# lucieDLE/TMRNet

Measured on AMD Instinct MI355X. Metric: train frames/sec, TMRNet ResNet50 seq=10 LFB=40, higher is better.
Workload: dtype fp32; 1 GPU; C2/C3: TMRNet ResNet50+LSTM+NLBlock train step; model=resnet_lstm (train_only_non-local_pretrained), global_batch=64, clips_per_gpu=64, seq_len=10, lfb_len=40, parallelism=dp1, input_transform=reference train transform (use_flip=1) on device

## Files before the change

### include/tmr.h

```cpp
#ifndef TMR_H_
#define TMR_H_

#ifdef TMR_HOST_ONLY
typedef struct ihipStream_t* hipStream_t;
#else
#include <hip/hip_runtime.h>
#endif
#include <stddef.h>
#include <stdint.h>

#ifdef __cplusplus
extern "C" {
#endif

#define TMR_ABI_VERSION 8

int tmr_abi_version(void);
const char* tmr_last_error(void);
void tmr_clear_error(void);

typedef struct tmr_conv_desc {
  int n, h, w, c;
  int k;
  int r, s, stride, pad;
  int ho, wo;
  int pad_w;
  int x_ld, y_ld;
  int math;
  int max_frames;
  int io;
  int groups;
} tmr_conv_desc;
#define TMR_MATH_F32 0
#define TMR_MATH_BF16 1
#define TMR_IO_X_BF16 1
#define TMR_IO_W_BF16 2
#define TMR_IO_DY_BF16 4
#define TMR_IO_Y_BF16 16
#define TMR_IO_BN_BF16 32
#define TMR_IO_G16 128
#define TMR_IO_WT_BF16 8
#define TMR_IO_ENGINE 256
#define TMR_IO_CLASSES 512
#define TMR_IO_TILES 1024
#define TMR_IO_WT_F32 64

int tmr_conv2d_fwd(const tmr_conv_desc* d, const float* x, const float* w_krsc,
                   const float* bias, float* y, float beta, hipStream_t stream);
int tmr_conv2d_fwd_fused(const tmr_conv_desc* d, const float* x, const float* w_krsc,
                         const float* scale, const float* shift, const float* residual, float* y,
                         int relu, hipStream_t stream);
int tmr_conv2d_fwd_stats_parts(const tmr_conv_desc* d);
int tmr_conv2d_fwd_bnstats(const tmr_conv_desc* d, const float* x, const float* w_krsc, float* y,
                           void* stats, size_t stats_bytes, hipStream_t stream);
int tmr_conv2d_dgrad(const tmr_conv_desc* d, const float* dy, const float* w_krsc, float* dx,
                     float beta, hipStream_t stream);
int tmr_conv2d_dgrad_bnbwd_parts(const tmr_conv_desc* d);
int tmr_conv2d_dgrad_bnbwd(const tmr_conv_desc* d, const float* dy, const float* w_krsc, float* dx,
                           float beta, const float* y, const float* z, const float* scale,
                           const float* shift, const float* mean, int mask, void* parts,
                           size_t parts_bytes, hipStream_t stream);
size_t tmr_conv2d_wgrad_ws_bytes(const tmr_conv_desc* d);
int tmr_conv2d_wgrad(const tmr_conv_desc* d, const float* x, const float* dy, float* dw_oihw,
                     int c_real, float beta, float* ws, size_t ws_bytes, hipStream_t stream);
int tmr_conv2d_dgrad_bnbwd_acc(const tmr_conv_desc* d, const float* dy, const float* w_krsc,
                               void* dx, float beta, const void* dx_old, int old_bf16,
                               const float* y, const float* z, const float* scale,
                               const float* shift, const float* mean, int mask, void* parts,
                               size_t parts_bytes, hipStream_t stream);
int tmr_gemm_nt(int M, int N, int K, const float* A, int lda, const float* B, int ldb,
                const float* bias, float* C, int ldc, float beta, hipStream_t stream);
int tmr_gemm_nn(int M, int N, int K, const float* A, int lda, const float* B, int ldb, float* C,
                int ldc, float beta, hipStream_t stream);
int tmr_gemm_tn(int M, int N, int K, const float* A, int lda, const float* B, int ldb, float* C,
                int ldc, float beta, hipStream_t stream);

int tmr_weight_oihw_to_krsc(const float* w, float* wk, int k, int c, int r, int s, int cpad,
                            hipStream_t stream);
int tmr_nchw_to_nhwc(const float* x, float* y, int n, int c, int h, int w, int cpad,
                     hipStream_t stream);
int tmr_nhwc_to_nchw(const float* x, float* y, int n, int c, int cstore, int h, int w,
                     hipStream_t stream);
int tmr_crop_normalize(const uint8_t* frames, const int32_t* offsets, float* out, int f, int hin,
                       int win, int seq_len, int crop, float m0, float m1, float m2, float s0,
                       float s1, float s2, hipStream_t stream);

typedef struct tmr_clip_aug {
  int32_t x1, y1;
  int32_t flip;
  int32_t rotate;
  int32_t a[6];
  int32_t jitter;
  int32_t hue_shift;
  float brightness, contrast, saturation;
  int32_t reserved;
} tmr_clip_aug;
int tmr_clip_augment(const uint8_t* frames, const tmr_clip_aug* params, int32_t* lmean, float* out,
                     int f, int hin, int win, int crop, float m0, float m1, float m2, float s0,
                     float s1, float s2, hipStream_t stream);

size_t tmr_bn_ws_bytes(int rows, int c);
int tmr_bn_fwd_stats(const float* y, int rows, int c, const float* gamma, const float* beta,
                     float* running_mean, float* running_var, float momentum, float eps,
                     float* save_mean, float* save_invstd, float* scale, float* shift, void* ws,
                     size_t ws_bytes, hipStream_t stream);
int tmr_bn_finalize(const void* partials, int nparts, int c, const float* gamma, const float* beta,
                    float* running_mean, float* running_var, float momentum, float eps,
                    float* save_mean, float* save_invstd, float* scale, float* shift,
                    hipStream_t stream);
size_t tmr_bn_parts_ws_bytes(int nparts, int c);
int tmr_bn_finalize_ws(const void* partials, int nparts, int c, const float* gamma,
                       const float* beta, float* running_mean, float* running_var, float momentum,
                       float eps, float* save_mean, float* save_invstd, float* scale, float* shift,
                       void* ws, size_t ws_bytes, hipStream_t stream);
int tmr_bn_eval_params(const float* gamma, const float* beta, const float* running_mean,
                       const float* running_var, float eps, int c, float* scale, float* shift,
                       hipStream_t stream);
int tmr_bn_apply(const float* y, const float* scale, const float* shift, const float* residual,
                 float* z, int rows, int c, int relu, hipStream_t stream);
int tmr_bn_apply2(const float* y, const float* scale, const float* shift, const float* yr,
                  const float* rscale, const float* rshift, float* z, int rows, int c, int relu,
                  hipStream_t stream);
int tmr_bn_bwd_maxpool(const float* dyp, const uint8_t* argmax, int n, int h, int w, int ho, int wo,
                       const float* y, const float* scale, const float* shift,
                       const float* save_mean, const float* save_invstd, const float* gamma,
                       float* dy, float* dgamma, float* dbeta, int c, void* ws, size_t ws_bytes,
                       hipStream_t stream);
int tmr_bn_bwd_parts(const float* g, const float* y, const void* parts, int nparts,
                     const float* save_mean, const float* save_invstd, const float* gamma,
                     float* dy, float* dgamma, float* dbeta, int rows, int c, void* ws,
                     size_t ws_bytes, hipStream_t stream);
int tmr_bn_bwd(const float* dz, const float* y, const float* z, const float* scale,
               const float* shift, const float* save_mean, const float* save_invstd,
               const float* gamma, float* dy, float* dres, float* dgamma, float* dbeta, int rows,
               int c, int relu, void* ws, size_t ws_bytes, hipStream_t stream);

int tmr_bn_apply_x(const float* y, const float* scale, const float* shift, const float* residual,
                   void* z, int rows, int c, int relu, int out_bf16, hipStream_t stream);
int tmr_bn_bwd_parts_x(const float* g, const float* y, const void* parts, int nparts,
                       const float* save_mean, const float* save_invstd, const float* gamma,
                       void* dy, float* dgamma, float* dbeta, int rows, int c, void* ws,
                       size_t ws_bytes, int out_bf16, hipStream_t stream);
int tmr_bn_bwd_x(const float* dz, const float* y, const float* z, const float* scale,
                 const float* shift, const float* save_mean, const float* save_invstd,
                 const float* gamma, void* dy, float* dres, float* dgamma, float* dbeta, int rows,
                 int c, int relu, void* ws, size_t ws_bytes, int out_bf16, hipStream_t stream);
int tmr_bn_bwd_maxpool_x(const float* dyp, const uint8_t* argmax, int n, int h, int w, int ho,
                         int wo, const float* y, const float* scale, const float* shift,
                         const float* save_mean, const float* save_invstd, const float* gamma,
                         void* dy, float* dgamma, float* dbeta, int c, void* ws, size_t ws_bytes,
                         int out_bf16, hipStream_t stream);
int tmr_weight_oihw_to_krsc_x(const float* w, void* wk, int k, int c, int r, int s, int cpad,
                              int out_bf16, hipStream_t stream);
int tmr_weight_oihw_to_crsk_x(const float* w, void* wt, int k, int c, int r, int s, int out_bf16,
                              hipStream_t stream);
typedef struct tmr_wlayout {
  const float* w;
  void* out;
  long long n;
  long long block0;
  int k, c, rs, cpad;
  int kind, bf16;
} tmr_wlayout;
int tmr_weight_layouts_epb(void);
int tmr_weight_layouts_multi(const tmr_wlayout* table, int n, int total_blocks, hipStream_t stream);
int tmr_bn_apply_dual(const float* y, const float* scale, const float* shift, const float* residual,
                      float* z, void* z16, int rows, int c, int relu, hipStream_t stream);
int tmr_bn_apply_bits(const float* y, const float* scale, const float* shift,
                      const float* residual, float* z, uint32_t* bits, int rows, int c,
                      hipStream_t stream);
int tmr_bn_apply2_bits(const float* y, const float* scale, const float* shift, const float* yr,
                       const float* rscale, const float* rshift, float* z, uint32_t* bits,
                       int rows, int c, hipStream_t stream);
int tmr_bn_apply2_x(const float* y, const float* scale, const float* shift, const float* yr,
                    const float* rscale, const float* rshift, float* z, void* z16, int rows, int c,
                    int relu, hipStream_t stream);
int tmr_maxpool2d_fwd_bn_x(const float* x, const float* scale, const float* shift, void* y,
                           uint8_t* argmax, int n, int h, int w, int c, int ho, int wo, int out_bf16,
                           hipStream_t stream);

int tmr_bn_apply_a16(const void* y, const float* scale, const float* shift, const void* residual,
                     void* z, int rows, int c, int relu, hipStream_t stream);
int tmr_bn_apply2_a16(const void* y, const float* scale, const float* shift, const void* yr,
                      const float* rscale, const float* rshift, void* z, int rows, int c, int relu,
                      hipStream_t stream);
int tmr_bn_apply_bits_a16(const void* y, const float* scale, const float* shift,
                          const void* residual, void* z, uint32_t* bits, int rows, int c,
                          hipStream_t stream);
int tmr_bn_apply2_bits_a16(const void* y, const float* scale, const float* shift, const void* yr,
                           const float* rscale, const float* rshift, void* z, uint32_t* bits,
                           int rows, int c, hipStream_t stream);
int tmr_bn_bwd_a16(const float* dz, const void* y, const void* z, const float* scale,
                   const float* shift, const float* save_mean, const float* save_invstd,
                   const float* gamma, void* dy, float* dres, float* dgamma, float* dbeta, int rows,
                   int c, int relu, void* ws, size_t ws_bytes, hipStream_t stream);
int tmr_bn_bwd_parts_a16(const float* g, const void* y, const void* parts, int nparts,
                         const float* save_mean, const float* save_invstd, const float* gamma,
                         void* dy, float* dgamma, float* dbeta, int rows, int c, void* ws,
                         size_t ws_bytes, hipStream_t stream);
int tmr_bn_bwd_parts_g16(const void* g, const void* y, const void* parts, int nparts,
                         const float* save_mean, const float* save_invstd, const float* gamma,
                         void* dy, float* dgamma, float* dbeta, int rows, int c, void* ws,
                         size_t ws_bytes, hipStream_t stream);
int tmr_bn_bwd_g16(const void* dz, const void* y, const float* save_mean,
                   const float* save_invstd, const float* gamma, void* dy, float* dgamma,
                   float* dbeta, int rows, int c, void* ws, size_t ws_bytes, hipStream_t stream);
size_t tmr_bn_bwd_parts_ds_ws_bytes(int nparts, int rows, int c);
int tmr_bn_bwd_parts_ds(const void* g, const void* y, const void* parts, int nparts,
                        const float* save_mean, const float* save_invstd, const float* gamma,
                        void* dy, float* dgamma, float* dbeta, const void* y_ds,
                        const float* save_mean_ds, const float* save_invstd_ds,
                        const float* gamma_ds, void* dy_ds, float* dgamma_ds, float* dbeta_ds,
                        int rows, int c, int bf16, void* ws, size_t ws_bytes, hipStream_t stream);
int tmr_bn_bwd_maxpool_a16(const float* dyp, const uint8_t* argmax, int n, int h, int w, int ho,
                           int wo, const void* y, const float* scale, const float* shift,
                           const float* save_mean, const float* save_invstd, const float* gamma,
                           void* dy, float* dgamma, float* dbeta, int c, void* ws, size_t ws_bytes,
                           hipStream_t stream);
int tmr_maxpool2d_fwd_bn_a16(const void* x, const float* scale, const float* shift, void* y,
                             uint8_t* argmax, int n, int h, int w, int c, int ho, int wo,
                             hipStream_t stream);
int tmr_avgpool_fwd_a16(const void* x, float* y, int n, int hw, int c, hipStream_t stream);
int tmr_cast_f32_bf16(const float* x, void* y, long n, hipStream_t stream);
int tmr_nhwc4_to_bf16x8(const float* x4, void* y8, long npix, hipStream_t stream);

int tmr_resize_ksize(int in_size, int out_size);
int tmr_resize_coeffs(int in_size, int out_size, int32_t* bounds, int32_t* k, int ksize);
size_t tmr_resize_tmp_bytes(int n, int h, int w, int oh, int ow);
int tmr_resize_u8(const uint8_t* in, int n, int h, int w, uint8_t* tmp, size_t tmp_bytes,
                  uint8_t* out, int oh, int ow, const int32_t* bounds_h, const int32_t* k_h,
                  int ksize_h, const int32_t* bounds_v, const int32_t* k_v, int ksize_v, int y0,
                  int y1, hipStream_t stream);
#define TMR_RESIZE_BOX_INTS 10
int tmr_resize_u8_boxes(const uint8_t* in, int n, int h, int w, const int32_t* desc_host,
                        const int32_t* desc, const int32_t* pool, long pool_ints, uint8_t* tmp,
                        size_t tmp_bytes, uint8_t* out, int oh, int ow, hipStream_t stream);

size_t tmr_margin_ws_bytes(int n, int h, int w);
int tmr_margin_boxes(const uint8_t* in, int n, int h, int w, void* ws, size_t ws_bytes,
                     int32_t* boxes, hipStream_t stream);
int tmr_margin_mask(const uint8_t* in, int n, int h, int w, void* ws, size_t ws_bytes,
                    uint8_t* mask, hipStream_t stream);
int tmr_frame_sums(const uint8_t* in, int n, int h, int w, int64_t* sums, hipStream_t stream);

#define TMR_JPEG_GRAY 0
#define TMR_JPEG_444 1
#define TMR_JPEG_420 2
typedef struct tmr_jpeg_info {
  int32_t width, height;
  int32_t ncomp;
  int32_t sampling;
  int32_t blocks_w[3], blocks_h[3];
  uint16_t qt[3][64];
  uint64_t coef_bytes;
} tmr_jpeg_info;
int tmr_jpeg_probe(const uint8_t* data, size_t len, tmr_jpeg_info* info);
int tmr_jpeg_entropy_decode(const uint8_t* data, size_t len, tmr_jpeg_info* info, int16_t* coef,
                            size_t coef_bytes);
size_t tmr_jpeg_ws_bytes(int f, int h, int w, int sampling);
int tmr_jpeg_reconstruct(const int16_t* coef, const uint16_t* qt, int f, int h, int w,
                         int sampling, uint8_t* ws, size_t ws_bytes, uint8_t* out,
                         const int32_t* out_index, int out_frames, hipStream_t stream);

int tmr_maxpool2d_fwd(const float* x, float* y, uint8_t* argmax, int n, int h, int w, int c,
                      int ho, int wo, hipStream_t stream);
int tmr_maxpool2d_bwd(const float* dy, const uint8_t* argmax, float* dx, int n, int h, int w,
                      int c, int ho, int wo, hipStream_t stream);
int tmr_maxpool2d_fwd_bn(const float* x, const float* scale, const float* shift, float* y,
                         uint8_t* argmax, int n, int h, int w, int c, int ho, int wo,
                         hipStream_t stream);
int tmr_avgpool_fwd(const float* x, float* y, int n, int hw, int c, hipStream_t stream);
int tmr_avgpool_bwd(const float* dy, float* dx, int n, int hw, int c, hipStream_t stream);

int tmr_splat_gap(const float* x, float* gap, int n, int hw, int c, hipStream_t stream);
int tmr_splat_combine(const float* x, const float* z, float* att, float* out, int n, int hw, int c,
                      hipStream_t stream);
int tmr_splat_bwd(const float* dout, const float* x, const float* att, float* dz, int n, int hw,
                  int c, hipStream_t stream);
int tmr_splat_bwd_apply(const float* dout, const float* att, const float* dgap, float* dx, int n,
                        int hw, int c, hipStream_t stream);
int tmr_center_cols(const float* x, int rows, int cols, float* center, float* xc,
                    hipStream_t stream);
int tmr_axpy(int n, float alpha, const float* x, float* y, hipStream_t stream);
int tmr_avgpool2d_fwd(const float* x, float* y, int n, int h, int w, int c, int ho, int wo, int k,
                      int s, int p, int count_include_pad, hipStream_t stream);
int tmr_avgpool2d_bwd(const float* dy, float* dx, int n, int h, int w, int c, int ho, int wo, int k,
                      int s, int p, int count_include_pad, hipStream_t stream);

int tmr_splat_gap_bn(const void* y, const float* scale, const float* shift, float* gap, int n,
                     int hw, int c, int act16, hipStream_t stream);
int tmr_splat_att(const float* zl, float* att, int n, int c, hipStream_t stream);
int tmr_splat_combine_bn(const void* y, const float* scale, const float* shift, const float* att,
                         void* out, int n, int hw, int c, int act16, hipStream_t stream);
int tmr_splat_bwd_reduce_bn(const float* dout, const void* y, const float* scale,
                            const float* shift, const float* mean, const float* att, float* dzl,
// ... 147 lines not shown
```

### tmrnet_amd/_lib.py

```python
import ctypes
import os

import torch

_HERE = os.path.dirname(os.path.abspath(__file__))
LIB_PATH = os.environ.get("TMR_LIB_PATH") or os.path.join(_HERE, "libtmr.so")

P = ctypes.c_void_p
I = ctypes.c_int
L = ctypes.c_long
F = ctypes.c_float
U64 = ctypes.c_uint64
SZ = ctypes.c_size_t


class ConvDesc(ctypes.Structure):
    _fields_ = [(n, ctypes.c_int) for n in
                ("n", "h", "w", "c", "k", "r", "s", "stride", "pad", "ho", "wo", "pad_w",
                 "x_ld", "y_ld", "math", "max_frames", "io", "groups")]


DP = ctypes.POINTER(ConvDesc)


_NL_FIELDS = ("w1", "b1", "w2", "b2", "w3", "b3", "ln_w", "ln_b", "w4", "b4")


class NLBlockPtrs(ctypes.Structure):
    _fields_ = [(n, ctypes.c_void_p) for n in _NL_FIELDS]


class JpegInfo(ctypes.Structure):
    _fields_ = [("width", ctypes.c_int32), ("height", ctypes.c_int32), ("ncomp", ctypes.c_int32),
                ("sampling", ctypes.c_int32), ("blocks_w", ctypes.c_int32 * 3),
                ("blocks_h", ctypes.c_int32 * 3), ("qt", (ctypes.c_uint16 * 64) * 3),
                ("coef_bytes", ctypes.c_uint64)]


JP = ctypes.POINTER(JpegInfo)

SIGNATURES = {
    "tmr_abi_version": [],
    "tmr_last_error": [],
    "tmr_clear_error": [],
    "tmr_conv2d_fwd": [DP, P, P, P, P, F, P],
    "tmr_conv2d_fwd_fused": [DP, P, P, P, P, P, P, I, P],
    "tmr_conv2d_fwd_stats_parts": [DP],
    "tmr_conv2d_fwd_bnstats": [DP, P, P, P, P, SZ, P],
    "tmr_conv2d_dgrad": [DP, P, P, P, F, P],
    "tmr_conv2d_dgrad_bnbwd_parts": [DP],
    "tmr_conv2d_dgrad_bnbwd": [DP, P, P, P, F, P, P, P, P, P, I, P, SZ, P],
    "tmr_conv2d_wgrad_ws_bytes": [DP],
    "tmr_conv2d_wgrad": [DP, P, P, P, I, F, P, SZ, P],
    "tmr_conv2d_dgrad_bnbwd_acc": [DP, P, P, P, F, P, I, P, P, P, P, P, I, P, SZ, P],
    "tmr_bn_apply_x": [P, P, P, P, P, I, I, I, I, P],
    "tmr_bn_bwd_parts_x": [P, P, P, I, P, P, P, P, P, P, I, I, P, SZ, I, P],
    "tmr_bn_bwd_x": [P, P, P, P, P, P, P, P, P, P, P, P, I, I, I, P, SZ, I, P],
    "tmr_bn_bwd_maxpool_x": [P, P, I, I, I, I, I, P, P, P, P, P, P, P, P, P, I, P, SZ, I, P],
    "tmr_weight_oihw_to_krsc_x": [P, P, I, I, I, I, I, I, P],
    "tmr_weight_oihw_to_crsk_x": [P, P, I, I, I, I, I, P],
    "tmr_bn_apply_dual": [P, P, P, P, P, P, I, I, I, P],
    "tmr_bn_apply2_x": [P, P, P, P, P, P, P, P, I, I, I, P],
    "tmr_bn_apply_bits": [P, P, P, P, P, P, I, I, P],
    "tmr_bn_apply2_bits": [P, P, P, P, P, P, P, P, I, I, P],
    "tmr_maxpool2d_fwd_bn_x": [P, P, P, P, P, I, I, I, I, I, I, I, P],
    "tmr_bn_apply_a16": [P, P, P, P, P, I, I, I, P],
    "tmr_bn_apply2_a16": [P, P, P, P, P, P, P, I, I, I, P],
    "tmr_bn_apply_bits_a16": [P, P, P, P, P, P, I, I, P],
    "tmr_bn_apply2_bits_a16": [P, P, P, P, P, P, P, P, I, I, P],
    "tmr_bn_bwd_a16": [P, P, P, P, P, P, P, P, P, P, P, P, I, I, I, P, SZ, P],
    "tmr_bn_bwd_parts_a16": [P, P, P, I, P, P, P, P, P, P, I, I, P, SZ, P],
    "tmr_bn_bwd_parts_g16": [P, P, P, I, P, P, P, P, P, P, I, I, P, SZ, P],
    "tmr_bn_bwd_g16": [P, P, P, P, P, P, P, P, I, I, P, SZ, P],
    "tmr_weight_layouts_epb": [],
    "tmr_weight_layouts_multi": [P, I, I, P],
    "tmr_bn_bwd_parts_ds_ws_bytes": [I, I, I],
    "tmr_bn_bwd_parts_ds": [P, P, P, I, P, P, P, P, P, P, P, P, P, P, P, P, P, I, I, I, P, SZ, P],
    "tmr_bn_bwd_maxpool_a16": [P, P, I, I, I, I, I, P, P, P, P, P, P, P, P, P, I, P, SZ, P],
    "tmr_maxpool2d_fwd_bn_a16": [P, P, P, P, P, I, I, I, I, I, I, P],
    "tmr_avgpool_fwd_a16": [P, P, I, I, I, P],
    "tmr_cast_f32_bf16": [P, P, ctypes.c_long, P],
    "tmr_nhwc4_to_bf16x8": [P, P, ctypes.c_long, P],
    "tmr_adam_step_multi": [P, I, ctypes.c_int64, P, P],
    "tmr_resize_ksize": [I, I],
    "tmr_resize_coeffs": [I, I, P, P, I],
    "tmr_resize_tmp_bytes": [I, I, I, I, I],
    "tmr_resize_u8": [P, I, I, I, P, SZ, P, I, I, P, P, I, P, P, I, I, I, P],
    "tmr_resize_u8_boxes": [P, I, I, I, P, P, P, L, P, SZ, P, I, I, P],
    "tmr_margin_ws_bytes": [I, I, I],
    "tmr_margin_boxes": [P, I, I, I, P, SZ, P, P],
    "tmr_margin_mask": [P, I, I, I, P, SZ, P, P],
    "tmr_frame_sums": [P, I, I, I, P, P],
    "tmr_jpeg_probe": [P, SZ, JP],
    "tmr_jpeg_entropy_decode": [P, SZ, JP, P, SZ],
    "tmr_jpeg_ws_bytes": [I, I, I, I],
    "tmr_jpeg_reconstruct": [P, P, I, I, I, I, P, SZ, P, P, I, P],
    "tmr_gemm_nt": [I, I, I, P, I, P, I, P, P, I, F, P],
    "tmr_gemm_nn": [I, I, I, P, I, P, I, P, I, F, P],
    "tmr_gemm_tn": [I, I, I, P, I, P, I, P, I, F, P],
    "tmr_weight_oihw_to_krsc": [P, P, I, I, I, I, I, P],
    "tmr_nchw_to_nhwc": [P, P, I, I, I, I, I, P],
    "tmr_nhwc_to_nchw": [P, P, I, I, I, I, I, P],
    "tmr_clip_augment": [P, P, P, P, I, I, I, I, F, F, F, F, F, F, P],
    "tmr_crop_normalize": [P, P, P, I, I, I, I, I, F, F, F, F, F, F, P],
    "tmr_bn_ws_bytes": [I, I],
    "tmr_bn_fwd_stats": [P, I, I, P, P, P, P, F, F, P, P, P, P, P, SZ, P],
    "tmr_bn_finalize": [P, I, I, P, P, P, P, F, F, P, P, P, P, P],
    "tmr_bn_finalize_ws": [P, I, I, P, P, P, P, F, F, P, P, P, P, P, SZ, P],
    "tmr_bn_parts_ws_bytes": [I, I],
    "tmr_bn_eval_params": [P, P, P, P, F, I, P, P, P],
    "tmr_bn_apply": [P, P, P, P, P, I, I, I, P],
    "tmr_bn_apply2": [P, P, P, P, P, P, P, I, I, I, P],
    "tmr_bn_bwd_parts": [P, P, P, I, P, P, P, P, P, P, I, I, P, SZ, P],
    "tmr_bn_bwd_maxpool": [P, P, I, I, I, I, I, P, P, P, P, P, P, P, P, P, I, P, SZ, P],
    "tmr_bn_bwd": [P, P, P, P, P, P, P, P, P, P, P, P, I, I, I, P, SZ, P],
    "tmr_maxpool2d_fwd": [P, P, P, I, I, I, I, I, I, P],
    "tmr_maxpool2d_fwd_bn": [P, P, P, P, P, I, I, I, I, I, I, P],
    "tmr_maxpool2d_bwd": [P, P, P, I, I, I, I, I, I, P],
    "tmr_avgpool_fwd": [P, P, I, I, I, P],
    "tmr_avgpool_bwd": [P, P, I, I, I, P],
    "tmr_splat_gap": [P, P, I, I, I, P],
    "tmr_splat_combine": [P, P, P, P, I, I, I, P],
    "tmr_splat_bwd": [P, P, P, P, I, I, I, P],
    "tmr_splat_bwd_apply": [P, P, P, P, I, I, I, P],
    "tmr_splat_gap_bn": [P, P, P, P, I, I, I, I, P],
    "tmr_splat_att": [P, P, I, I, P],
    "tmr_splat_combine_bn": [P, P, P, P, P, I, I, I, I, P],
    "tmr_splat_bwd_reduce_bn": [P, P, P, P, P, P, P, P, I, I, I, I, P],
    "tmr_splat_bn0_coefs": [P, P, P, P, P, P, P, P, P, I, I, I, P],
    "tmr_splat_bwd_apply_bn": [P, P, P, P, P, P, P, P, P, I, I, I, I, P],
    "tmr_avgpool2d_fwd_a16": [P, P, I, I, I, I, I, I, I, I, I, I, P],
    "tmr_fill_f32": [P, L, F, P],
    "tmr_seq_last": [P, P, I, I, I, P],
    "tmr_seq_last_bwd": [P, P, P, I, I, I, P],
    "tmr_counters_add": [P, I, ctypes.c_int64, P],
    "tmr_center_cols": [P, I, I, P, P, P],
    "tmr_axpy": [I, F, P, P, P],
    "tmr_avgpool2d_fwd": [P, P, I, I, I, I, I, I, I, I, I, I, P],
    "tmr_avgpool2d_bwd": [P, P, I, I, I, I, I, I, I, I, I, I, P],
    "tmr_col_sum": [P, I, I, I, P, F, P],
    "tmr_dropout_mask": [P, L, F, U64, U64, P],
    "tmr_softmax_max": [P, I, I, P, P, P, P],
    "tmr_ce_sum": [P, P, P, I, I, F, P, P, P, P],
    "tmr_sgd_chunk": [],
    "tmr_sgd_step_multi": [P, I, ctypes.c_int64, P, P],
    "tmr_sgd_step": [P, P, P, L, F, F, F, F, I, I, P],
    "tmr_lfb_index": [P, I, P, I, I, P, P],
    "tmr_lfb_gather": [P, P, P, L, I, P],
    "tmr_layernorm_relu_fwd": [P, P, P, P, P, P, I, I, F, P],
    "tmr_layernorm_relu_bwd": [P, P, P, P, P, P, P, P, P, I, I, P],
    "tmr_residual_mask": [P, P, P, P, L, P],
    "tmr_mask_relu_fwd": [P, P, P, L, P],
    "tmr_mask_relu_bwd": [P, P, P, P, L, P],
    "tmr_mul": [P, P, P, P, L, P],
    "tmr_nl_attn_ws_bytes": [I, I, I],
    "tmr_nl_attn_fwd": [P, P, P, P, P, I, I, I, F, P, SZ, P],
    "tmr_nl_attn_bwd": [P, P, P, P, P, P, P, I, I, I, F, P, SZ, P],
    "tmr_linear_fwd": [P, I, I, I, P, P, P, P],
    "tmr_linear_bwd": [P, P, I, I, I, P, P, P, P, F, P],
    "tmr_nlblock_saved_bytes": [I, I],
    "tmr_nlblock_ws_bytes": [I, I],
    "tmr_nlblock_fwd": [P, P, P, P, I, I, P, P, P, SZ, P, SZ, P],
    "tmr_nlblock_bwd": [P, P, P, P, P, I, I, P, P, SZ, P, P, P, P, SZ, P],
    "tmr_timeconv_saved_bytes": [I, I],
    "tmr_timeconv_ws_bytes": [I, I],
    "tmr_timeconv_fwd": [P, I, I, P, P, P, P, P, P, P, P, SZ, P, SZ, P],
    "tmr_timeconv_wgrad": [P, P, I, I, P, P, P, P, SZ, P, P, P, P, P, P, P, P, SZ, P],
    "tmr_lstm_saved_bytes": [I, I, I],
    "tmr_lstm_ws_bytes": [I, I, I, I],
    "tmr_lstm_fwd": [P, I, I, I, I, P, P, P, P, P, P, P, P, SZ, P, SZ, P],
    "tmr_lstm_bwd": [P, P, I, I, I, I, P, P, P, P, SZ, P, P, P, P, P, P, SZ, P],
    "tmr_lstm_window_ws_bytes": [I, I, I],
    "tmr_lstm_window_fwd": [P, L, P, I, I, I, P, P, P, P, SZ, P],
    "tmr_lstm_sync_status": [P,ctypes.POINTER(ctypes.c_uint), P],
    "tmr_lstm_status_or": [P, P, P],
    "tmr_test_hold_cus": [I, F, P],
    "tmr_dgrad_ws_launches": [],
    "tmr_timeconv_max5_fwd": [P, P, P, P, P, P, I, I, I, P],
    "tmr_timeconv_max5_bwd": [P, P, P, P, P, P, I, I, I, P],
    "tmr_lstm_cell_fwd": [P, I, P, P, P, I, P, P, I, I, P],
    "tmr_lstm_cell_bwd": [P, I, P, P, P, P, P, P, I, P, I, I, P],
}
_RESTYPES = {
    "tmr_last_error": ctypes.c_char_p,
    "tmr_clear_error": None,
    "tmr_conv2d_wgrad_ws_bytes": SZ,
    "tmr_dgrad_ws_launches": L,
    "tmr_resize_tmp_bytes": SZ,
    "tmr_margin_ws_bytes": SZ,
    "tmr_jpeg_ws_bytes": SZ,
    "tmr_bn_ws_bytes": SZ,
    "tmr_bn_parts_ws_bytes": SZ,
    "tmr_bn_bwd_parts_ds_ws_bytes": SZ,
    "tmr_sgd_chunk": ctypes.c_int64,
    "tmr_nl_attn_ws_bytes": SZ,
    "tmr_nlblock_saved_bytes": SZ,
    "tmr_nlblock_ws_bytes": SZ,
    "tmr_timeconv_saved_bytes": SZ,
    "tmr_timeconv_ws_bytes": SZ,
    "tmr_lstm_saved_bytes": SZ,
    "tmr_lstm_ws_bytes": SZ,
    "tmr_lstm_window_ws_bytes": SZ,
}

_lib = None


def lib():
    global _lib
    if _lib is None:
        if not os.path.exists(LIB_PATH):
            raise RuntimeError(
                "libtmr.so not found at %s: build it with `make` or "
                "`python -c 'import __graft_entry__ as g; g.build()'` (no CPU fallback exists)"
                % LIB_PATH)
        h = ctypes.CDLL(LIB_PATH)
        for name, args in SIGNATURES.items():
            fn = getattr(h, name)
            fn.argtypes = args
            fn.restype = _RESTYPES.get(name, ctypes.c_int)
        _lib = h
    return _lib


def exported_symbols():
    return list(SIGNATURES)


def _conv(a):
    if isinstance(a, torch.Tensor):
        return ctypes.c_void_p(a.data_ptr())
    return a


def stream_ptr(device=None):
    return ctypes.c_void_p(torch.cuda.current_stream(device).cuda_stream)


def call(name, *args):
    fn = getattr(lib(), name)
    rc = fn(*[_conv(a) for a in args])
    if rc != 0:
        raise RuntimeError("%s failed (%d): %s" % (name, rc, lib().tmr_last_error().decode()))
    return rc


def query(name, *args):
    h = lib()
    h.tmr_clear_error()
    fn = getattr(h, name)
    v = fn(*[_conv(a) for a in args])
    err = h.tmr_last_error()
    if (_RESTYPES.get(name, ctypes.c_int) is ctypes.c_int and v < 0) or err:
        raise RuntimeError("%s failed (%d): %s" % (name, v, (err or b"").decode()))
    return v
```

### tmrnet_amd/csrc/bn.hip

```cpp
#include "common.h"
#include "tmr.h"
#include <type_traits>

namespace {

constexpr int NT = 256;

struct Plan {
  int cthreads;
  int rthreads;
  int cblocks;
  int rpb;
  int nrb;
};

Plan make_plan(int rows, int c) {
  Plan p;
  int c4 = c / 4;
  p.cthreads = c4 < 64 ? c4 : 64;
  p.rthreads = NT / p.cthreads;
  p.cblocks = c4 / p.cthreads;
  int rpb = rows / 1024;
  int minr = p.rthreads * 8;
  if (rpb < minr) rpb = minr;
// ... 914 lines not shown
        ld8(y, pix * c8 + cq, v);
#pragma unroll
        for (int e = 0; e < 8; ++e) g[e] = 0.f;
#pragma unroll
        for (int ddy = 0; ddy < 2; ++ddy)
#pragma unroll
          for (int ddx = 0; ddx < 2; ++ddx) {
            if (ddy > py || ddx > px || !pin[ddy][ddx]) continue;
            const uint32_t id = (uint32_t)((py + 1 - 2 * ddy) * 3 + (px + 1 - 2 * ddx));
            const float dv[8] = {d0[ddy][ddx].x, d0[ddy][ddx].y, d0[ddy][ddx].z, d0[ddy][ddx].w,
                                 d1[ddy][ddx].x, d1[ddy][ddx].y, d1[ddy][ddx].z, d1[ddy][ddx].w};
#pragma unroll
            for (int e = 0; e < 8; ++e) {
              const uint32_t ab = ((e < 4 ? a[ddy][ddx].x : a[ddy][ddx].y) >> (8 * (e & 3))) & 0xffu;
              if (ab == id) g[e] += dv[e];
            }
          }
        float o[8];
#pragma unroll
        for (int e = 0; e < 8; ++e) {
          const float gm = fmaf(v[e], sc[e], sf[e]) > 0.f ? g[e] : 0.f;
          o[e] = fmaf(A[e], gm, fmaf(B[e], v[e], C[e]));
        }
        st8(dy, pix * c8 + cq, o);
      }
  }
}

#ifndef TMR_BN_BITS8
#define TMR_BN_BITS8 1
#endif
template <bool RES>
__global__ __launch_bounds__(NT) void bn_apply_bits8_k(const float* __restrict__ y,
                                                       const float* __restrict__ scale,
                                                       const float* __restrict__ shift,
                                                       const float* __restrict__ res,
                                                       const float* __restrict__ yr,
                                                       const float* __restrict__ rscale,
                                                       const float* __restrict__ rshift,
                                                       float* __restrict__ z,
                                                       uint32_t* __restrict__ bits, long n8, int c8) {
  const int lane = threadIdx.x & 63;
  const long stride = (long)gridDim.x * NT;
  auto apply = [&](long i, const float (&yv)[8], const float (&rv)[8]) -> uint32_t {
    const int cc = chan_of(i, c8) * 8;
    float v[8];
#pragma unroll
    for (int h = 0; h < 2; ++h) {
      const float4 sc = *reinterpret_cast<const float4*>(scale + cc + 4 * h);
      const float4 sf = *reinterpret_cast<const float4*>(shift + cc + 4 * h);
      const float s4[4] = {sc.x, sc.y, sc.z, sc.w}, f4[4] = {sf.x, sf.y, sf.z, sf.w};
      if (yr) {
        const float4 rs = *reinterpret_cast<const float4*>(rscale + cc + 4 * h);
        const float4 rf = *reinterpret_cast<const float4*>(rshift + cc + 4 * h);
        const float r4[4] = {rs.x, rs.y, rs.z, rs.w}, q4[4] = {rf.x, rf.y, rf.z, rf.w};
#pragma unroll
        for (int e = 0; e < 4; ++e)
          v[4 * h + e] = fmaf(yv[4 * h + e], s4[e], f4[e]) + fmaf(rv[4 * h + e], r4[e], q4[e]);
      } else {
#pragma unroll
        for (int e = 0; e < 4; ++e) {
          v[4 * h + e] = fmaf(yv[4 * h + e], s4[e], f4[e]);
          if (RES) v[4 * h + e] += rv[4 * h + e];
        }
      }
    }
    uint32_t b = 0;
#pragma unroll
    for (int e = 0; e < 8; ++e) {
      v[e] = fmaxf(v[e], 0.f);
      b |= (uint32_t)(v[e] > 0.f) << e;
    }
    st8(z, i, v);
    return b;
  };
  auto put = [&](uint32_t byte, long i, bool ok) {
    uint32_t w = byte << (8 * (lane & 3));
    w |= (uint32_t)__shfl_xor((int)w, 1, 64);
    w |= (uint32_t)__shfl_xor((int)w, 2, 64);
    if ((lane & 3) == 0 && ok) bits[i >> 2] = w;
  };
  const float* rsrc = RES ? res : yr;
  for (long base = blockIdx.x * (long)NT + (threadIdx.x & ~63); base < n8; base += 2 * stride) {
    const long i = base + lane, j = i + stride;
    const bool oi = i < n8, oj = j < n8;
    float ya[8], ra[8], yb[8], rb[8];
    if (oi) {
      ld8(y, i, ya);
      if (rsrc) ld8(rsrc, i, ra);
    }
    if (oj) {
      ld8(y, j, yb);
      if (rsrc) ld8(rsrc, j, rb);
    }
    const uint32_t bi = oi ? apply(i, ya, ra) : 0u;
    const uint32_t bj = oj ? apply(j, yb, rb) : 0u;
    put(bi, i, oi);
    put(bj, j, oj);
  }
}

int ew_blocks(long n4) {
  long b = (n4 + NT - 1) / NT;
  if (b > 2048 * 4) b = 2048 * 4;
  return (int)(b > 0 ? b : 1);
}

}

TMR_API size_t tmr_bn_ws_bytes(int rows, int c) {
  if (rows <= 0 || c < 4 || c % 4) {
    tmr_set_error("tmr_bn_ws_bytes: bad size (rows %d, channels %d)", rows, c);
    return 0;
  }
  return ws_need(rows, c);
}

TMR_API int tmr_bn_fwd_stats(const float* y, int rows, int c, const float* gamma,
                             const float* beta, float* running_mean, float* running_var,
                             float momentum, float eps, float* save_mean, float* save_invstd,
                             float* scale, float* shift, void* ws, size_t ws_bytes,
                             hipStream_t stream) {
  TMR_CHECK_ARG(c % 4 == 0 && c >= 4, "tmr_bn_fwd_stats: channels %d must be a multiple of 4", c);
  TMR_CHECK_ARG(rows > 0, "tmr_bn_fwd_stats: empty input");
  TMR_CHECK_ARG(plan_covers(c), "tmr_bn_fwd_stats: unsupported channel count %d", c);
  TMR_CHECK_ARG(ws && ws_bytes >= ws_need(rows, c), "tmr_bn_fwd_stats: workspace too small");
  Plan p = make_plan(rows, c);
  float4* part = (float4*)ws;
  hipLaunchKernelGGL(bn_stats_partial, dim3(p.nrb, p.cblocks), dim3(NT), 0, stream, y, rows, c,
                     p.rpb, p.cthreads, part);
  TMR_CHECK_LAUNCH("bn_stats_partial");
  return tmr_bn_finalize(part, p.nrb, c, gamma, beta, running_mean, running_var, momentum, eps,
                         save_mean, save_invstd, scale, shift, stream);
}

TMR_API int tmr_bn_finalize(const void* partials, int nparts, int c, const float* gamma,
                            const float* beta, float* running_mean, float* running_var,
                            float momentum, float eps, float* save_mean, float* save_invstd,
                            float* scale, float* shift, hipStream_t stream) {
  TMR_CHECK_ARG(nparts > 0 && c > 0, "tmr_bn_finalize: empty partials");
  hipLaunchKernelGGL(bn_finalize_k, dim3(c), dim3(NT), 0, stream, (const float4*)partials,
                     nparts, c, gamma, beta, running_mean, running_var, momentum, eps, save_mean,
                     save_invstd, scale, shift);
  TMR_CHECK_LAUNCH("bn_finalize");
  return 0;
}

TMR_API size_t tmr_bn_parts_ws_bytes(int nparts, int c) {
  if (nparts <= 0 || c <= 0) {
    tmr_set_error("tmr_bn_parts_ws_bytes: bad size (parts %d, channels %d)", nparts, c);
    return 0;
  }
  return slab_ws_bytes(nparts, c) + (size_t)3 * c * sizeof(float) + 64;
}

TMR_API int tmr_bn_finalize_ws(const void* partials, int nparts, int c, const float* gamma,
                               const float* beta, float* running_mean, float* running_var,
                               float momentum, float eps, float* save_mean, float* save_invstd,
                               float* scale, float* shift, void* ws, size_t ws_bytes,
                               hipStream_t stream) {
  TMR_CHECK_ARG(nparts > 0 && c > 0, "tmr_bn_finalize_ws: empty partials");
  TMR_CHECK_ARG(ws && ws_bytes >= slab_ws_bytes(nparts, c), "tmr_bn_finalize_ws: workspace too small");
  const SlabPlan p = slab_plan(nparts, c);
  hipLaunchKernelGGL(parts_slab_k<0>, dim3(p.groups, p.nslabs), dim3(256), 0, stream, partials,
                     nparts, c, p.rows, (double*)ws);
  TMR_CHECK_LAUNCH("bn_parts_slab");
  hipLaunchKernelGGL(finalize_slabs_k, dim3(p.groups), dim3(SLAB_CH * SLAB_PH), 0, stream,
                     (const double*)ws, p.nslabs, (const float4*)partials, c, gamma, beta,
                     running_mean, running_var, momentum, eps, save_mean, save_invstd, scale,
                     shift);
  TMR_CHECK_LAUNCH("bn_finalize_slabs");
  return 0;
}

TMR_API int tmr_bn_eval_params(const float* gamma, const float* beta, const float* running_mean,
                               const float* running_var, float eps, int c, float* scale,
                               float* shift, hipStream_t stream) {
  hipLaunchKernelGGL(bn_eval_params_k, dim3(cdiv(c, 256)), dim3(256), 0, stream, gamma, beta,
                     running_mean, running_var, eps, c, scale, shift);
  TMR_CHECK_LAUNCH("bn_eval_params");
  return 0;
}

TMR_API int tmr_bn_apply(const float* y, const float* scale, const float* shift,
                         const float* residual, float* z, int rows, int c, int relu,
                         hipStream_t stream) {
  return tmr_bn_apply_x(y, scale, shift, residual, z, rows, c, relu, 0, stream);
}

TMR_API int tmr_bn_apply_x(const float* y, const float* scale, const float* shift,
                           const float* residual, void* zv, int rows, int c, int relu,
                           int out_bf16, hipStream_t stream) {
  TMR_CHECK_ARG(c % 4 == 0, "tmr_bn_apply: channels %d must be a multiple of 4", c);
  long n4 = (long)rows * c / 4;
  int nb = ew_blocks(n4);
  int c4 = c / 4;
  if (out_bf16) {
    TMR_CHECK_ARG(!residual, "tmr_bn_apply_x: a bf16 output is for conv-operand-only tensors (no residual)");
    if (relu) hipLaunchKernelGGL((bn_apply_k<false, true, __bf16>), dim3(nb), dim3(NT), 0, stream, y, scale, shift, residual, (__bf16*)zv, n4, c4);
    else hipLaunchKernelGGL((bn_apply_k<false, false, __bf16>), dim3(nb), dim3(NT), 0, stream, y, scale, shift, residual, (__bf16*)zv, n4, c4);
    TMR_CHECK_LAUNCH("bn_apply");
    return 0;
  }
  float* z = (float*)zv;
  if (residual) {
    if (relu) hipLaunchKernelGGL((bn_apply_k<true, true>), dim3(nb), dim3(NT), 0, stream, y, scale, shift, residual, z, n4, c4);
    else hipLaunchKernelGGL((bn_apply_k<true, false>), dim3(nb), dim3(NT), 0, stream, y, scale, shift, residual, z, n4, c4);
  } else {
    if (relu) hipLaunchKernelGGL((bn_apply_k<false, true>), dim3(nb), dim3(NT), 0, stream, y, scale, shift, residual, z, n4, c4);
    else hipLaunchKernelGGL((bn_apply_k<false, false>), dim3(nb), dim3(NT), 0, stream, y, scale, shift, residual, z, n4, c4);
  }
  TMR_CHECK_LAUNCH("bn_apply");
  return 0;
}

TMR_API int tmr_bn_apply2(const float* y, const float* scale, const float* shift, const float* yr,
                          const float* rscale, const float* rshift, float* z, int rows, int c,
                          int relu, hipStream_t stream) {
  return tmr_bn_apply2_x(y, scale, shift, yr, rscale, rshift, z, nullptr, rows, c, relu, stream);
}

TMR_API int tmr_bn_apply2_x(const float* y, const float* scale, const float* shift, const float* yr,
                            const float* rscale, const float* rshift, float* z, void* z16,
                            int rows, int c, int relu, hipStream_t stream) {
  TMR_CHECK_ARG(c % 4 == 0, "tmr_bn_apply2: channels %d must be a multiple of 4", c);
  TMR_CHECK_ARG(y && scale && shift && yr && rscale && rshift && z, "tmr_bn_apply2: null operand");
  TMR_CHECK_ARG(yr != z, "tmr_bn_apply2: the branch input must not alias z");
  const long n4 = (long)rows * c / 4;
  __bf16* h = (__bf16*)z16;
  if (relu && h)
    hipLaunchKernelGGL((bn_apply2_k<true, true>), dim3(ew_blocks(n4)), dim3(NT), 0, stream, y, scale,
                       shift, yr, rscale, rshift, z, n4, c / 4, h);
  else if (relu)
    hipLaunchKernelGGL((bn_apply2_k<true>), dim3(ew_blocks(n4)), dim3(NT), 0, stream, y, scale, shift,
                       yr, rscale, rshift, z, n4, c / 4, h);
  else if (h)
    hipLaunchKernelGGL((bn_apply2_k<false, true>), dim3(ew_blocks(n4)), dim3(NT), 0, stream, y, scale,
                       shift, yr, rscale, rshift, z, n4, c / 4, h);
  else
    hipLaunchKernelGGL((bn_apply2_k<false>), dim3(ew_blocks(n4)), dim3(NT), 0, stream, y, scale, shift,
                       yr, rscale, rshift, z, n4, c / 4, h);
  TMR_CHECK_LAUNCH("bn_apply2");
  return 0;
}

TMR_API int tmr_bn_apply_bits(const float* y, const float* scale, const float* shift,
                              const float* residual, float* z, uint32_t* bits, int rows, int c,
                              hipStream_t stream) {
  TMR_CHECK_ARG(c % 4 == 0 && y && scale && shift && z && bits,
                "tmr_bn_apply_bits: null operand or channels %d not a multiple of 4", c);
  const long n4 = (long)rows * c / 4;
  if (n4 == 0) return 0;
  if (TMR_BN_BITS8 && c % 8 == 0 && (((uintptr_t)y | (uintptr_t)residual | (uintptr_t)z) & 15) == 0) {
    if (residual)
      hipLaunchKernelGGL((bn_apply_bits8_k<true>), dim3(ew_blocks(n4 / 2)), dim3(NT), 0, stream, y,
                         scale, shift, residual, nullptr, nullptr, nullptr, z, bits, n4 / 2, c / 8);
    else
      hipLaunchKernelGGL((bn_apply_bits8_k<false>), dim3(ew_blocks(n4 / 2)), dim3(NT), 0, stream, y,
                         scale, shift, nullptr, nullptr, nullptr, nullptr, z, bits, n4 / 2, c / 8);
  } else if (residual)
    hipLaunchKernelGGL((bn_apply_bits_k<true, float>), dim3(ew_blocks(n4)), dim3(NT), 0, stream, y, scale,
                       shift, residual, nullptr, nullptr, nullptr, z, bits, n4, c / 4);
  else
    hipLaunchKernelGGL((bn_apply_bits_k<false, float>), dim3(ew_blocks(n4)), dim3(NT), 0, stream, y, scale,
                       shift, nullptr, nullptr, nullptr, nullptr, z, bits, n4, c / 4);
  TMR_CHECK_LAUNCH("bn_apply_bits");
  return 0;
}

TMR_API int tmr_bn_apply2_bits(const float* y, const float* scale, const float* shift,
                               const float* yr, const float* rscale, const float* rshift, float* z,
                               uint32_t* bits, int rows, int c, hipStream_t stream) {
  TMR_CHECK_ARG(c % 4 == 0 && y && scale && shift && yr && rscale && rshift && z && bits,
                "tmr_bn_apply2_bits: null operand or channels %d not a multiple of 4", c);
  TMR_CHECK_ARG(yr != z, "tmr_bn_apply2_bits: the branch input must not alias z");
  const long n4 = (long)rows * c / 4;
  if (n4 == 0) return 0;
  if (TMR_BN_BITS8 && c % 8 == 0 && (((uintptr_t)y | (uintptr_t)yr | (uintptr_t)z) & 15) == 0)
    hipLaunchKernelGGL((bn_apply_bits8_k<false>), dim3(ew_blocks(n4 / 2)), dim3(NT), 0, stream, y,
                       scale, shift, nullptr, yr, rscale, rshift, z, bits, n4 / 2, c / 8);
  else
    hipLaunchKernelGGL((bn_apply_bits_k<false, float>), dim3(ew_blocks(n4)), dim3(NT), 0, stream, y, scale,
                       shift, nullptr, yr, rscale, rshift, z, bits, n4, c / 4);
  TMR_CHECK_LAUNCH("bn_apply2_bits");
  return 0;
}

TMR_API int tmr_bn_apply_bits_a16(const void* y, const float* scale, const float* shift,
                                  const void* residual, void* z, uint32_t* bits, int rows, int c,
                                  hipStream_t stream) {
  TMR_CHECK_ARG(c % 4 == 0 && y && scale && shift && z && bits,
                "tmr_bn_apply_bits_a16: null operand or channels %d not a multiple of 4", c);
  const long n4 = (long)rows * c / 4;
  if (n4 == 0) return 0;
  const __bf16* yb = (const __bf16*)y;
  if (residual)
    hipLaunchKernelGGL((bn_apply_bits_k<true, __bf16>), dim3(ew_blocks(n4)), dim3(NT), 0, stream, yb,
                       scale, shift, (const __bf16*)residual, nullptr, nullptr, nullptr, (__bf16*)z,
                       bits, n4, c / 4);
  else
    hipLaunchKernelGGL((bn_apply_bits_k<false, __bf16>), dim3(ew_blocks(n4)), dim3(NT), 0, stream, yb,
                       scale, shift, nullptr, nullptr, nullptr, nullptr, (__bf16*)z, bits, n4, c / 4);
  TMR_CHECK_LAUNCH("bn_apply_bits_a16");
  return 0;
}

// ... 55 lines not shown
  double* part = (double*)ws;
  float* coef = (float*)((char*)ws + (size_t)p.nrb * c * 2 * sizeof(double));
  const dim3 pg(p.nrb, p.cblocks);
  float* dzw = const_cast<float*>(dz);
  if (dres == dz) {
    if (mask == 1)
      hipLaunchKernelGGL((bn_bwd_partial<1, true>), pg, dim3(NT), 0, stream, dzw, y, z, scale, shift, save_mean, rows, c, p.rpb, p.cthreads, part);
    else if (mask == 2)
      hipLaunchKernelGGL((bn_bwd_partial<2, true>), pg, dim3(NT), 0, stream, dzw, y, z, scale, shift, save_mean, rows, c, p.rpb, p.cthreads, part);
    else
      hipLaunchKernelGGL((bn_bwd_partial<0>), pg, dim3(NT), 0, stream, dzw, y, z, scale, shift, save_mean, rows, c, p.rpb, p.cthreads, part);
    mask = 0;
    dres = nullptr;
  } else if (mask == 1)
    hipLaunchKernelGGL((bn_bwd_partial<1>), pg, dim3(NT), 0, stream, dzw, y, z, scale, shift, save_mean, rows, c, p.rpb, p.cthreads, part);
  else if (mask == 2)
    hipLaunchKernelGGL((bn_bwd_partial<2>), pg, dim3(NT), 0, stream, dzw, y, z, scale, shift, save_mean, rows, c, p.rpb, p.cthreads, part);
  else
    hipLaunchKernelGGL((bn_bwd_partial<0>), pg, dim3(NT), 0, stream, dzw, y, z, scale, shift, save_mean, rows, c, p.rpb, p.cthreads, part);
  TMR_CHECK_LAUNCH("bn_bwd_partial");
  hipLaunchKernelGGL(bn_bwd_final, dim3(c), dim3(NT), 0, stream, part, p.nrb, rows, c,
                     save_mean, save_invstd, gamma, dgamma, dbeta, coef);
  TMR_CHECK_LAUNCH("bn_bwd_final");
  long n4 = (long)rows * c / 4;
  int nb = ew_blocks(n4);
  int c4 = c / 4;
#define TMR_BN_APPLY(M, D)                                                                     \
  if (out_bf16)                                                                                  \
    hipLaunchKernelGGL((bn_bwd_apply<M, D, __bf16>), dim3(nb), dim3(NT), 0, stream, dz, y, z,    \
                       scale, shift, coef, (__bf16*)dyv, dres, n4, c4);                          \
  else                                                                                           \
    hipLaunchKernelGGL((bn_bwd_apply<M, D>), dim3(nb), dim3(NT), 0, stream, dz, y, z, scale,     \
                       shift, coef, (float*)dyv, dres, n4, c4)
  if (dres) {
    if (mask == 1) { TMR_BN_APPLY(1, true); } else if (mask == 2) { TMR_BN_APPLY(2, true); } else { TMR_BN_APPLY(0, true); }
  } else {
    if (mask == 1) { TMR_BN_APPLY(1, false); } else if (mask == 2) { TMR_BN_APPLY(2, false); } else { TMR_BN_APPLY(0, false); }
  }
#undef TMR_BN_APPLY
  TMR_CHECK_LAUNCH("bn_bwd_apply");
  return 0;
}

TMR_API int tmr_bn_bwd_maxpool(const float* dyp, const uint8_t* argmax, int n, int h, int w,
                               int ho, int wo, const float* y, const float* scale,
                               const float* shift, const float* save_mean,
                               const float* save_invstd, const float* gamma, float* dy,
                               float* dgamma, float* dbeta, int c, void* ws, size_t ws_bytes,
                               hipStream_t stream) {
  return tmr_bn_bwd_maxpool_x(dyp, argmax, n, h, w, ho, wo, y, scale, shift, save_mean,
                              save_invstd, gamma, dy, dgamma, dbeta, c, ws, ws_bytes, 0, stream);
}

static int bn_bwd_maxpool_impl(const float* dyp, const uint8_t* argmax, int n, int h, int w,
                               int ho, int wo, const float* y, const float* scale,
                               const float* shift, const float* save_mean,
                               const float* save_invstd, const float* gamma, void* dyv,
                               float* dgamma, float* dbeta, int c, void* ws, size_t ws_bytes,
                               int out_bf16, float* coef_out, hipStream_t stream);

TMR_API int tmr_bn_bwd_maxpool_x(const float* dyp, const uint8_t* argmax, int n, int h, int w,
                                 int ho, int wo, const float* y, const float* scale,
                                 const float* shift, const float* save_mean,
                                 const float* save_invstd, const float* gamma, void* dyv,
                                 float* dgamma, float* dbeta, int c, void* ws, size_t ws_bytes,
                                 int out_bf16, hipStream_t stream) {
  TMR_CHECK_ARG(c >= 4 && plan_covers(c), "tmr_bn_bwd_maxpool: unsupported channel count %d", c);
  TMR_CHECK_ARG(dyv, "tmr_bn_bwd_maxpool: null dy");
  return bn_bwd_maxpool_impl(dyp, argmax, n, h, w, ho, wo, y, scale, shift, save_mean,
                             save_invstd, gamma, dyv, dgamma, dbeta, c, ws, ws_bytes, out_bf16,
                             nullptr, stream);
}

static int bn_bwd_maxpool_impl(const float* dyp, const uint8_t* argmax, int n, int h, int w,
                               int ho, int wo, const float* y, const float* scale,
                               const float* shift, const float* save_mean,
                               const float* save_invstd, const float* gamma, void* dyv,
                               float* dgamma, float* dbeta, int c, void* ws, size_t ws_bytes,
                               int out_bf16, float* coef_out, hipStream_t stream) {
  const long rows_l = (long)n * h * w;
  TMR_CHECK_ARG(c % 4 == 0 && c >= 4 && rows_l > 0 && rows_l < 0x7fffffffL,
                "tmr_bn_bwd_maxpool: bad shape n=%d h=%d w=%d c=%d", n, h, w, c);
  TMR_CHECK_ARG(ho == (h + 2 - 3) / 2 + 1 && wo == (w + 2 - 3) / 2 + 1,
                "tmr_bn_bwd_maxpool: pooled %dx%d is not MaxPool2d(3,2,1) of %dx%d", ho, wo, h, w);
  const int rows = (int)rows_l;
  TMR_CHECK_ARG(plan_covers(c), "tmr_bn_bwd_maxpool: unsupported channel count %d", c);
  TMR_CHECK_ARG(ws && ws_bytes >= ws_need(rows, c), "tmr_bn_bwd_maxpool: workspace too small");
  PoolGeo pg;
  pg.dyp = dyp; pg.am = (const uchar4*)argmax;
  pg.dHW = make_fastdiv((uint32_t)(h * w)); pg.dW = make_fastdiv((uint32_t)w);
  pg.ho = ho; pg.wo = wo;
  const int prows = n * ho * wo;
  Plan p = make_plan(prows, c);
  double* part = (double*)ws;
  float* coef = coef_out ? coef_out : (float*)((char*)ws + (size_t)p.nrb * c * 2 * sizeof(double));
  hipLaunchKernelGGL(stem_bwd_partial_pooled<float>, dim3(p.nrb, p.cblocks), dim3(NT), 0, stream, pg, h, w,
                     y, scale, shift, save_mean, prows, c, p.rpb, p.cthreads,
                     make_fastdiv((uint32_t)(ho * wo)), make_fastdiv((uint32_t)wo), part);
  TMR_CHECK_LAUNCH("stem_bwd_partial_pooled");
  hipLaunchKernelGGL(bn_bwd_final, dim3(c), dim3(NT), 0, stream, part, p.nrb, rows, c,
                     save_mean, save_invstd, gamma, dgamma, dbeta, coef);
  TMR_CHECK_LAUNCH("bn_bwd_final");
  if (!dyv) return 0;
  const long n4 = rows_l * c / 4;
  const int c8 = c / 8;
  if (c % 8 == 0 && (c8 & (c8 - 1)) == 0 && n4 / 2 < 0x7fffffffL &&
      (((uintptr_t)dyp | (uintptr_t)y | (uintptr_t)dyv) & 15) == 0 && ((uintptr_t)argmax & 7) == 0) {
    const int qh = (h + 1) / 2, qw = (w + 1) / 2;
    const int nq = n * qh * qw * c8;
    const FastDiv dqhw = make_fastdiv((uint32_t)(qh * qw)), dqw = make_fastdiv((uint32_t)qw);
    if (out_bf16)
      hipLaunchKernelGGL((stem_bwd_apply8q<float, __bf16>), dim3(ew_blocks(nq)), dim3(NT), 0, stream,
                         pg, h, w, dqhw, dqw, y, scale, shift, coef, (__bf16*)dyv, nq, __builtin_ctz(c8));
    else
      hipLaunchKernelGGL((stem_bwd_apply8q<float, float>), dim3(ew_blocks(nq)), dim3(NT), 0, stream,
                         pg, h, w, dqhw, dqw, y, scale, shift, coef, (float*)dyv, nq, __builtin_ctz(c8));
  } else if (out_bf16)
    hipLaunchKernelGGL(stem_bwd_apply<__bf16>, dim3(ew_blocks(n4)), dim3(NT), 0, stream, pg, y, scale,
                       shift, coef, (__bf16*)dyv, n4, c / 4);
  else
    hipLaunchKernelGGL(stem_bwd_apply<float>, dim3(ew_blocks(n4)), dim3(NT), 0, stream, pg, y, scale,
                       shift, coef, (float*)dyv, n4, c / 4);
  TMR_CHECK_LAUNCH("stem_bwd_apply");
  return 0;
}

TMR_API int tmr_bn_bwd_parts(const float* g, const float* y, const void* parts, int nparts,
                             const float* save_mean, const float* save_invstd, const float* gamma,
                             float* dy, float* dgamma, float* dbeta, int rows, int c, void* ws,
                             size_t ws_bytes, hipStream_t stream) {
  return tmr_bn_bwd_parts_x(g, y, parts, nparts, save_mean, save_invstd, gamma, dy, dgamma, dbeta,
                            rows, c, ws, ws_bytes, 0, stream);
}

TMR_API int tmr_bn_bwd_parts_x(const float* g, const float* y, const void* parts, int nparts,
                               const float* save_mean, const float* save_invstd,
                               const float* gamma, void* dyv, float* dgamma, float* dbeta,
                               int rows, int c, void* ws, size_t ws_bytes, int out_bf16,
                               hipStream_t stream) {
  TMR_CHECK_ARG(c % 4 == 0 && c >= 4 && rows > 0 && nparts > 0,
                "tmr_bn_bwd_parts: bad shape rows=%d c=%d parts=%d", rows, c, nparts);
  TMR_CHECK_ARG(ws && ws_bytes >= tmr_bn_parts_ws_bytes(nparts, c),
                "tmr_bn_bwd_parts: workspace too small (need tmr_bn_parts_ws_bytes)");
  const SlabPlan sp = slab_plan(nparts, c);
  double* slabs = (double*)ws;
  float* coef = (float*)((char*)ws + slab_ws_bytes(nparts, c));
  hipLaunchKernelGGL(parts_slab_k<1>, dim3(sp.groups, sp.nslabs), dim3(256), 0, stream, parts,
                     nparts, c, sp.rows, slabs);
  TMR_CHECK_LAUNCH("bn_parts_slab");
  hipLaunchKernelGGL(bwd_final_slabs_k, dim3(sp.groups), dim3(SLAB_CH * SLAB_PH), 0, stream,
                     (const double*)slabs, sp.nslabs, rows, c, save_mean, save_invstd, gamma,
                     dgamma, dbeta, coef);
  TMR_CHECK_LAUNCH("bn_bwd_final_slabs");
  const long n4 = (long)rows * c / 4;
  if (out_bf16)
    hipLaunchKernelGGL((bn_bwd_apply<0, false, __bf16, float>), dim3(ew_blocks(n4)), dim3(NT), 0, stream, g,
                       y, nullptr, nullptr, nullptr, coef, (__bf16*)dyv, nullptr, n4, c / 4);
  else if (c % 8 == 0 && (((uintptr_t)g | (uintptr_t)y | (uintptr_t)dyv) & 15) == 0)
    hipLaunchKernelGGL((bn_bwd_apply8_k<float, float, float>), dim3(ew_blocks(n4 / 2)), dim3(NT), 0,
                       stream, g, y, coef, (float*)dyv, n4 / 2, c / 8);
  else
    hipLaunchKernelGGL((bn_bwd_apply<0, false, float, float>), dim3(ew_blocks(n4)), dim3(NT), 0, stream, g, y,
                       nullptr, nullptr, nullptr, coef, (float*)dyv, nullptr, n4, c / 4);
  TMR_CHECK_LAUNCH("bn_bwd_apply");
  return 0;
}


static bool apply8_ok(int c, const void* y, const void* r, const void* z) {
  return c % 8 == 0 && (((uintptr_t)y | (uintptr_t)r | (uintptr_t)z) & 15) == 0;
}

TMR_API int tmr_bn_apply_a16(const void* y, const float* scale, const float* shift,
                             const void* residual, void* z, int rows, int c, int relu,
                             hipStream_t stream) {
  TMR_CHECK_ARG(c % 4 == 0 && y && scale && shift && z, "tmr_bn_apply_a16: bad arguments (c %d)", c);
  const long n4 = (long)rows * c / 4;
  const int nb = ew_blocks(n4), c4 = c / 4;
  const __bf16 *yb = (const __bf16*)y, *rb = (const __bf16*)residual;
  __bf16* zb = (__bf16*)z;
  if (apply8_ok(c, y, residual, z)) {
    const long n8 = n4 / 2;
    const int nb8 = ew_blocks(n8), c8 = c / 8;
    if (rb) {
      if (relu) hipLaunchKernelGGL((bn_apply8_a16_k<true, true, false>), dim3(nb8), dim3(NT), 0, stream, yb, scale, shift, rb, nullptr, nullptr, zb, n8, c8);
      else hipLaunchKernelGGL((bn_apply8_a16_k<true, false, false>), dim3(nb8), dim3(NT), 0, stream, yb, scale, shift, rb, nullptr, nullptr, zb, n8, c8);
    } else {
      if (relu) hipLaunchKernelGGL((bn_apply8_a16_k<false, true, false>), dim3(nb8), dim3(NT), 0, stream, yb, scale, shift, nullptr, nullptr, nullptr, zb, n8, c8);
      else hipLaunchKernelGGL((bn_apply8_a16_k<false, false, false>), dim3(nb8), dim3(NT), 0, stream, yb, scale, shift, nullptr, nullptr, nullptr, zb, n8, c8);
    }
  } else if (rb) {
    if (relu) hipLaunchKernelGGL((bn_apply_k<true, true, __bf16, false, __bf16>), dim3(nb), dim3(NT), 0, stream, yb, scale, shift, rb, zb, n4, c4, nullptr);
    else hipLaunchKernelGGL((bn_apply_k<true, false, __bf16, false, __bf16>), dim3(nb), dim3(NT), 0, stream, yb, scale, shift, rb, zb, n4, c4, nullptr);
  } else {
    if (relu) hipLaunchKernelGGL((bn_apply_k<false, true, __bf16, false, __bf16>), dim3(nb), dim3(NT), 0, stream, yb, scale, shift, rb, zb, n4, c4, nullptr);
    else hipLaunchKernelGGL((bn_apply_k<false, false, __bf16, false, __bf16>), dim3(nb), dim3(NT), 0, stream, yb, scale, shift, rb, zb, n4, c4, nullptr);
  }
  TMR_CHECK_LAUNCH("bn_apply_a16");
  return 0;
}

TMR_API int tmr_bn_apply2_a16(const void* y, const float* scale, const float* shift, const void* yr,
                              const float* rscale, const float* rshift, void* z, int rows, int c,
                              int relu, hipStream_t stream) {
  TMR_CHECK_ARG(c % 4 == 0, "tmr_bn_apply2_a16: channels %d must be a multiple of 4", c);
  TMR_CHECK_ARG(y && scale && shift && yr && rscale && rshift && z, "tmr_bn_apply2_a16: null operand");
  TMR_CHECK_ARG(yr != z, "tmr_bn_apply2_a16: the branch input must not alias z");
  const long n4 = (long)rows * c / 4;
  const __bf16 *yb = (const __bf16*)y, *rb = (const __bf16*)yr;
  if (apply8_ok(c, y, yr, z)) {
    const long n8 = n4 / 2;
    if (relu)
      hipLaunchKernelGGL((bn_apply8_a16_k<false, true, true>), dim3(ew_blocks(n8)), dim3(NT), 0,
                         stream, yb, scale, shift, rb, rscale, rshift, (__bf16*)z, n8, c / 8);
    else
      hipLaunchKernelGGL((bn_apply8_a16_k<false, false, true>), dim3(ew_blocks(n8)), dim3(NT), 0,
                         stream, yb, scale, shift, rb, rscale, rshift, (__bf16*)z, n8, c / 8);
  } else if (relu)
    hipLaunchKernelGGL((bn_apply2_k<true, false, __bf16, __bf16>), dim3(ew_blocks(n4)), dim3(NT), 0,
                       stream, yb, scale, shift, rb, rscale, rshift, (__bf16*)z, n4, c / 4, nullptr);
  else
    hipLaunchKernelGGL((bn_apply2_k<false, false, __bf16, __bf16>), dim3(ew_blocks(n4)), dim3(NT), 0,
                       stream, yb, scale, shift, rb, rscale, rshift, (__bf16*)z, n4, c / 4, nullptr);
  TMR_CHECK_LAUNCH("bn_apply2_a16");
  return 0;
}

TMR_API int tmr_bn_bwd_a16(const float* dz, const void* y, const void* z, const float* scale,
                           const float* shift, const float* save_mean, const float* save_invstd,
                           const float* gamma, void* dy, float* dres, float* dgamma, float* dbeta,
                           int rows, int c, int relu, void* ws, size_t ws_bytes,
                           hipStream_t stream) {
  TMR_CHECK_ARG(c % 4 == 0 && c >= 4, "tmr_bn_bwd_a16: channels %d must be a multiple of 4", c);
  TMR_CHECK_ARG(rows > 0, "tmr_bn_bwd_a16: empty input");
  TMR_CHECK_ARG(plan_covers(c), "tmr_bn_bwd_a16: unsupported channel count %d", c);
  TMR_CHECK_ARG(ws && ws_bytes >= ws_need(rows, c), "tmr_bn_bwd_a16: workspace too small");
  TMR_CHECK_ARG(!relu || z || (scale && shift),
                "tmr_bn_bwd_a16: relu backward needs the saved output z or the forward scale/shift");
  int mask = relu ? (z ? 1 : 2) : 0;
  Plan p = make_plan(rows, c);
  double* part = (double*)ws;
  float* coef = (float*)((char*)ws + (size_t)p.nrb * c * 2 * sizeof(double));
  const dim3 pg(p.nrb, p.cblocks);
  float* dzw = const_cast<float*>(dz);
  const __bf16 *yb = (const __bf16*)y, *zb = (const __bf16*)z;
  if (dres == dz) {
    if (mask == 1)
      hipLaunchKernelGGL((bn_bwd_partial<1, true, __bf16>), pg, dim3(NT), 0, stream, dzw, yb, zb, scale, shift, save_mean, rows, c, p.rpb, p.cthreads, part);
    else if (mask == 2)
      hipLaunchKernelGGL((bn_bwd_partial<2, true, __bf16>), pg, dim3(NT), 0, stream, dzw, yb, zb, scale, shift, save_mean, rows, c, p.rpb, p.cthreads, part);
    else
      hipLaunchKernelGGL((bn_bwd_partial<0, false, __bf16>), pg, dim3(NT), 0, stream, dzw, yb, zb, scale, shift, save_mean, rows, c, p.rpb, p.cthreads, part);
    mask = 0;
    dres = nullptr;
  } else if (mask == 1)
    hipLaunchKernelGGL((bn_bwd_partial<1, false, __bf16>), pg, dim3(NT), 0, stream, dzw, yb, zb, scale, shift, save_mean, rows, c, p.rpb, p.cthreads, part);
  else if (mask == 2)
    hipLaunchKernelGGL((bn_bwd_partial<2, false, __bf16>), pg, dim3(NT), 0, stream, dzw, yb, zb, scale, shift, save_mean, rows, c, p.rpb, p.cthreads, part);
  else
    hipLaunchKernelGGL((bn_bwd_partial<0, false, __bf16>), pg, dim3(NT), 0, stream, dzw, yb, zb, scale, shift, save_mean, rows, c, p.rpb, p.cthreads, part);
  TMR_CHECK_LAUNCH("bn_bwd_partial");
  hipLaunchKernelGGL(bn_bwd_final, dim3(c), dim3(NT), 0, stream, part, p.nrb, rows, c,
                     save_mean, save_invstd, gamma, dgamma, dbeta, coef);
  TMR_CHECK_LAUNCH("bn_bwd_final");
  const long n4 = (long)rows * c / 4;
  const int nb = ew_blocks(n4), c4 = c / 4;
  __bf16* db = (__bf16*)dy;
#define TMR_BN_APPLY16(M, D)                                                                    \
  hipLaunchKernelGGL((bn_bwd_apply<M, D, __bf16, __bf16>), dim3(nb), dim3(NT), 0, stream, dz, yb, \
                     zb, scale, shift, coef, db, dres, n4, c4)
  if (dres) {
    if (mask == 1) { TMR_BN_APPLY16(1, true); } else if (mask == 2) { TMR_BN_APPLY16(2, true); } else { TMR_BN_APPLY16(0, true); }
  } else if (mask == 0 && c % 8 == 0 && (((uintptr_t)dz | (uintptr_t)y | (uintptr_t)dy) & 15) == 0) {
    hipLaunchKernelGGL(bn_bwd_apply8_a16<float>, dim3(ew_blocks(n4 / 2)), dim3(NT), 0, stream, dz,
                       yb, coef, db, n4 / 2, c / 8);
  } else {
    if (mask == 1) { TMR_BN_APPLY16(1, false); } else if (mask == 2) { TMR_BN_APPLY16(2, false); } else { TMR_BN_APPLY16(0, false); }
  }
#undef TMR_BN_APPLY16
  TMR_CHECK_LAUNCH("bn_bwd_apply");
  return 0;
}

TMR_API int tmr_bn_bwd_g16(const void* dz, const void* y, const float* save_mean,
                           const float* save_invstd, const float* gamma, void* dy, float* dgamma,
                           float* dbeta, int rows, int c, void* ws, size_t ws_bytes,
                           hipStream_t stream) {
  TMR_CHECK_ARG(c % 8 == 0 && c >= 8 && rows > 0, "tmr_bn_bwd_g16: bad shape rows=%d c=%d", rows, c);
  TMR_CHECK_ARG((((uintptr_t)dz | (uintptr_t)y | (uintptr_t)dy) & 15) == 0,
                "tmr_bn_bwd_g16: dz / y / dy must be 16-B aligned");
  TMR_CHECK_ARG(plan_covers(c), "tmr_bn_bwd_g16: unsupported channel count %d", c);
  TMR_CHECK_ARG(ws && ws_bytes >= ws_need(rows, c), "tmr_bn_bwd_g16: workspace too small");
  Plan p = make_plan(rows, c);
  double* part = (double*)ws;
  float* coef = (float*)((char*)ws + (size_t)p.nrb * c * 2 * sizeof(double));
  const __bf16 *gb = (const __bf16*)dz, *yb = (const __bf16*)y;
  hipLaunchKernelGGL((bn_bwd_partial<0, false, __bf16, const __bf16>), dim3(p.nrb, p.cblocks), dim3(NT),
                     0, stream, gb, yb, nullptr, nullptr, nullptr, save_mean, rows, c, p.rpb,
                     p.cthreads, part);
  TMR_CHECK_LAUNCH("bn_bwd_partial_g16");
  hipLaunchKernelGGL(bn_bwd_final, dim3(c), dim3(NT), 0, stream, part, p.nrb, rows, c,
                     save_mean, save_invstd, gamma, dgamma, dbeta, coef);
  TMR_CHECK_LAUNCH("bn_bwd_final");
  const long n8 = (long)rows * c / 8;
  hipLaunchKernelGGL(bn_bwd_apply8_a16<__bf16>, dim3(ew_blocks(n8)), dim3(NT), 0, stream, gb, yb,
                     coef, (__bf16*)dy, n8, c / 8);
// ... 212 lines not shown
```

### tmrnet_amd/csrc/gemm16_kernel.h

```cpp
#pragma once
#include "gemm16_select.h"
#include <cstring>
#include <type_traits>

namespace tmrg {

typedef short s16x4_t __attribute__((ext_vector_type(4)));
typedef short s16x8_t __attribute__((ext_vector_type(8)));
#define TMR_LDS_AS __attribute__((address_space(3)))

__device__ __forceinline__ void glds16(__amdgpu_buffer_rsrc_t r, unsigned char* dst, uint32_t voff) {
  __builtin_amdgcn_raw_ptr_buffer_load_lds(r, (TMR_LDS_AS void*)dst, 16, voff, 0, 0, 0);
}

template <int R>
__device__ __forceinline__ int mn_swz(int k) {
  return R >= 128 ? ((k & 3) << 2) : (((k >> 1) & 1) << 2);
}

__device__ __forceinline__ void store_g8(const GemmArgs& a, long off, const float (&v)[8]) {
  if (a.g16) {
    uint32_t w[4];
#pragma unroll
    for (int e = 0; e < 4; ++e)
// ... 270 lines not shown
      if (n0 + c < a.N) a.bn_part[(long)(m0 / BM) * a.part_ld + n0 + c] = make_float2(t0, t1);
    }
  }
};

template <int BM, int BN, int WM, int WN, int TM, int TN>
__device__ __forceinline__ void epilogue_lds_bnbwd(const GemmArgs& a, floatx16 (&acc)[TM][TN],
                                                   float* lds, int lds_floats, int m0, int n0) {
  constexpr int NT = 64 * WM * WN;
  constexpr int LDC = BN + 4;
  constexpr int CG = BN / 8;
  constexpr int RPP = NT / CG;
  static_assert(NT % CG == 0, "threads per column group");
  int etid = threadIdx.x;
  asm volatile("" : "+v"(etid));
  const int lane = etid & 63, wave = etid >> 6;
  const int wm = wave / WN, wn = wave % WN;
  const int l31 = lane & 31, hh = lane >> 5;
  const int cg = etid % CG, rsub = etid / CG;
  const int col = n0 + 8 * cg;
  const bool okc = col < a.N;
  float mu[8], bsc[8], bsh[8], cs[8], cq[8];
#pragma unroll
  for (int e = 0; e < 8; ++e) {
    const int c = okc ? col + e : 0;
    mu[e] = okc ? a.bn_mean[c] : 0.f;
    bsc[e] = (okc && a.bn_mask == 2) ? a.bn_sc[c] : 0.f;
    bsh[e] = (okc && a.bn_mask == 2) ? a.bn_sh[c] : (a.bn_mask == 0 ? 1.f : 0.f);
    cs[e] = 0.f;
    cq[e] = 0.f;
  }
  const bool has_beta = a.beta != 0.f;
  const int rchunk = min(BM, (lds_floats / LDC) / (BM / WM) * (BM / WM));
  for (int r0 = 0; r0 < BM; r0 += rchunk) {
    __syncthreads();
    const int wr0 = wm * (BM / WM);
    if (wr0 >= r0 && wr0 < r0 + rchunk) {
#pragma unroll
      for (int i = 0; i < TM; ++i)
#pragma unroll
        for (int j = 0; j < TN; ++j)
#pragma unroll
          for (int r = 0; r < 16; ++r) {
            const int row = wr0 - r0 + 32 * i + (r & 3) + 8 * (r >> 2) + 4 * hh;
            lds[row * LDC + wn * (BN / WN) + 32 * j + l31] = acc[i][j][r];
          }
    }
    __syncthreads();
    const int nrow = min(rchunk, BM - r0);
    for (int rr = rsub; rr < nrow; rr += RPP) {
      const int row = m0 + r0 + rr;
      const bool ok = okc && row < a.M;
      long pix = row;
      if (ok && a.osy != 0) {
        const uint32_t n = fdiv((uint32_t)row, a.dHW);
        const uint32_t rem = row - n * a.dHW.d;
        const uint32_t y = fdiv(rem, a.dW);
        const uint32_t x = rem - y * a.dW.d;
        pix = ((long)n * a.oH + (long)y * a.osy + a.oyc) * a.oW + (long)x * a.osx + a.oxc;
      }
      const long off = pix * a.ldc + col;
      float yv[8], zv[8], old[8];
      if (ok) {
        if (a.bn16) {
          const uint4 yw = *reinterpret_cast<const uint4*>(reinterpret_cast<const __bf16*>(a.bn_y) + off);
          const uint32_t yu[4] = {yw.x, yw.y, yw.z, yw.w};
#pragma unroll
          for (int e = 0; e < 4; ++e) {
            yv[2 * e] = __uint_as_float(yu[e] << 16);
            yv[2 * e + 1] = __uint_as_float(yu[e] & 0xffff0000u);
          }
          if (a.bn_mask == 1) {
            const uint4 zw = *reinterpret_cast<const uint4*>(reinterpret_cast<const __bf16*>(a.bn_z) + off);
            const uint32_t zu[4] = {zw.x, zw.y, zw.z, zw.w};
#pragma unroll
            for (int e = 0; e < 4; ++e) {
              zv[2 * e] = __uint_as_float(zu[e] << 16);
              zv[2 * e + 1] = __uint_as_float(zu[e] & 0xffff0000u);
            }
          }
        } else {
          const float4 y0 = *reinterpret_cast<const float4*>(a.bn_y + off);
          const float4 y1 = *reinterpret_cast<const float4*>(a.bn_y + off + 4);
          yv[0] = y0.x; yv[1] = y0.y; yv[2] = y0.z; yv[3] = y0.w;
          yv[4] = y1.x; yv[5] = y1.y; yv[6] = y1.z; yv[7] = y1.w;
          if (a.bn_mask == 1) {
            const float4 z0 = *reinterpret_cast<const float4*>(a.bn_z + off);
            const float4 z1 = *reinterpret_cast<const float4*>(a.bn_z + off + 4);
            zv[0] = z0.x; zv[1] = z0.y; zv[2] = z0.z; zv[3] = z0.w;
            zv[4] = z1.x; zv[5] = z1.y; zv[6] = z1.z; zv[7] = z1.w;
          }
        }
        if (a.bn_mask == 3) {
          const uint32_t wrd = reinterpret_cast<const uint32_t*>(a.bn_z)[off >> 5];
          const uint32_t b8 = wrd >> (off & 31);
#pragma unroll
          for (int e = 0; e < 8; ++e) zv[e] = ((b8 >> e) & 1u) ? 1.f : 0.f;
        } else if (a.bn_mask != 1) {
#pragma unroll
          for (int e = 0; e < 8; ++e) zv[e] = 0.f;
        }
        if (has_beta) {
          uint4 c0, c1;
          load_old8(a, off, c0, c1);
          unpack_old8(a, c0, c1, old);
        } else {
#pragma unroll
          for (int e = 0; e < 8; ++e) old[e] = 0.f;
        }
        const float4 a0 = *reinterpret_cast<const float4*>(lds + rr * LDC + 8 * cg);
        const float4 a1 = *reinterpret_cast<const float4*>(lds + rr * LDC + 8 * cg + 4);
        const float av[8] = {a0.x, a0.y, a0.z, a0.w, a1.x, a1.y, a1.z, a1.w};
        float v[8];
#pragma unroll
        for (int e = 0; e < 8; ++e) {
          float t = fmaf(a.beta, old[e], av[e]);
          const bool keep = zv[e] + fmaf(yv[e], bsc[e], bsh[e]) > 0.f;
          t = keep ? t : 0.f;
          if (a.g16) t = bf16_rne(t);
          v[e] = t;
          cs[e] += t;
          cq[e] = fmaf(t, yv[e] - mu[e], cq[e]);
        }
        store_g8(a, off, v);
      }
    }
  }
  __syncthreads();
  float* red = lds;
#pragma unroll
  for (int e = 0; e < 8; ++e) {
    red[(rsub * BN + 8 * cg + e) * 2] = cs[e];
    red[(rsub * BN + 8 * cg + e) * 2 + 1] = cq[e];
  }
  __syncthreads();
  for (int c = etid; c < BN; c += NT) {
    float t0 = 0.f, t1 = 0.f;
    for (int q = 0; q < RPP; ++q) {
      t0 += red[(q * BN + c) * 2];
      t1 += red[(q * BN + c) * 2 + 1];
    }
    if (n0 + c < a.N) a.bn_part[(long)(m0 / BM) * a.part_ld + n0 + c] = make_float2(t0, t1);
  }
}

typedef float f32x4_t __attribute__((ext_vector_type(4)));

template <int BM, int BN, int WM, int WN, int NST>
constexpr int occ16() {
  return (WM * WN >= 16 || (WM * WN == 8 && (BM * BN <= 128 * 128 || NST == 1))) ? 4 : 2;
}

template <int MODE, int BM, int BN, int WM, int WN, int TAPV, int PIPE, int F32, int NST, int EPF = 0,
          int INF16 = 0>
__device__ __forceinline__ void gemm16_body(const GemmArgs& a, const int bid, const int split) {
  constexpr uint32_t ES = F32 ? 4u : 2u;
  constexpr int EPC = 16 / ES;
  constexpr int BK = 128 / ES;
  constexpr int NW = WM * WN;
  constexpr int TM = BM / WM / 32, TN = BN / WN / 32;
  constexpr bool MN = (MODE == MODE_WGRAD);
  constexpr int ABYTES = BM * 128, BBYTES = BN * 128, STAGE = ABYTES + BBYTES;
  constexpr int NIA = ABYTES / (1024 * NW), NIB = BBYTES / (1024 * NW);
  static_assert(NIA >= 1 && NIB >= 1 && NIA * 1024 * NW == ABYTES && NIB * 1024 * NW == BBYTES,
                "LDS-DMA pieces per wave");
  static_assert(TM >= 1 && TN >= 1, "wave tile");
  static_assert(!MN || (BM >= 64 && BN >= 64), "reduction-major images need >= 64 columns");
  constexpr int CPRA = BM * (int)ES / 16, CPRB = BN * (int)ES / 16;
  using Frag = typename std::conditional<F32 != 0, f32x4_t, bf16x8>::type;
  constexpr int EPI = WM * BN * 2 * 4;
  static_assert(NST == 2 || (NST == 1 && MODE != MODE_WGRAD), "one-stage form: FWD / DGRAD");
  constexpr int LDSROWB = (BN + 4) * (BM / WM) * 4, LDSFULL = (BN + 4) * BM * 4;
  constexpr int LDSNEED = MODE != MODE_DGRAD ? 0 : (LDSFULL <= 70 * 1024 ? LDSFULL : LDSROWB);
  constexpr int SMEM1 = STAGE > EPI ? (STAGE > LDSNEED ? STAGE : LDSNEED) : (EPI > LDSNEED ? EPI : LDSNEED);
  constexpr int SMEM2 = 2 * STAGE > EPI ? 2 * STAGE : EPI;
  constexpr int SMEM = NST == 1 ? SMEM1 : (SMEM2 > LDSNEED ? SMEM2 : LDSNEED);
  __shared__ __attribute__((aligned(1024))) unsigned char smem[SMEM];

  const int tid = threadIdx.x;
  const int lane = tid & 63;
  const int wave = __builtin_amdgcn_readfirstlane(tid >> 6);
  const int wm = wave / WN, wn = wave % WN;
  const int l31 = lane & 31, hh = lane >> 5;

  const int nnt = (a.N + BN - 1) / BN;
  const int m0 = (bid / nnt) * BM;
  const int n0 = (bid % nnt) * BN;

  int kbeg = 0, kend = a.K;
  if (MODE == MODE_WGRAD) {
    kbeg = split * a.kchunk;
    kend = min(a.K, kbeg + a.kchunk);
  }
  const int ntiles = kend > kbeg ? (kend - kbeg + BK - 1) / BK : 0;

  const __amdgpu_buffer_rsrc_t rA = make_rsrc(a.A, a.Abytes);
  const __amdgpu_buffer_rsrc_t rB = make_rsrc(a.B, a.Bbytes);
  const int cmask = (1 << a.log2C) - 1;

  auto kc_row = [&](int q) { return 8 * (wave + NW * q) + (lane >> 3); };
  auto kc_chunk = [&](int q) { return (lane & 7) ^ ((kc_row(q) >> 1) & 7); };

  uint32_t apix[MN ? 1 : NIA];
  int ay[MN ? 1 : NIA], ax[MN ? 1 : NIA], ach[MN ? 1 : NIA];
  bool aok[MN ? 1 : NIA];
  uint32_t aco[MN ? NIA : 1];
  int akr[MN ? NIA : 1];
  bool acok[MN ? NIA : 1];
  if constexpr (!MN) {
#pragma unroll
    for (int q = 0; q < NIA; ++q) {
      const int m = m0 + kc_row(q);
      aok[q] = m < a.M;
      const uint32_t mm = aok[q] ? (uint32_t)m : 0u;
      const uint32_t n = fdiv(mm, a.dHW);
      const uint32_t rem = mm - n * a.dHW.d;
      const uint32_t y = fdiv(rem, a.dW);
      const uint32_t x = rem - y * a.dW.d;
      ay[q] = (int)y * a.sy;
      ax[q] = (int)x * a.sx;
      apix[q] = (uint32_t)(((int)n * a.Hs + ay[q]) * a.Ws + ax[q]) * (uint32_t)a.lds * ES;
      ach[q] = EPC * kc_chunk(q);
    }
  } else {
#pragma unroll
    for (int q = 0; q < NIA; ++q) {
      const int s = 64 * (wave + NW * q) + lane;
      const int k = s / CPRA;
      const int ch = (s % CPRA) ^ (F32 ? (k & 1) << 3 : mn_swz<BM>(k));
      const int i = m0 + EPC * ch;
      akr[q] = k;
      acok[q] = i < a.M;
      aco[q] = (uint32_t)i * ES;
    }
  }
  uint32_t brow[MN ? 1 : NIB];
  int bch[MN ? 1 : NIB];
  bool bok[NIB];
  int bdy[MN ? NIB : 1], bdx[MN ? NIB : 1], bkr[MN ? NIB : 1];
  uint32_t bco[MN ? NIB : 1];
  if constexpr (!MN) {
#pragma unroll
    for (int q = 0; q < NIB; ++q) {
      const int j = n0 + kc_row(q);
      bok[q] = j < a.N;
      const uint32_t jj = bok[q] ? (uint32_t)j : 0u;
      brow[q] = jj * (uint32_t)(MODE == MODE_DGRAD ? a.ldbt : a.ldb) * ES;
      bch[q] = EPC * kc_chunk(q);
    }
  } else {
#pragma unroll
    for (int q = 0; q < NIB; ++q) {
      const int s = 64 * (wave + NW * q) + lane;
      const int k = s / CPRB;
      const int ch = (s % CPRB) ^ (F32 ? (k & 1) << 3 : mn_swz<BN>(k));
      const int j = n0 + EPC * ch;
      const int tap = a.ntaps == 1 ? 0 : (j >> a.log2C);
      const int c = a.ntaps == 1 ? j : (j & cmask);
      int ri, si;
      tap_split(a, tap, ri, si);
      bdy[q] = a.oy0 + a.dyr * ri;
      bdx[q] = a.ox0 + a.dxs * si;
      bco[q] = (uint32_t)c * ES;
      bok[q] = j < a.N && tap < a.ntaps;
      bkr[q] = k;
    }
  }

  auto stage = [&](int kt, int buf) {
    const int kb = kbeg + kt * BK;
    unsigned char* As = smem + buf * STAGE;
    unsigned char* Bs = As + ABYTES;
    if constexpr (!MN) {
      int tapU = 0, cbU = kb, dyU = a.oy0, dxU = a.ox0;
      if (!TAPV && a.ntaps != 1) {
        tapU = kb >> a.log2C;
        cbU = kb & cmask;
        int ri, si;
        tap_split(a, tapU, ri, si);
        dyU = a.oy0 + a.dyr * ri;
        dxU = a.ox0 + a.dxs * si;
      }
#pragma unroll
      for (int q = 0; q < NIA; ++q) {
        const int k = kb + ach[q];
        int tap = tapU, c = cbU + ach[q], dy = dyU, dx = dxU;
        if (TAPV) {
          tap = k >> a.log2C;
          c = k & cmask;
          int ri, si;
          tap_split(a, tap, ri, si);
          dy = a.oy0 + a.dyr * ri;
          dx = a.ox0 + a.dxs * si;
        }
        const int ys = ay[q] + dy, xs = ax[q] + dx;
        const bool ok = aok[q] && k < kend && tap < a.ntaps && (unsigned)ys < (unsigned)a.Hs &&
                        (unsigned)xs < (unsigned)a.Ws;
        const uint32_t off = apix[q] + (uint32_t)((dy * a.Ws + dx) * a.lds + c) * ES;
        glds16(rA, As + 1024 * (wave + NW * q), ok ? off : OOB);
      }
      if constexpr (MODE == MODE_FWD) {
#pragma unroll
        for (int q = 0; q < NIB; ++q) {
          const int k = kb + bch[q];
          const bool ok = bok[q] && k < kend;
          glds16(rB, Bs + 1024 * (wave + NW * q), ok ? brow[q] + (uint32_t)k * ES : OOB);
        }
      } else {
        int tapB = 0, coB = kb, rsB = 0;
        if (!TAPV) {
          if (a.ntaps != 1) {
            tapB = kb >> a.log2C;
            coB = kb & cmask;
          }
          int ri, si;
          tap_split(a, tapB, ri, si);
          rsB = (a.wr0 + a.wst * ri) * a.wS + (a.ws0 + a.wst * si);
        }
#pragma unroll
        for (int q = 0; q < NIB; ++q) {
          const int k = kb + bch[q];
          int tap = tapB, co = coB + bch[q], rs = rsB;
          if (TAPV) {
            tap = k >> a.log2C;
            co = k & cmask;
            int ri, si;
            tap_split(a, tap, ri, si);
            rs = (a.wr0 + a.wst * ri) * a.wS + (a.ws0 + a.wst * si);
          }
          const bool ok = bok[q] && k < kend && tap < a.ntaps;
          const uint32_t off = brow[q] + (uint32_t)((rs << a.log2C) + co) * ES;
          glds16(rB, Bs + 1024 * (wave + NW * q), ok ? off : OOB);
        }
      }
    } else {
#pragma unroll
      for (int q = 0; q < NIA; ++q) {
        const int m = kb + akr[q];
        const bool ok = acok[q] && m < kend;
        const uint32_t off = (uint32_t)m * (uint32_t)a.ldb * ES + aco[q];
        glds16(rA, As + 1024 * (wave + NW * q), ok ? off : OOB);
      }
#pragma unroll
      for (int q = 0; q < NIB; ++q) {
        const int m = kb + bkr[q];
        const uint32_t mm = m < kend ? (uint32_t)m : 0u;
        const uint32_t n = fdiv(mm, a.dHW);
        const uint32_t rem = mm - n * a.dHW.d;
        const uint32_t y = fdiv(rem, a.dW);
        const uint32_t x = rem - y * a.dW.d;
        const int ys = (int)y * a.sy + bdy[q], xs = (int)x * a.sx + bdx[q];
        const bool ok = m < kend && bok[q] && (unsigned)ys < (unsigned)a.Hs &&
                        (unsigned)xs < (unsigned)a.Ws;
        const uint32_t off = (uint32_t)(((int)n * a.Hs + ys) * a.Ws + xs) * (uint32_t)a.lds * ES + bco[q];
        glds16(rB, Bs + 1024 * (wave + NW * q), ok ? off : OOB);
      }
    }
  };

  const int kx = (l31 >> 1) & 7;
  const int tg = lane >> 4, tq = (lane >> 2) & 3, tp = lane & 3;
  auto tr_frag = [&](const unsigned char* img, int R, int swz, int cb, int s) -> bf16x8 {
    const int col = cb + 16 * (tg & 1) + 4 * tp;
    const int k0 = 16 * s + 8 * (tg >> 1) + tq;
    const uint32_t cbyte = (uint32_t)((((col >> 3) ^ swz) << 4) + (col & 7) * 2);
    const s16x4_t v0 = __builtin_amdgcn_ds_read_tr16_b64_v4i16(
        (TMR_LDS_AS s16x4_t*)(img + k0 * R * 2 + cbyte));
    const s16x4_t v1 = __builtin_amdgcn_ds_read_tr16_b64_v4i16(
        (TMR_LDS_AS s16x4_t*)(img + (k0 + 4) * R * 2 + cbyte));
    const s16x8_t w = __builtin_shufflevector(v0, v1, 0, 1, 2, 3, 4, 5, 6, 7);
    return __builtin_bit_cast(bf16x8, w);
  };
  const int swzA = mn_swz<BM>(tq), swzB = mn_swz<BN>(tq);
  auto mn_frag32 = [&](const unsigned char* img, int R, int cb, int s) -> f32x4_t {
    const int col = cb + l31;
    const uint32_t cbyte = (uint32_t)((((col >> 2) ^ (hh << 3)) << 4) + (col & 3) * 4);
    f32x4_t v;
#pragma unroll
    for (int t = 0; t < 4; ++t)
      v[t] = *reinterpret_cast<const float*>(img + (8 * s + 2 * t + hh) * R * 4 + cbyte);
    return v;
  };

  floatx16 acc[TM][TN];
#pragma unroll
  for (int i = 0; i < TM; ++i)
#pragma unroll
    for (int j = 0; j < TN; ++j)
#pragma unroll
      for (int r = 0; r < 16; ++r) acc[i][j][r] = 0.f;

  constexpr bool LDSEPI = MODE == MODE_DGRAD && LDSROWB <= SMEM;
  constexpr bool PRE = LDSEPI && NW < 8;
  constexpr int LATED = EPF != 0 ? TMR_EPI_LATE_F : TMR_EPI_LATE;
  constexpr bool LATE = LDSEPI && NW == 8 && LDSNEED == LDSFULL && LATED > 0;
  using Epi = LdsBnbwd<BM, BN, WM, WN, SMEM,
                      PRE ? (EPF == 1 ? TMR_EPI_DEPTH_F16 : TMR_EPI_DEPTH) : (LATE ? 0 : 1),
                      PRE ? (EPF == 1 ? TMR_EPI_TOPUP_F16 : (EPF == 2 ? TMR_EPI_TOPUP_F32 : TMR_EPI_TOPUP))
                          : (LATE ? LATED : 0),
                      EPF>;
  typename Epi::In pf[(PRE || LATE) ? Epi::DT : 1];
  if constexpr (PRE) {
    if (a.bn_part != nullptr) Epi::prefetch(a, m0, n0, pf);
  }

  const int arow0 = wm * (BM / WM) + l31;
  const int brow0 = wn * (BN / WN) + l31;
  auto frags = [&](int buf, int s, Frag (&av)[TM], Frag (&bv)[TN]) {
    const unsigned char* As = smem + buf * STAGE;
    const unsigned char* Bs = As + ABYTES;
    const int ch = (2 * s + hh) ^ kx;
#pragma unroll
    for (int i = 0; i < TM; ++i) {
      if constexpr (!MN)
        av[i] = *reinterpret_cast<const Frag*>(As + (arow0 + 32 * i) * 128 + (ch << 4));
      else if constexpr (!F32)
        av[i] = tr_frag(As, BM, swzA, wm * (BM / WM) + 32 * i, s);
      else
        av[i] = mn_frag32(As, BM, wm * (BM / WM) + 32 * i, s);
    }
#pragma unroll
    for (int j = 0; j < TN; ++j) {
      if constexpr (!MN)
        bv[j] = *reinterpret_cast<const Frag*>(Bs + (brow0 + 32 * j) * 128 + (ch << 4));
      else if constexpr (!F32)
        bv[j] = tr_frag(Bs, BN, swzB, wn * (BN / WN) + 32 * j, s);
      else
        bv[j] = mn_frag32(Bs, BN, wn * (BN / WN) + 32 * j, s);
    }
  };
  auto mfmas = [&](const Frag (&av)[TM], const Frag (&bv)[TN]) {
    if (PIPE) __builtin_amdgcn_s_setprio(1);
    if constexpr (F32) {
#pragma unroll
      for (int t = 0; t < 4; ++t)
#pragma unroll
        for (int i = 0; i < TM; ++i)
#pragma unroll
          for (int j = 0; j < TN; ++j)
            acc[i][j] = __builtin_amdgcn_mfma_f32_32x32x2f32(av[i][t], bv[j][t], acc[i][j], 0, 0, 0);
    } else {
#pragma unroll
      for (int i = 0; i < TM; ++i)
#pragma unroll
        for (int j = 0; j < TN; ++j)
          acc[i][j] = __builtin_amdgcn_mfma_f32_32x32x16_bf16(av[i], bv[j], acc[i][j], 0, 0, 0);
    }
    if (PIPE) __builtin_amdgcn_s_setprio(0);
  };
  constexpr int KSTEPS = BK / (2 * EPC);
  static_assert(KSTEPS == 4, "four k-steps per k-tile (the PIPE 1 schedule)");
  auto compute = [&](int buf) {
#pragma unroll
    for (int s = 0; s < KSTEPS; ++s) {
      Frag av[TM], bv[TN];
      frags(buf, s, av, bv);
      mfmas(av, bv);
    }
  };

  if (ntiles > 0 && PIPE == 0) {
    stage(0, 0);
    for (int kt = 0; kt < ntiles; ++kt) {
      asm volatile("s_waitcnt vmcnt(0)" ::: "memory");
      __syncthreads();
      if (kt + 1 < ntiles) stage(kt + 1, (kt + 1) & 1);
      compute(kt & 1);
    }
  } else if (NST == 1 && ntiles > 0) {
    for (int kt = 0; kt < ntiles; ++kt) {
      if (kt > 0) __syncthreads();
      stage(kt, 0);
      asm volatile("s_waitcnt vmcnt(0)" ::: "memory");
      __syncthreads();
      compute(0);
    }
  } else if (ntiles > 0) {
    stage(0, 0);
    for (int kt = 0; kt < ntiles; ++kt) {
      asm volatile("s_waitcnt vmcnt(0)" ::: "memory");
      __syncthreads();
      const int buf = kt & 1;
      Frag a0[TM], b0[TN], a1[TM], b1[TN];
      frags(buf, 0, a0, b0);
      if (kt + 1 < ntiles) stage(kt + 1, buf ^ 1);
      frags(buf, 1, a1, b1);
      mfmas(a0, b0);
      frags(buf, 2, a0, b0);
      mfmas(a1, b1);
      frags(buf, 3, a1, b1);
      mfmas(a0, b0);
      mfmas(a1, b1);
    }
  }
  __syncthreads();

  if constexpr (LDSEPI) {
    if (a.bn_part != nullptr) {
      if constexpr (PRE) {
        Epi::run(a, acc, reinterpret_cast<float*>(smem), m0, n0, pf);
      } else if constexpr (LATE) {
        Epi::prefetch(a, m0, n0, pf);
        Epi::run(a, acc, reinterpret_cast<float*>(smem), m0, n0, pf);
      } else
        epilogue_lds_bnbwd<BM, BN, WM, WN, TM, TN>(a, acc, reinterpret_cast<float*>(smem), SMEM / 4,
                                                    m0, n0);
      return;
    }
  }
  epilogue_batched<MODE, BM, BN, WM, WN, TM, TN, INF16>(a, acc, reinterpret_cast<float*>(smem), m0,
                                                        n0, split);
}

template <int MODE, int BM, int BN, int WM, int WN, int TAPV, int PIPE = 1, int F32 = 0, int NST = 2,
          int EPF = 0>
__global__ __launch_bounds__(64 * WM * WN, (occ16<BM, BN, WM, WN, NST>()))
void gemm16_kernel(const GemmArgs a) {
  int bid, split;
  xcd_work(bid, split);
  gemm16_body<MODE, BM, BN, WM, WN, TAPV, PIPE, F32, NST, EPF>(a, bid, split);
}

__device__ __forceinline__ void par_tile(const GemmPar& p, int w, int& cls, int& t) {
  const int ch = w / PAR_G, off = w - ch * PAR_G;
  int base = 0, prev = 0;
  cls = 0;
  t = 1 << 30;
  for (int n = p.n; n > 0; --n) {
    const int tn = (p.c[n - 1].tiles + PAR_G - 1) / PAR_G;
    const int span = n * (tn - prev);
    if (ch < base + span) {
      const int q = ch - base;
      cls = q % n;
      t = (prev + q / n) * PAR_G + off;
      return;
    }
    base += span;
    prev = tn;
  }
}

template <int BM, int BN, int WM, int WN, int F32, int EPF = 0>
__global__ __launch_bounds__(64 * WM * WN, (occ16<BM, BN, WM, WN, 2>()))
void gemm16_par_kernel(const GemmPar p) {
  int w, split;
  xcd_work(w, split);
  int cls, t;
  par_tile(p, w, cls, t);
  cls = __builtin_amdgcn_readfirstlane(cls);
  t = __builtin_amdgcn_readfirstlane(t);
  if (t >= p.c[cls].tiles) return;
  GemmArgs a = p.a;
  const ParClass& c = p.c[cls];
  auto own = [](auto v) {
    asm volatile("" : "+s"(v));
    return v;
  };
  a.M = own(c.M);
  a.K = own(c.K);
  a.ntaps = own(c.ntaps);
  a.tapS = own(c.tapS);
  a.tapSinv = own(c.tapSinv);
  a.oy0 = own(c.oy0);
  a.ox0 = own(c.ox0);
  a.wr0 = own(c.wr0);
  a.ws0 = own(c.ws0);
  a.oyc = own(c.oyc);
  a.oxc = own(c.oxc);
  a.dHW = FastDiv{own(c.dHW.d), own(c.dHW.m), own(c.dHW.s)};
  a.dW = FastDiv{own(c.dW.d), own(c.dW.m), own(c.dW.s)};
  a.bn_part = own(c.bn_part);
  gemm16_body<MODE_DGRAD, BM, BN, WM, WN, 0, 1, F32, 2, EPF>(a, t, 0);
}

}
#include "gemm16_ws.h"
namespace tmrg {

template <int MODE, int BM, int BN, int WM, int WN, int F32>
int launch16_cfg(const GemmArgs& a, bool tapv, dim3 grid, hipStream_t st) {
  const dim3 blk(64 * WM * WN);
  if constexpr (MODE == MODE_FWD && F32 == 0) {
    if (a.c16 && a.scale) return launch16_inf16<BM, BN, WM, WN>(a, tapv, grid, st);
  }
  constexpr int kmax = 64;
  if constexpr (MODE == MODE_FWD && F32 == 0 && WM * WN == 4 &&
                ((BM == 128 && BN == 128) || (BM == 256 && BN == 64))) {
    if (!tapv && a.K > 0 && a.K <= kmax) {
      hipLaunchKernelGGL((gemm16_kernel<MODE, BM, BN, WM, WN, 0, 1, F32, 1>), grid, blk, 0, st, a);
      TMR_CHECK_LAUNCH("gemm16_kernel (one stage)");
      return 0;
    }
  }
  if constexpr (MODE == MODE_FWD && F32 == 0 && BM == 256 && BN == 256) {
    if (!tapv && a.K > 0 && a.K <= kmax) {
      const dim3 g2((unsigned)(cdiv(a.M, 256) * cdiv(a.N, 128)), grid.y, 1);
      hipLaunchKernelGGL((gemm16_kernel<MODE, 256, 128, 4, 2, 0, 1, F32, 1>), g2, dim3(512), 0, st, a);
      TMR_CHECK_LAUNCH("gemm16_kernel (one stage, 256x128)");
      return 0;
    }
  }
  constexpr bool FORMS = MODE == MODE_DGRAD && TMR_EPI_FORMS &&
                         (WM * WN == 4 || (WM * WN == 8 && TMR_EPI_LATE_F > 0));
  if constexpr (FORMS) {
    const int f = a.bn_part != nullptr ? epi_form(a) : 0;
    if (f == (F32 ? 2 : 1)) {
      if (tapv)
        hipLaunchKernelGGL((gemm16_kernel<MODE, BM, BN, WM, WN, 1, 1, F32, 2, F32 ? 2 : 1>), grid, blk, 0, st, a);
      else
        hipLaunchKernelGGL((gemm16_kernel<MODE, BM, BN, WM, WN, 0, 1, F32, 2, F32 ? 2 : 1>), grid, blk, 0, st, a);
      TMR_CHECK_LAUNCH("gemm16_kernel (dgrad epilogue form)");
      return 0;
    }
  }
  if (tapv) {
    hipLaunchKernelGGL((gemm16_kernel<MODE, BM, BN, WM, WN, 1, 1, F32>), grid, blk, 0, st, a);
  } else {
    hipLaunchKernelGGL((gemm16_kernel<MODE, BM, BN, WM, WN, 0, 1, F32>), grid, blk, 0, st, a);
  }
  TMR_CHECK_LAUNCH(F32 ? "gemm16_kernel (fp32)" : "gemm16_kernel");
  return 0;
}

template <int MODE, int F32>
int launch16_switch(const GemmArgs& a, int cfg, bool tapv, dim3 grid, hipStream_t st) {
  switch (cfg) {
    case 1: return launch16_cfg<MODE, 256, 128, 4, 2, F32>(a, tapv, grid, st);
    case 2: return launch16_cfg<MODE, 128, 128, 2, 2, F32>(a, tapv, grid, st);
    case 3: return launch16_cfg<MODE, 256, 64, 4, 1, F32>(a, tapv, grid, st);
    case 4: return launch16_cfg<MODE, 64, 256, 1, 4, F32>(a, tapv, grid, st);
    case 7: return launch16_cfg<MODE, 128, 128, 4, 2, F32>(a, tapv, grid, st);
    case 5: return launch16_cfg<MODE, 64, 64, 2, 2, F32>(a, tapv, grid, st);
    case 0: return launch16_cfg<MODE, 256, 256, 2, 4, F32>(a, tapv, grid, st);
    case 6: return launch16_cfg<MODE, 256, 256, 4, 4, F32>(a, tapv, grid, st);
    default: break;
  }
  TMR_CHECK_ARG(false, "gemm16: no tile config %d", cfg);
  return 1;
}

template <int MODE, int F32>
int check16(const GemmArgs& a, int cfg) {
  TMR_CHECK_ARG(((uintptr_t)a.A & 15) == 0 && ((uintptr_t)a.B & 15) == 0,
                "gemm (LDS-DMA path): operands must be 16-B aligned");
  constexpr bool f32 = F32 != 0;
  TMR_CHECK_ARG((a.prec == TMR_MATH_F32) == f32, "gemm (LDS-DMA path): precision dispatch");
  TMR_CHECK_ARG(!f32 || (a.lds % 4 == 0 && a.log2C >= 2 &&
                         (MODE == MODE_DGRAD ? (a.ldbt % 4 == 0 && a.N % 8 == 0 && a.ldc % 4 == 0 &&
                                                ((uintptr_t)a.C & 15) == 0)
                                             : a.ldb % 4 == 0)),
                "gemm (fp32 LDS-DMA path): 4-channel pieces, 16-B row strides (view %d)", MODE);
  const Cfg16 c = kCfgs16[cfg];
  TMR_CHECK_ARG(a.bn_part == nullptr || a.bn_mask != 3 ||
                    (MODE == MODE_DGRAD && !(c.bm == 256 && c.bn == 256)),
                "gemm: ReLU-mask bits (mask 3) need the LDS-DMA dgrad's LDS-staged epilogue (tile %dx%d)",
                c.bm, c.bn);
  TMR_CHECK_ARG(!a.g16 || (MODE == MODE_DGRAD && a.bn_part != nullptr &&
                           !(c.bm == 256 && c.bn == 256) && ((uintptr_t)a.C & 15) == 0 &&
                           a.ldc % 8 == 0),
                "gemm: a bf16 BN-backward gradient (TMR_IO_G16) needs the fused LDS-staged dgrad "
                "epilogue, 16-B aligned rows (tile %dx%d)", c.bm, c.bn);
  TMR_CHECK_ARG((!a.Cold && !a.cold16) ||
                    (MODE == MODE_DGRAD && a.bn_part != nullptr && !(c.bm == 256 && c.bn == 256) &&
                     ((uintptr_t)(a.Cold ? a.Cold : a.C) & 15) == 0),
                "gemm: a separate / bf16 old dx needs the fused LDS-staged dgrad epilogue (tile %dx%d)",
                c.bm, c.bn);
  return 0;
}

template <int MODE, int F32>
int launch_gemm16_t(const GemmArgs& a, int splits, hipStream_t st) {
  constexpr bool f32 = F32 != 0;
  const int cfg = pick_cfg16(a.M, a.N, a.K, MODE, f32);
// ... 92 lines not shown
```

### tmrnet_amd/csrc/gemm16_select.h

```cpp
#pragma once
#include "gemm_kernel.h"

namespace tmrg {

struct Cfg16 { int bm, bn; };
constexpr Cfg16 kCfgs16[] = {{256, 256}, {256, 128}, {128, 128}, {256, 64}, {64, 256}, {64, 64},
                              {256, 256},
                              {128, 128}};

inline bool use32(const GemmArgs& a, int mode) {
  if (a.prec != TMR_MATH_F32 || a.sab) return false;
  if (mode == MODE_DGRAD) return a.wt != 0;
  if (!a.dma32) return false;
  if ((((uintptr_t)a.A | (uintptr_t)a.B) & 15) != 0) return false;
  if (mode == MODE_WGRAD)
    return a.M % 4 == 0 && a.log2C >= 2 && a.ldb % 4 == 0 && a.lds % 4 == 0 && a.N % 4 == 0;
  return a.lds % 4 == 0 && a.ldb % 4 == 0 && a.log2C >= 2 && (a.ntaps != 1 || a.K % 4 == 0);
}

inline bool use16(const GemmArgs& a, int mode) {
  if (a.prec == TMR_MATH_F32) return use32(a, mode);
  if (a.prec != TMR_MATH_BF16 || a.sab != 3) return false;
  if (mode == MODE_DGRAD && !a.wt) return false;
  if (a.lds % 8) return false;
  if (mode == MODE_WGRAD) return a.M % 8 == 0 && a.log2C >= 3 && a.ldb % 8 == 0 && a.N % 8 == 0;
  if (mode == MODE_FWD && a.ldb % 8) return false;
  if (mode == MODE_DGRAD && a.ldbt % 8) return false;
  return a.ntaps == 1 ? (a.K % 8 == 0 && (mode == MODE_FWD || a.log2C >= 3)) : a.log2C >= 3;
}

inline long cfg16_tiles(long M, long N, int c) {
  return ((M + kCfgs16[c].bm - 1) / kCfgs16[c].bm) * ((N + kCfgs16[c].bn - 1) / kCfgs16[c].bn);
}

inline int pick_cfg16(long M, long N, long K, int mode, bool f32 = false) {
  static const int forced = env_int("TMR_GEMM16_CFG", -1);
  if (forced >= 0 && forced < (int)(sizeof(kCfgs16) / sizeof(kCfgs16[0]))) return forced;
  int cfg;
  if (f32 && mode == MODE_WGRAD) {
    if (M <= 64) return (N <= 64 || N >= 512) ? 5 : 4;
    if (N <= 64) return 5;
    if (M >= 256 && N >= 256 && 2.0 * M * N * K >= 100e9) return 6;
    return 7;
  }
  if (f32 && M >= 256 && mode == MODE_DGRAD && N >= 512) {
    static const int wide = env_int("TMR_DGRAD32_WIDE_CFG", 7);
    return cfg16_tiles(M, N, wide) >= 256 ? wide : 2;
  }
  if (f32 && M >= 256 && mode == MODE_FWD && N == 128)
    return cfg16_tiles(M, N, 7) >= 256 ? 7 : 2;
  if (mode == MODE_WGRAD) {
    if (M <= 64) cfg = N <= 64 ? 5 : (N >= 512 ? 4 : 2);
    else if (N <= 64) cfg = 3;
    else cfg = (M >= 256 && N >= 1024 && K * cfg16_tiles(M, N, 6) >= (1L << 21)) ? 6 : 7;
  } else if (N <= 64) {
    cfg = M >= 256 ? 3 : 5;
  } else if (mode == MODE_FWD && N >= 256 && M >= 256) {
    cfg = 6;
  } else {
    cfg = 2;
  }
  if (mode != MODE_WGRAD && cfg16_tiles(M, N, cfg) < (f32 && cfg == 6 ? 224 : 256)) {
    for (const int c2 : {1, 2, 5}) {
      if ((long)kCfgs16[c2].bm * kCfgs16[c2].bn >= (long)kCfgs16[cfg].bm * kCfgs16[cfg].bn ||
          cfg16_tiles(M, N, c2) <= cfg16_tiles(M, N, cfg))
        continue;
      cfg = c2;
      if (cfg16_tiles(M, N, cfg) >= 256) break;
    }
  }
  return cfg;
}

inline int gemm_tile_bm(const GemmArgs& a, int mode) {
  return use16(a, mode) ? kCfgs16[pick_cfg16(a.M, a.N, a.K, mode, a.prec == TMR_MATH_F32)].bm
                        : kCfgs[pick_cfg(a.M, a.N, a.K, mode)].bm;
}
inline long gemm_tiles(const GemmArgs& a, int mode) {
  return use16(a, mode) ? cfg16_tiles(a.M, a.N, pick_cfg16(a.M, a.N, a.K, mode, a.prec == TMR_MATH_F32))
                        : cfg_tiles(a.M, a.N, pick_cfg(a.M, a.N, a.K, mode));
}

constexpr int PAR_MAX = 4;
struct ParClass {
  int M, K, ntaps, tapS, tapSinv, oy0, ox0, wr0, ws0, oyc, oxc, tiles;
  FastDiv dHW, dW;
  float2* bn_part;
};
struct GemmPar {
  GemmArgs a;
  ParClass c[PAR_MAX];
  int n;
};
constexpr int PAR_G = 64;

extern long g_dgrad_ws_launches;

template <int F32>
int launch_gemm16_par(const GemmArgs* as, int n, hipStream_t st);
extern template int launch_gemm16_par<0>(const GemmArgs*, int, hipStream_t);
extern template int launch_gemm16_par<1>(const GemmArgs*, int, hipStream_t);
template <int MODE, int F32>
int launch_gemm16(const GemmArgs& a, int splits, hipStream_t st);
extern template int launch_gemm16<MODE_FWD, 0>(const GemmArgs&, int, hipStream_t);
extern template int launch_gemm16<MODE_FWD, 1>(const GemmArgs&, int, hipStream_t);
extern template int launch_gemm16<MODE_DGRAD, 0>(const GemmArgs&, int, hipStream_t);
extern template int launch_gemm16<MODE_DGRAD, 1>(const GemmArgs&, int, hipStream_t);
extern template int launch_gemm16<MODE_WGRAD, 0>(const GemmArgs&, int, hipStream_t);
extern template int launch_gemm16<MODE_WGRAD, 1>(const GemmArgs&, int, hipStream_t);

template <int BM, int BN, int WM, int WN>
int launch16_inf16(const GemmArgs& a, bool tapv, dim3 grid, hipStream_t st);
extern template int launch16_inf16<256, 128, 4, 2>(const GemmArgs&, bool, dim3, hipStream_t);
extern template int launch16_inf16<128, 128, 2, 2>(const GemmArgs&, bool, dim3, hipStream_t);
extern template int launch16_inf16<256, 64, 4, 1>(const GemmArgs&, bool, dim3, hipStream_t);
extern template int launch16_inf16<64, 256, 1, 4>(const GemmArgs&, bool, dim3, hipStream_t);
extern template int launch16_inf16<128, 128, 4, 2>(const GemmArgs&, bool, dim3, hipStream_t);
extern template int launch16_inf16<64, 64, 2, 2>(const GemmArgs&, bool, dim3, hipStream_t);
extern template int launch16_inf16<256, 256, 2, 4>(const GemmArgs&, bool, dim3, hipStream_t);
extern template int launch16_inf16<256, 256, 4, 4>(const GemmArgs&, bool, dim3, hipStream_t);

}
```

### tmrnet_amd/csrc/gemm16_wgrad_f32.hip

```cpp
#include "gemm16_kernel.h"

namespace tmrg {
template int launch_gemm16<MODE_WGRAD, 1>(const GemmArgs& a, int splits, hipStream_t st);
}
```

### tmrnet_amd/csrc/gemm_conv.hip

```cpp
#include "direct_conv.h"
#include "gemm16_select.h"

#include <type_traits>

using namespace tmrg;

namespace {

__device__ __forceinline__ float split_sum(const float* __restrict__ slabs, int nsplit, long slab,
                                           long src) {
  float s = 0.f;
  int p = 0;
  for (; p + 8 <= nsplit; p += 8) {
    float v[8];
#pragma unroll
    for (int u = 0; u < 8; ++u) v[u] = slabs[(p + u) * slab + src];
#pragma unroll
    for (int u = 0; u < 8; ++u) s += v[u];
  }
  for (; p < nsplit; ++p) s += slabs[p * slab + src];
  return s;
}

__global__ void wgrad_reduce_kernel(const float* __restrict__ slabs, int nsplit, long slab,
// ... 397 lines not shown

long tmrg::g_dgrad_ws_launches = 0;
TMR_API long tmr_dgrad_ws_launches(void) { return __atomic_load_n(&g_dgrad_ws_launches, __ATOMIC_RELAXED); }

TMR_API int tmr_conv2d_dgrad_bnbwd_parts(const tmr_conv_desc* d) {
  if (!d || d->n <= 0) {
    tmr_set_error("tmr_conv2d_dgrad_bnbwd_parts: null or empty descriptor");
    return -1;
  }
  if (const auto* f = direct_view(d, &DirectConv::dgrad)) return f->parts(d);
  BnBwdFuse fz{};
  fz.count_only = true;
  long np = 0;
  if (dgrad_bnbwd_run(d, nullptr, nullptr, nullptr, 1.f, fz, &np, nullptr)) return -1;
  return (int)np;
}

static int dgrad_bnbwd_entry(const tmr_conv_desc* d, const float* dy, const float* w_krsc,
                             float* dx, float beta, const void* dx_old, int old_bf16,
                             const float* y, const float* z, const float* scale,
                             const float* shift, const float* mean, int mask, void* parts,
                             size_t parts_bytes, hipStream_t stream) {
  TMR_CHECK_ARG(xld_of(d) == d->c, "tmr_conv2d_dgrad_bnbwd: dx must be dense (x_ld == c)");
  TMR_CHECK_ARG(ngroups(d) == 1 || mask != 3,
                "tmr_conv2d_dgrad_bnbwd: a grouped dgrad takes no ReLU-mask bits");
  TMR_CHECK_ARG(y && mean && parts, "tmr_conv2d_dgrad_bnbwd: null y / mean / parts");
  TMR_CHECK_ARG(!(d->io & TMR_IO_G16) ||
                    (d->math == TMR_MATH_BF16 && (d->io & TMR_IO_WT_BF16) &&
                     (d->c / ngroups(d)) % 8 == 0),
                "tmr_conv2d_dgrad_bnbwd: a bf16 gradient (TMR_IO_G16) needs bf16 math on the LDS-DMA "
                "engine (TMR_IO_WT_BF16), channels per group a multiple of 8");
  TMR_CHECK_ARG(!dx_old || ngroups(d) == 1, "tmr_conv2d_dgrad_bnbwd: a separate old dx takes no groups");
  TMR_CHECK_ARG(ngroups(d) == 1 || beta == 0.f || !(d->io & TMR_IO_G16),
                "tmr_conv2d_dgrad_bnbwd: a grouped dgrad accumulates (beta != 0) into fp32 dx only");
  TMR_CHECK_ARG(mask == 0 || (mask == 1 && z) || (mask == 2 && scale && shift) || (mask == 3 && z),
                "tmr_conv2d_dgrad_bnbwd: mask %d needs z (1, 3: bits) or scale/shift (2)", mask);
  TMR_CHECK_ARG(mask != 3 || ((d->io & (TMR_IO_WT_F32 | TMR_IO_WT_BF16)) &&
                              ((long)d->h * d->w * d->c) % 32 == 0),
                "tmr_conv2d_dgrad_bnbwd: ReLU-mask bits (mask 3) need the LDS-DMA dgrad "
                "(TMR_IO_WT_F32 / TMR_IO_WT_BF16) and h*w*c a multiple of 32");
  const int np = tmr_conv2d_dgrad_bnbwd_parts(d);
  TMR_CHECK_ARG(np >= 0 && parts_bytes >= (size_t)np * d->c * sizeof(float2),
                "tmr_conv2d_dgrad_bnbwd: parts buffer too small");
  if (const auto* f = direct_view(d, &DirectConv::dgrad)) {
    TMR_CHECK_ARG(!dx_old && !((d->io & TMR_IO_G16) && beta != 0.f),
                  "tmr_conv2d_dgrad_bnbwd: the direct 3x3 dgrad takes no old dx / "
                  "accumulating bf16 gradient");
    return f->run(d, dy, w_krsc, dx, beta, y, z, scale, shift, mean, mask, parts, stream);
  }
  BnBwdFuse fz{};
  fz.y = y; fz.z = z; fz.sc = scale; fz.sh = shift; fz.mean = mean; fz.mask = mask;
  fz.part = (float2*)parts;
  fz.part_ld = d->c;
  fz.old = dx_old;
  fz.old16 = beta != 0.f ? old_bf16 : 0;
  return dgrad_bnbwd_run(d, dy, w_krsc, dx, beta, fz, nullptr, stream);
}

TMR_API int tmr_conv2d_dgrad_bnbwd(const tmr_conv_desc* d, const float* dy, const float* w_krsc,
                                   float* dx, float beta, const float* y, const float* z,
                                   const float* scale, const float* shift, const float* mean,
                                   int mask, void* parts, size_t parts_bytes, hipStream_t stream) {
  TMR_CHECK_ARG(d, "tmr_conv2d_dgrad_bnbwd: null descriptor");
  return dgrad_bnbwd_entry(d, dy, w_krsc, dx, beta, nullptr, (d->io & TMR_IO_G16) ? 1 : 0, y, z,
                           scale, shift, mean, mask, parts, parts_bytes, stream);
}

TMR_API int tmr_conv2d_dgrad_bnbwd_acc(const tmr_conv_desc* d, const float* dy,
                                       const float* w_krsc, void* dx, float beta,
                                       const void* dx_old, int old_bf16, const float* y,
                                       const float* z, const float* scale, const float* shift,
                                       const float* mean, int mask, void* parts,
                                       size_t parts_bytes, hipStream_t stream) {
  TMR_CHECK_ARG(d, "tmr_conv2d_dgrad_bnbwd_acc: null descriptor");
  TMR_CHECK_ARG(beta != 0.f && dx_old && ((uintptr_t)dx_old & 15) == 0 &&
                    (d->io & TMR_IO_G16) && (d->io & TMR_IO_WT_BF16),
                "tmr_conv2d_dgrad_bnbwd_acc: needs beta != 0, a 16-B aligned old dx and a bf16 "
                "output (TMR_IO_G16) on the bf16 LDS-DMA engine (TMR_IO_WT_BF16)");
  return dgrad_bnbwd_entry(d, dy, w_krsc, (float*)dx, beta, dx_old, old_bf16 ? 1 : 0, y, z, scale,
                           shift, mean, mask, parts, parts_bytes, stream);
}

TMR_API int tmr_conv2d_dgrad(const tmr_conv_desc* d, const float* dy, const float* w_krsc,
                             float* dx, float beta, hipStream_t stream) {
  TMR_CHECK_ARG(d, "tmr_conv2d_dgrad: null descriptor");
  return for_slices(d, [&](const tmr_conv_desc& c, int g, int f0) {
    return conv_dgrad_impl(&c, adv(dy, y_off(c, g, f0), esz_dy(d)), adv(w_krsc, w_off(c, g), esz_w(d)),
                           dx + x_off(c, g, f0), beta, stream);
  });
}

static void wgrad_fill(const tmr_conv_desc* d, GemmArgs& a) {
  a = GemmArgs{};
  a.M = d->k; a.N = d->r * d->s * d->c; a.K = d->n * d->ho * d->wo;
  a.log2C = ilog2_exact(d->c);
  set_taps(a, d->r, d->s);
  a.oy0 = -d->pad; a.ox0 = -d->pad_w; a.dyr = 1; a.dxs = 1;
  set_grid(a, d->n, d->ho, d->wo);
  a.Hs = d->h; a.Ws = d->w; a.sy = d->stride; a.sx = d->stride;
  a.lds = xld_of(d); a.ldb = yld_of(d); a.ldc = a.N; a.beta = 0.f;
  a.Abytes = clamp_bytes_e(span((long)d->n * d->ho * d->wo, a.ldb, d->k), esz_dy(d));
  a.prec = d->math;
  a.Bbytes = clamp_bytes_e(span((long)d->n * d->h * d->w, a.lds, d->c), esz_x(d));
  a.sab = ((d->io & TMR_IO_DY_BF16) ? 1 : 0) | ((d->io & TMR_IO_X_BF16) ? 2 : 0);
  a.dma32 = d->math == TMR_MATH_F32;
}

static int wgrad_plan(const tmr_conv_desc* d, int* splits, int* kchunk, long* slab) {
  const long Mred = (long)d->n * d->ho * d->wo;
  const long Mo = d->k, No = (long)d->r * d->s * d->c;
  GemmArgs a;
  wgrad_fill(d, a);
  const long tiles = gemm_tiles(a, MODE_WGRAD);
  static const long target = env_int("TMR_WGRAD_TARGET", 512);
  static const long minrows = env_int("TMR_WGRAD_MINROWS", 1024);
  long sp = target / (tiles > 0 ? tiles : 1);
  if (sp < 1) sp = 1;
  long maxsp = Mred / minrows;
  if (maxsp < 1) maxsp = 1;
  if (sp > maxsp) sp = maxsp;
  long kc = (Mred + sp - 1) / sp;
  kc = (kc + 63) / 64 * 64;
  sp = (Mred + kc - 1) / kc;
  *splits = (int)sp;
  *kchunk = (int)kc;
  *slab = Mo * No;
  return 0;
}

static const DirectConv::Wgrad* direct_wgrad(const tmr_conv_desc* d, int c_real) {
  const DirectConv::Wgrad* f = direct_view(d, &DirectConv::wgrad);
  return f && (c_real == 0 || f->c_real == 0 || f->c_real == c_real) ? f : nullptr;
}

TMR_API size_t tmr_conv2d_wgrad_ws_bytes(const tmr_conv_desc* d) {
  if (!d || d->n <= 0 || d->k <= 0 || d->c <= 0 || d->r <= 0 || d->s <= 0) {
    tmr_set_error("tmr_conv2d_wgrad_ws_bytes: null or empty descriptor");
    return 0;
  }
  size_t bytes = 0;
  const auto plan = [&](const tmr_conv_desc& c, int, int) {
    int sp, kc;
    long slab;
    wgrad_plan(&c, &sp, &kc, &slab);
    if ((size_t)sp * slab * sizeof(float) > bytes) bytes = (size_t)sp * slab * sizeof(float);
    return 0;
  };
  if (for_slices(d, plan, true)) return 0;
  if (const auto* f = direct_wgrad(d, 0))
    if (bytes < f->ws_bytes(d)) bytes = f->ws_bytes(d);
  return bytes;
}

static int conv_wgrad_impl(const tmr_conv_desc* d, const float* x, const float* dy,
                           float* dw_oihw, int c_real, float beta, float* ws, size_t ws_bytes,
                           hipStream_t stream) {
  TMR_CHECK_ARG(d->math == TMR_MATH_F32 || d->math == TMR_MATH_BF16, "tmr_conv2d: bad math mode %d", d->math);
  const int lc = ilog2_exact(d->c);
  TMR_CHECK_ARG(lc >= 2, "tmr_conv2d_wgrad: stored input channels %d must be a power of two >= 4", d->c);
  TMR_CHECK_ARG(c_real >= 1 && c_real <= d->c, "tmr_conv2d_wgrad: bad c_real %d", c_real);
  if (const auto* f = direct_wgrad(d, c_real)) {
    DirectSlabs sl{};
    const int rc = f->run(d, x, dy, ws, ws_bytes, &sl, stream);
    if (rc) return rc;
    hipLaunchKernelGGL(wgrad_reduce_taps_kernel, dim3(d->k, cdiv(c_real, 64)), dim3(256), 0, stream,
                       ws, sl.n, sl.elems, dw_oihw, sl.taps, sl.cstored, c_real, beta);
    TMR_CHECK_LAUNCH("wgrad_reduce_taps_kernel");
    return 0;
  }
  int sp, kc;
  long slab;
  wgrad_plan(d, &sp, &kc, &slab);
  TMR_CHECK_ARG(ws && ws_bytes >= (size_t)sp * slab * sizeof(float),
                "tmr_conv2d_wgrad: workspace too small (%zu < %zu)", ws_bytes,
                (size_t)sp * slab * sizeof(float));
  GemmArgs a;
  wgrad_fill(d, a);
  a.A = dy; a.B = x; a.C = ws; a.bias = nullptr;
  a.kchunk = kc; a.slab = slab;
  a.Cbytes = clamp_bytes(slab);
  bool al = aligned16(x) && aligned16(dy) && (d->k % 4 == 0) && a.lds % 4 == 0 && a.ldb % 4 == 0;
  const int rc = launch_gemm<MODE_WGRAD>(a, al, sp, stream);
  if (rc) return rc;
  const int ntaps = d->r * d->s;
  if (ntaps > 1 && ntaps <= kReduceTaps) {
    hipLaunchKernelGGL(wgrad_reduce_taps_kernel, dim3(d->k, cdiv(c_real, 64)), dim3(256), 0,
                       stream, ws, sp, slab, dw_oihw, ntaps, d->c, c_real, beta);
    TMR_CHECK_LAUNCH("wgrad_reduce_taps_kernel");
    return 0;
  }
  long total = (long)d->k * ntaps * c_real;
  int blocks = (int)((total + 255) / 256);
  if (blocks > 4096) blocks = 4096;
  hipLaunchKernelGGL(wgrad_reduce_kernel, dim3(blocks), dim3(256), 0, stream, ws, sp, slab,
                     dw_oihw, d->k, ntaps, d->c, c_real, beta);
  TMR_CHECK_LAUNCH("wgrad_reduce_kernel");
  return 0;
}

TMR_API int tmr_conv2d_wgrad(const tmr_conv_desc* d, const float* x, const float* dy,
                             float* dw_oihw, int c_real, float beta, float* ws, size_t ws_bytes,
                             hipStream_t stream) {
  TMR_CHECK_ARG(d, "tmr_conv2d_wgrad: null descriptor");
  return for_slices(d, [&](const tmr_conv_desc& c, int g, int f0) {
    return conv_wgrad_impl(&c, adv(x, x_off(c, g, f0), esz_x(d)), adv(dy, y_off(c, g, f0), esz_dy(d)),
                           dw_oihw + (long)g * c.k * c_real * c.r * c.s, c_real,
                           f0 == 0 ? beta : 1.f, ws, ws_bytes, stream);
  });
}

TMR_API int tmr_gemm_nt(int M, int N, int K, const float* A, int lda, const float* B, int ldb,
                        const float* bias, float* C, int ldc, float beta, hipStream_t stream) {
  TMR_CHECK_ARG(M >= 0 && N >= 0 && K >= 0, "tmr_gemm_nt: negative size");
  GemmArgs a{};
  a.A = A; a.B = B; a.C = C; a.bias = bias;
  a.M = M; a.N = N; a.K = K; a.log2C = 0;
  set_taps(a, 1, 1);
  a.dyr = 1; a.dxs = 1;
  set_grid(a, M, 1, 1);
  a.Hs = 1; a.Ws = 1; a.sy = 1; a.sx = 1;
  a.lds = lda; a.ldb = ldb; a.ldc = ldc; a.beta = beta;
  a.Abytes = clamp_bytes(M > 0 ? (long)(M - 1) * lda + K : 0);
  a.Bbytes = clamp_bytes(N > 0 ? (long)(N - 1) * ldb + K : 0);
  a.Cbytes = clamp_bytes(M > 0 ? (long)(M - 1) * ldc + N : 0);
  bool al = aligned16(A) && aligned16(B) && lda % 4 == 0 && ldb % 4 == 0 && K % 4 == 0;
  return launch_gemm<MODE_FWD>(a, al, 1, stream);
}

TMR_API int tmr_gemm_nn(int M, int N, int K, const float* A, int lda, const float* B, int ldb,
                        float* C, int ldc, float beta, hipStream_t stream) {
  TMR_CHECK_ARG(M >= 0 && N >= 0 && K >= 0, "tmr_gemm_nn: negative size");
  GemmArgs a{};
  a.A = A; a.B = B; a.C = C; a.bias = nullptr;
  a.M = M; a.N = N; a.K = K; a.log2C = 0;
  set_taps(a, 1, 1);
  a.oy0 = 0; a.ox0 = 0; a.dyr = -1; a.dxs = -1;
  a.wr0 = 0; a.ws0 = 0; a.wst = 1; a.wS = 1;
  set_grid(a, M, 1, 1);
  a.Hs = 1; a.Ws = 1; a.sy = 1; a.sx = 1;
  a.lds = lda; a.ldb = ldb; a.ldc = ldc; a.beta = beta;
  a.oH = 1; a.oW = 1; a.osy = 1; a.osx = 1; a.oyc = 0; a.oxc = 0;
  a.Abytes = clamp_bytes(M > 0 ? (long)(M - 1) * lda + K : 0);
  a.Bbytes = clamp_bytes(K > 0 ? (long)(K - 1) * ldb + N : 0);
  a.Cbytes = clamp_bytes(M > 0 ? (long)(M - 1) * ldc + N : 0);
  bool al = aligned16(A) && aligned16(B) && lda % 4 == 0 && ldb % 4 == 0 && K % 4 == 0 &&
            N % 4 == 0;
  return launch_gemm<MODE_DGRAD>(a, al, 1, stream);
}

TMR_API int tmr_gemm_tn(int M, int N, int K, const float* A, int lda, const float* B, int ldb,
                        float* C, int ldc, float beta, hipStream_t stream) {
  TMR_CHECK_ARG(M >= 0 && N >= 0 && K >= 0, "tmr_gemm_tn: negative size");
  GemmArgs a{};
  a.A = A; a.B = B; a.C = C; a.bias = nullptr;
  a.M = M; a.N = N; a.K = K; a.log2C = 0;
  set_taps(a, 1, 1);
  a.dyr = 1; a.dxs = 1;
  set_grid(a, K, 1, 1);
  a.Hs = 1; a.Ws = 1; a.sy = 1; a.sx = 1;
  a.lds = ldb; a.ldb = lda; a.ldc = ldc; a.beta = beta;
  a.kchunk = K > 0 ? K : 1; a.slab = 0;
  a.Abytes = clamp_bytes(K > 0 ? (long)(K - 1) * lda + M : 0);
  a.Bbytes = clamp_bytes(K > 0 ? (long)(K - 1) * ldb + N : 0);
  a.Cbytes = clamp_bytes(M > 0 ? (long)(M - 1) * ldc + N : 0);
  bool al = aligned16(A) && aligned16(B) && lda % 4 == 0 && ldb % 4 == 0 && M % 4 == 0 &&
            N % 4 == 0;
  return launch_gemm<MODE_WGRAD>(a, al, 1, stream);
}
```

### tmrnet_amd/ops.py

```python
import contextlib
import threading
import weakref

import numpy as np
import torch

from ._lib import call, query, stream_ptr, ConvDesc
from . import health
import ctypes

f32 = torch.float32

PROF = None


class _prof:
    def __init__(self, kind, flops, shape=None, nbytes=0):
        self.kind, self.flops, self.shape, self.nbytes = kind, flops, shape, nbytes

    def __enter__(self):
        if PROF is not None:
            self.e0 = torch.cuda.Event(enable_timing=True)
            self.e1 = torch.cuda.Event(enable_timing=True)
            self.e0.record()
# ... 229 lines not shown
    n, ho, wo, k = dy.shape
    k2, r, s, c = _dgrad_w(w_krsc, wt, groups)
    h, w = in_hw
    d = conv_desc(n, h, w, c, k, r, s, stride, pad, pad_w, math=math, io=_io(None, w_krsc, dy, wt),
                  groups=groups)
    assert (d.ho, d.wo) == (ho, wo), ((d.ho, d.wo), (ho, wo))
    if out is None:
        out = _empty((n, h, w, c), dy)
    d.x_ld = _nhwc_ld(out, "dx")
    d.y_ld = _nhwc_ld(dy, "dy")
    with _prof("conv_dgrad" + _SUFFIX[math], 2.0 * n * ho * wo * k * r * s * c / groups, (n, h, w, c, k, r, stride),
               _esz(dy) * n * ho * wo * k + _esz(w_krsc) * w_krsc.numel()
               + 4 * n * h * w * c * (2 if beta else 1)):
        call("tmr_conv2d_dgrad", ctypes.byref(d), dy, w_krsc, out, float(beta), stream_ptr())
    return out


def conv_dgrad_bnbwd(dy, w_krsc, in_hw, stride, pad, y, mean, mask, z=None, scale=None,
                     shift=None, out=None, beta=0.0, math="fp32", wt=False, groups=1,
                     g16=False, old=None):
    if old is not None:
        if not (g16 and beta != 0.0 and out is None and groups == 1):
            raise RuntimeError("conv_dgrad_bnbwd: a separate old dx needs g16, beta, no out / "
                               "groups")
        if old.dtype not in (f32, BF16) or not old.is_contiguous():
            raise RuntimeError("conv_dgrad_bnbwd: old dx must be a contiguous fp32 / bf16 tensor")
    if g16 and groups > 1 and beta != 0.0:
        raise RuntimeError("conv_dgrad_bnbwd: a grouped dgrad accumulates (beta != 0) into an fp32 "
                           "dx only")
    _req_op(w_krsc, "w"); _req_op(y, "y"); _req(mean, "mean")
    if mask == 3:
        if z is None or z.dtype != torch.int32 or z.numel() * 32 < y.numel():
            raise RuntimeError("conv_dgrad_bnbwd: mask 3 takes the int32 ReLU-mask bits of y's shape")
    elif z is not None and z.dtype != y.dtype:
        raise RuntimeError("conv_dgrad_bnbwd: y and z must have one dtype")
    n, ho, wo, k = dy.shape
    k2, r, s, c = _dgrad_w(w_krsc, wt, groups)
    h, w = in_hw
    d = conv_desc(n, h, w, c, k, r, s, stride, pad, math=math,
                  io=_io(None, w_krsc, dy, wt) | (IO_BN if y.dtype == BF16 else 0)
                  | (IO_G16 if g16 else 0), groups=groups)
    assert (d.ho, d.wo) == (ho, wo), ((d.ho, d.wo), (ho, wo))
    if out is None:
        out = _empty((n, h, w, c), dy, dtype=BF16 if g16 else f32)
    elif out.dtype != (BF16 if g16 else f32):
        raise RuntimeError("conv_dgrad_bnbwd: dx must be %s" % ("bf16 (g16)" if g16 else "fp32"))
    if tuple(y.shape) != tuple(out.shape) or (z is not None and mask != 3
                                              and tuple(z.shape) != tuple(out.shape)):
        raise RuntimeError("conv_dgrad_bnbwd: y/z must have dx's shape %s" % (tuple(out.shape),))
    if old is not None and tuple(old.shape) != tuple(out.shape):
        raise RuntimeError("conv_dgrad_bnbwd: old dx must have dx's shape %s" % (tuple(out.shape),))
    d.x_ld = _nhwc_ld(out, "dx")
    d.y_ld = _nhwc_ld(dy, "dy")
    nparts = query("tmr_conv2d_dgrad_bnbwd_parts", ctypes.byref(d))
    if nparts < 0:
        raise RuntimeError("tmr_conv2d_dgrad_bnbwd_parts failed")
    parts = torch.empty((max(nparts, 1), c, 2), dtype=f32, device=dy.device)
    with _prof("conv_dgrad" + _SUFFIX[math], 2.0 * n * ho * wo * k * r * s * c / groups, (n, h, w, c, k, r, stride),
               _esz(dy) * n * ho * wo * k + _esz(w_krsc) * w_krsc.numel()
               + (2 if g16 else 4) * n * h * w * c
               + ((old.element_size() if old is not None else (2 if g16 else 4)) * n * h * w * c
                  if beta else 0)
               + y.element_size() * n * h * w * c * (2 if z is not None and mask != 3 else 1)
               + (n * h * w * c // 8 if mask == 3 else 0)):
        if old is not None:
            call("tmr_conv2d_dgrad_bnbwd_acc", ctypes.byref(d), dy, w_krsc, out, float(beta), old,
                 int(old.dtype == BF16), y, z, scale, shift, mean, int(mask), parts,
                 ctypes.c_size_t(parts.numel() * 4), stream_ptr())
        else:
            call("tmr_conv2d_dgrad_bnbwd", ctypes.byref(d), dy, w_krsc, out, float(beta), y, z,
                 scale, shift, mean, int(mask), parts, ctypes.c_size_t(parts.numel() * 4),
                 stream_ptr())
    return out, parts, nparts


def bn_bwd_maxpool(dyp, am, y, scale, shift, mean, inv, gamma, bf16=False):
    n, h, w, c = y.shape
    _, ho, wo, _ = dyp.shape
    ws, nb = _bn_ws(n * h * w, c, y.device)
    if y.dtype == BF16:
        dy = torch.empty_like(y)
        dgamma = _empty((c,), dyp); dbeta = _empty((c,), dyp)
        call("tmr_bn_bwd_maxpool_a16", dyp, am, n, h, w, ho, wo, y, scale, shift, mean, inv, gamma,
             dy, dgamma, dbeta, c, ws, ctypes.c_size_t(nb), stream_ptr())
        return dy, dgamma, dbeta
    dy = torch.empty_like(y, dtype=torch.bfloat16 if bf16 else y.dtype)
    dgamma = _empty((c,), y); dbeta = _empty((c,), y)
    call("tmr_bn_bwd_maxpool_x", dyp, am, n, h, w, ho, wo, y, scale, shift, mean, inv, gamma, dy,
         dgamma, dbeta, c, ws, ctypes.c_size_t(nb), int(bf16), stream_ptr())
    return dy, dgamma, dbeta


def bn_bwd_parts_ds(g, y, parts, nparts, mean, inv, gamma, yd, mean_d, inv_d, gamma_d):
    c = y.shape[-1]
    rows = y.numel() // c
    t = y.dtype
    if not (g.dtype == t and yd.dtype == t and t in (f32, BF16) and g.shape == y.shape == yd.shape
            and g.is_contiguous() and y.is_contiguous() and yd.is_contiguous()):
        raise RuntimeError("bn_bwd_parts_ds: g, y and y_ds must be contiguous tensors of one shape "
                           "and one dtype (fp32 or bf16)")
    nb = query("tmr_bn_bwd_parts_ds_ws_bytes", int(nparts), rows, c)
    ws = torch.empty(((nb + 7) // 8,), dtype=torch.float64, device=y.device)
    dy, dyd = torch.empty_like(y), torch.empty_like(yd)
    dg, db = _empty((c,), mean), _empty((c,), mean)
    dgd, dbd = _empty((c,), mean), _empty((c,), mean)
    call("tmr_bn_bwd_parts_ds", g, y, parts, int(nparts), mean, inv, gamma, dy, dg, db, yd, mean_d,
         inv_d, gamma_d, dyd, dgd, dbd, rows, c, int(t == BF16), ws, ctypes.c_size_t(ws.numel() * 8),
         stream_ptr())
    return dy, dg, db, dyd, dgd, dbd


def bn_bwd_parts(g, y, parts, nparts, mean, inv, gamma, bf16=False):
    c = y.shape[-1]
    rows = y.numel() // c
    nb = query("tmr_bn_parts_ws_bytes", int(nparts), c)
    ws = torch.empty(((nb + 7) // 8,), dtype=torch.float64, device=y.device)
    if y.dtype == BF16:
        dy = torch.empty_like(y)
        dgamma = _empty((c,), mean); dbeta = _empty((c,), mean)
        call("tmr_bn_bwd_parts_g16" if g.dtype == BF16 else "tmr_bn_bwd_parts_a16", g, y, parts,
             int(nparts), mean, inv, gamma, dy, dgamma, dbeta, rows, c, ws,
             ctypes.c_size_t(ws.numel() * 8), stream_ptr())
        return dy, dgamma, dbeta
    dy = torch.empty_like(y, dtype=torch.bfloat16 if bf16 else y.dtype)
    dgamma = _empty((c,), y); dbeta = _empty((c,), y)
    call("tmr_bn_bwd_parts_x", g, y, parts, int(nparts), mean, inv, gamma, dy, dgamma, dbeta, rows,
         c, ws, ctypes.c_size_t(ws.numel() * 8), int(bf16), stream_ptr())
    return dy, dgamma, dbeta


def conv_wgrad(x, dy, r, s, stride, pad, c_real=None, out=None, beta=0.0, pad_w=None,
               math="fp32", groups=1):
    n, h, w, c = x.shape
    k = dy.shape[3]
    c_real = c // groups if c_real is None else c_real
    d = conv_desc(n, h, w, c, k, r, s, stride, pad, pad_w, math=math, io=_io(x, None, dy),
                  groups=groups)
    d.x_ld = _nhwc_ld(x, "x")
    d.y_ld = _nhwc_ld(dy, "dy")
    assert (d.ho, d.wo) == tuple(dy.shape[1:3])
    if out is None:
        out = _empty((k, c_real, r, s), x)
    ws_bytes = query("tmr_conv2d_wgrad_ws_bytes", ctypes.byref(d))
    ws = torch.empty(max(1, (ws_bytes + 3) // 4), dtype=f32, device=x.device)
    with _prof("conv_wgrad" + _SUFFIX[math], 2.0 * n * d.ho * d.wo * k * r * s * c_real,
               (n, h, w, c, k, r, stride),
               _esz(x) * n * h * w * c + _esz(dy) * n * d.ho * d.wo * k
               + 4 * k * r * s * c_real):
        call("tmr_conv2d_wgrad", ctypes.byref(d), x, dy, out, int(c_real), float(beta), ws,
             ctypes.c_size_t(ws.numel() * 4), stream_ptr())
    return out


def gemm_nt(a, b, bias=None, out=None, beta=0.0, M=None, N=None, K=None, lda=None, ldb=None,
            ldc=None):
    M = a.shape[0] if M is None else M
    K = a.shape[1] if K is None else K
    N = b.shape[0] if N is None else N
    lda = a.stride(0) if lda is None else lda
    ldb = b.stride(0) if ldb is None else ldb
    if out is None:
        out = _empty((M, N), a)
    ldc = out.stride(0) if ldc is None else ldc
    call("tmr_gemm_nt", M, N, K, a, lda, b, ldb, bias, out, ldc, float(beta), stream_ptr())
    return out


def gemm_nn(a, b, out=None, beta=0.0, M=None, N=None, K=None, lda=None, ldb=None, ldc=None):
    M = a.shape[0] if M is None else M
    K = a.shape[1] if K is None else K
    N = b.shape[1] if N is None else N
    lda = a.stride(0) if lda is None else lda
    ldb = b.stride(0) if ldb is None else ldb
    if out is None:
        out = _empty((M, N), a)
    ldc = out.stride(0) if ldc is None else ldc
    call("tmr_gemm_nn", M, N, K, a, lda, b, ldb, out, ldc, float(beta), stream_ptr())
    return out


def gemm_tn(a, b, out=None, beta=0.0, M=None, N=None, K=None, lda=None, ldb=None, ldc=None):
    K = a.shape[0] if K is None else K
    M = a.shape[1] if M is None else M
    N = b.shape[1] if N is None else N
    lda = a.stride(0) if lda is None else lda
    ldb = b.stride(0) if ldb is None else ldb
    if out is None:
        out = _empty((M, N), a)
    ldc = out.stride(0) if ldc is None else ldc
    call("tmr_gemm_tn", M, N, K, a, lda, b, ldb, out, ldc, float(beta), stream_ptr())
    return out


def col_sum(x, rows, cols, ld, out=None, beta=0.0):
    if out is None:
        out = _empty((cols,), x)
    call("tmr_col_sum", x, rows, cols, ld, out, float(beta), stream_ptr())
    return out


class _LayoutRecord:
    def __init__(self, owner):
        self.lookup = {}
        self.rows = []
        self.table = None
        self.blocks = 0
        self.valid = True
        self.sources = [(weakref.ref(p), p.data_ptr()) for p in owner.parameters()]

    def live(self):
        for ref, ptr in self.sources:
            p = ref()
            if p is None or p.data_ptr() != ptr:
                return False
        return True


_LAYOUTS = weakref.WeakKeyDictionary()
_TLS = threading.local()


_WL_DTYPE = np.dtype([("w", "<u8"), ("out", "<u8"), ("n", "<i8"), ("block0", "<i8"),
                      ("k", "<i4"), ("c", "<i4"), ("rs", "<i4"), ("cpad", "<i4"),
                      ("kind", "<i4"), ("bf16", "<i4")])


def _session():
    st = getattr(_TLS, "session", None)
    if st is None:
        st = _TLS.session = [None, False]
    return st


LAYOUT_SESSIONS = True


def clear_layout_sessions(owner=None):
    if owner is None:
        _LAYOUTS.clear()
    else:
        _LAYOUTS.pop(owner, None)


def layout_session_count():
    return sum(len(v) for v in _LAYOUTS.values())


@contextlib.contextmanager
def layout_session(owner, key):
    if not LAYOUT_SESSIONS:
        yield
        return
    recs = _LAYOUTS.get(owner)
    if recs is None:
        recs = _LAYOUTS[owner] = {}
    key = (key, threading.get_ident())
    rec = recs.get(key)
    recording = rec is None or not rec.valid or rec.table is None or not rec.live()
    if recording:
        rec = recs[key] = _LayoutRecord(owner)
    else:
        call("tmr_weight_layouts_multi", rec.table, len(rec.rows), rec.blocks, stream_ptr())
    st = _session()
    prev = list(st)
    st[0], st[1] = rec, recording
    try:
        yield
    finally:
        st[0], st[1] = prev
        if recording and rec.rows and rec.valid:
            epb = int(query("tmr_weight_layouts_epb"))
            tab = np.zeros(len(rec.rows), dtype=_WL_DTYPE)
            b0 = 0
            for j, (wp, out, k, c, rs, cpad, kind, b16) in enumerate(rec.rows):
                n = out.numel()
                tab[j] = (wp, out.data_ptr(), n, b0, k, c, rs, cpad, kind, b16)
                b0 += (n + epb - 1) // epb
            rec.table = torch.from_numpy(tab.view(np.uint8).copy()).to(rec.rows[0][1].device)
            rec.blocks = b0


def _layout(key, convert, rows):
    rec, recording = _session()
    if rec is None:
        return convert()
    out = rec.lookup.get(key)
    if out is not None and not recording:
        return out
    out = convert()
    if recording:
        rec.lookup[key] = out
        rec.rows.extend(rows(out))
    else:
        rec.valid = False
    return out


def weight_to_krsc(w, cpad=None, bf16=False):
    k, c, r, s = w.shape
    cpad = c if cpad is None else cpad
    _req(w, "w")

    def convert():
        out = _empty((k, r, s, cpad), w, dtype=torch.bfloat16 if bf16 else f32)
        call("tmr_weight_oihw_to_krsc_x", w, out, k, c, r, s, cpad, int(bf16), stream_ptr())
        return out
# ... 644 lines not shown
```

### tmrnet_amd/trunk.py

```python
import os
import weakref

import torch
import torch.nn as nn

from . import ops


class Bottleneck(nn.Module):
    expansion = 4

    def __init__(self, inplanes, planes, stride=1, downsample=None):
        super().__init__()
        self.conv1 = nn.Conv2d(inplanes, planes, 1, bias=False)
        self.bn1 = nn.BatchNorm2d(planes)
        self.conv2 = nn.Conv2d(planes, planes, 3, stride=stride, padding=1, bias=False)
        self.bn2 = nn.BatchNorm2d(planes)
        self.conv3 = nn.Conv2d(planes, planes * 4, 1, bias=False)
        self.bn3 = nn.BatchNorm2d(planes * 4)
        self.relu = nn.ReLU(inplace=True)
        self.downsample = downsample
        self.stride = stride


def _make_layer(inplanes, planes, blocks, stride):
    downsample = None
    if stride != 1 or inplanes != planes * 4:
        downsample = nn.Sequential(nn.Conv2d(inplanes, planes * 4, 1, stride=stride, bias=False),
                                   nn.BatchNorm2d(planes * 4))
    layers = [Bottleneck(inplanes, planes, stride, downsample)]
    for _ in range(1, blocks):
        layers.append(Bottleneck(planes * 4, planes))
    return nn.Sequential(*layers)


_GRAD_READY = weakref.WeakKeyDictionary()


def set_grad_ready(share, fn):
    if fn is None:
        _GRAD_READY.pop(share, None)
    else:
        _GRAD_READY[share] = fn


def get_grad_ready(share):
    return _GRAD_READY.get(share, getattr(share, "grad_ready", None))

def _bn_momentum(bn):
    if bn.momentum is None:
        raise NotImplementedError("BatchNorm2d(momentum=None) (cumulative average) is not supported")
    return bn.momentum


BF16_STORE = os.environ.get("TMR_BF16_STORE", "1") != "0"


def _store16(math):
    return math == "bf16" and BF16_STORE


FULL16 = True

ACT16 = os.environ.get("TMR_BF16_ACT", "1") != "0"


G16 = os.environ.get("TMR_G16", "1") != "0"

R16 = os.environ.get("TMR_BF16_RESGRAD", "1") != "0"

DS_DUAL = True


def _ds_dual(g, r3, rd):
    y = r3["y"]
    return (DS_DUAL and g.is_contiguous() and g.dtype == y.dtype == rd["y"].dtype
            and y.shape == rd["y"].shape and y.shape[-1] % 8 == 0
            and not (_store16(r3["math"]) and y.dtype == torch.float32))



def _dma32(math):
    return math == "fp32"




def _full16(math):
    return _store16(math) and FULL16


def _act16(math):
    return _full16(math) and ACT16


def _infer16(share):
    return bool(not share.training and _full16(share.precision)
                and getattr(share, "infer_act16", False))


def _conv_bn(x, conv, bn, stride, pad, relu, training, residual=None, recs=None, math="fp32",
             defer=False, branch=None, nbt=None, dual=False, groups=1, y16=False):
    w = conv.weight
    k, c, r, s = w.shape
    cs = x.shape[3]
    s16 = _store16(math)
    if r == 1 and s == 1 and c == cs and not s16:
        wk = w.detach().contiguous().view(k, 1, 1, c)
    else:
        wk = ops.weight_to_krsc(w.detach().contiguous(), cpad=cs // groups, bf16=s16)
    if groups > 1 and not training:
        raise RuntimeError("grouped convs run in the train-mode trunk only")
    if training:
        y, stats, nparts = ops.conv_fwd_bnstats(x, wk, stride, pad, c_real=c * groups, math=math,
                                                y16=_act16(math), groups=groups)
        mean, inv, scale, shift = ops.bn_finalize(
            stats, nparts, bn.weight.detach(), bn.bias.detach(), bn.running_mean,
            bn.running_var, _bn_momentum(bn), bn.eps)
        if nbt is None:
            bn.num_batches_tracked.add_(1)
        else:
            nbt.append(bn.num_batches_tracked)
    else:
        scale, shift = ops.bn_eval_params(bn.weight.detach(), bn.bias.detach(), bn.running_mean,
                                          bn.running_var, bn.eps)
        return ops.conv_fwd_fused(x, wk, stride, pad, scale, shift, residual, relu, c_real=c,
                                  math=math, y16=y16)
    zbits = None
    bits = (recs is not None and relu and not dual and _dma32(math) and y.dtype == torch.float32
            and (residual is not None or branch is not None))
    if defer:
        z = None
    elif branch is not None and bits:
        z, zbits = ops.bn_apply2_bits(y, scale, shift, branch[0], branch[1], branch[2])
    elif bits:
        z, zbits = ops.bn_apply_bits(y, scale, shift, residual)
    elif branch is not None:
        z = ops.bn_apply2(y, scale, shift, branch[0], branch[1], branch[2], relu, dual=dual)
    elif dual:
        z = ops.bn_apply_dual(y, scale, shift, residual, relu)
    else:
        z = ops.bn_apply(y, scale, shift, residual, relu, bf16=s16 and residual is None)
    if recs is not None:
        has_res = residual is not None or branch is not None
        if groups > 1 and ((_full16(math) and x.dtype == torch.bfloat16) or _dma32(math)):
            wt = ops.weight_to_crsk_grouped(w.detach().contiguous(), groups,
                                            bf16=x.dtype == torch.bfloat16)
        elif _full16(math) and x.dtype == torch.bfloat16:
            wt = ops.weight_to_crsk(w.detach().contiguous())
        elif _dma32(math) and c % 8 == 0 and x.dtype == torch.float32:
            wt = ops.weight_to_crsk(w.detach().contiguous(), bf16=False)
        else:
            wt = None
        recs.append({"x": x, "wk": wk, "wt": wt, "y": y,
                     "z": (z[0] if dual else z) if has_res else None, "zbits": zbits,
                     "scale": scale, "shift": shift, "mean": mean, "inv": inv,
                     "stride": stride, "pad": pad, "relu": relu, "conv": conv, "bn": bn,
                     "c_real": c, "math": math, "groups": groups})
    return (y, scale, shift) if defer else z


def _conv_bn_bwd(rec, dz, grads, want_dres=False, dx_out=None, dx_beta=0.0, need_dx=True,
                 dres_inplace=False, parts=None, fuse_prev=None, pool=None, dy=None, g16=False,
                 r16=False):
    conv, bn = rec["conv"], rec["bn"]
    s16 = _store16(rec["math"])
    dy_given = dy is not None
    if dy_given:
        dres = None
    elif pool is not None:
        dy, dg, db = ops.bn_bwd_maxpool(pool[0], pool[1], rec["y"], rec["scale"], rec["shift"],
                                        rec["mean"], rec["inv"], bn.weight.detach(), bf16=s16)
        dres = None
    elif parts is not None:
        dy, dg, db = ops.bn_bwd_parts(dz, rec["y"], parts[0], parts[1], rec["mean"], rec["inv"],
                                      bn.weight.detach(), bf16=s16)
        dres = dz if want_dres else None
    else:
        dy, dres, dg, db = ops.bn_bwd(dz, rec["y"], rec["z"], rec["mean"], rec["inv"],
                                      bn.weight.detach(), rec["relu"], want_dres=want_dres,
                                      dres_out=dz if dres_inplace else None,
                                      scale=rec["scale"], shift=rec["shift"], bf16=s16)
    if not dy_given:
        grads[bn.weight] = dg
        grads[bn.bias] = db
    x = rec["x"]
    k, c, r, s = conv.weight.shape
    grp = rec.get("groups", 1)
    grads[conv.weight] = ops.conv_wgrad(x, dy, r, s, rec["stride"], rec["pad"],
                                        c_real=rec["c_real"], math=rec["math"],
                                        groups=grp)
    dx, fused = None, None
    if need_dx:
        hw = (x.shape[1], x.shape[2])
        wt = rec.get("wt") is not None
        wdg = rec["wt"] if wt else rec["wk"]
        if fuse_prev is not None:
            p = fuse_prev
            mask = (1 if p["z"] is not None else 2) if p["relu"] else 0
            zm = p["z"]
            if mask == 1 and wt and p.get("zbits") is not None:
                mask, zm = 3, p["zbits"]
            bf8 = (wt and p["y"].dtype == torch.bfloat16 and
                   (p["y"].shape[-1] // grp) % 8 == 0)
            gb = (g16 and G16 and mask == 2 and dx_out is None and dx_beta == 0.0 and bf8)
            rb = (r16 and R16 and mask in (1, 3) and dx_out is not None and dx_beta == 1.0 and bf8
                  and grp == 1)
            old = None
            if rb and dx_out.dtype != torch.bfloat16:
                old, dx_out = dx_out, None
            dx, pp, npp = ops.conv_dgrad_bnbwd(dy, wdg, hw, rec["stride"], rec["pad"],
                                               p["y"], p["mean"], mask, z=zm,
                                               scale=p["scale"], shift=p["shift"], out=dx_out,
                                               beta=dx_beta, math=rec["math"],
                                               wt=wt, groups=grp, g16=gb or rb, old=old)
            fused = (pp, npp)
        else:
            dx = ops.conv_dgrad(dy, wdg, hw, rec["stride"], rec["pad"], out=dx_out,
                                beta=dx_beta, math=rec["math"], wt=wt, groups=grp)
    return dx, dres, fused


class TrunkFn(torch.autograd.Function):

    @staticmethod
    def forward(ctx, x4, share, keep, *params):
        with ops.layout_session(share, ("resnet50", share.training, bool(keep),
                                 share.precision, _infer16(share))):
            return TrunkFn._forward(ctx, x4, share, keep, params)

    @staticmethod
    def _forward(ctx, x4, share, keep, params):
        training = share.training
        keep = keep and training
        recs = [] if keep else None
        nbt = []
        conv1, bn1, layers = share.trunk_parts()
        mt = share.precision
        a16 = training and _act16(mt)
        f16 = training and _full16(mt) and not a16
        i16 = _infer16(share)
        if training:
            xs = ops.nhwc4_to_bf16x8(x4) if (a16 and ops.engine_forced()) else x4
            y0, sc0, sh0 = _conv_bn(xs, conv1, bn1, 2, 3, True, training, recs=recs, math=mt,
                                    defer=True, nbt=nbt)
            p, am = ops.maxpool_fwd_bn(y0, sc0, sh0, bf16=f16)
            stem_hw = (y0.shape[1], y0.shape[2])
        elif i16:
            z = _conv_bn(ops.nhwc4_to_bf16x8(x4), conv1, bn1, 2, 3, True, training, math=mt,
                         y16=True)
            p, am = ops.maxpool_fwd_bn(z, torch.ones_like(bn1.running_mean),
                                       torch.zeros_like(bn1.running_mean))
            stem_hw = (z.shape[1], z.shape[2])
        else:
            z = _conv_bn(x4, conv1, bn1, 2, 3, True, training, recs=recs, math=mt, nbt=nbt)
            p, am = ops.maxpool_fwd(z)
            stem_hw = (z.shape[1], z.shape[2])
        h, hx = (None, p) if f16 else (p, p)
        blocks = []
        for layer in layers:
            for blk in layer:
                brec = [] if keep else None
                z1 = _conv_bn(hx, blk.conv1, blk.bn1, 1, 0, True, training, recs=brec, math=mt,
                              nbt=nbt, y16=i16)
                z2 = _conv_bn(z1, blk.conv2, blk.bn2, blk.stride, 1, True, training, recs=brec,
                              math=mt, nbt=nbt, y16=i16)
                if blk.downsample is not None:
                    idn = _conv_bn(hx, blk.downsample[0], blk.downsample[1], blk.stride, 0, False,
                                   training, recs=brec, math=mt, defer=training, nbt=nbt,
                                   y16=i16)
                else:
                    if h is None:
                        raise RuntimeError("identity residual of the stem output (no downsample)")
                    idn = h
                if isinstance(idn, tuple):
                    h = _conv_bn(z2, blk.conv3, blk.bn3, 1, 0, True, training, branch=idn,
                                 recs=brec, math=mt, nbt=nbt, dual=f16)
                else:
                    h = _conv_bn(z2, blk.conv3, blk.bn3, 1, 0, True, training, residual=idn,
                                 recs=brec, math=mt, nbt=nbt, dual=f16, y16=i16)
                h, hx = h if f16 else (h, h)
                blocks.append((blk, brec))
        feat = ops.avgpool_fwd(h)
        ops.counters_add_one(nbt)
        ctx.keep = keep
        if keep:
            ctx.share = share
            ctx.params = params
            ctx.stem = recs
            ctx.pool = (am, stem_hw)
            ctx.blocks = blocks
            ctx.last_hw = (h.shape[1], h.shape[2])
        return feat

    @staticmethod
    def backward(ctx, dfeat):
        if not ctx.keep:
            raise RuntimeError("trunk backward needs train mode and a forward with grad enabled")
        grads = {}
        g = ops.avgpool_bwd(dfeat.contiguous(), ctx.last_hw)
        blocks = ctx.blocks
        pending = None
        ready = get_grad_ready(ctx.share)
        while blocks:
            blk, brec = blocks.pop()
            has_ds = blk.downsample is not None
            r1, r2 = brec[0], brec[1]
            rd = brec[2] if has_ds else None
            r3 = brec[-1]
            prev3 = blocks[-1][1][-1] if blocks else None
            dyd = None
            if (has_ds and _ds_dual(g, r3, rd) and pending is not None):
                dy3, dg3, db3, dyd, dgd, dbd = ops.bn_bwd_parts_ds(
                    g, r3["y"], pending[0], pending[1], r3["mean"], r3["inv"],
                    r3["bn"].weight.detach(), rd["y"], rd["mean"], rd["inv"],
                    rd["bn"].weight.detach())
                grads[r3["bn"].weight], grads[r3["bn"].bias] = dg3, db3
                grads[rd["bn"].weight], grads[rd["bn"].bias] = dgd, dbd
                dz2, _, fz2 = _conv_bn_bwd(r3, None, grads, fuse_prev=r2, g16=True, dy=dy3)
                dres = g
                del dy3
            else:
                dz2, dres, fz2 = _conv_bn_bwd(r3, g, grads, want_dres=True, dres_inplace=True,
                                              parts=pending, fuse_prev=r2, g16=True)
            dz1, _, fz1 = _conv_bn_bwd(r2, dz2, grads, parts=fz2, fuse_prev=r1, g16=True)
            del dz2
            if has_ds:
                if dyd is not None:
                    dx, _, _ = _conv_bn_bwd(rd, None, grads, dy=dyd)
                    del dyd
                else:
                    dx, _, _ = _conv_bn_bwd(rd, dres, grads)
                dx, _, pending = _conv_bn_bwd(r1, dz1, grads, parts=fz1, dx_out=dx, dx_beta=1.0,
                                              fuse_prev=prev3, r16=True)
            else:
                dx, _, pending = _conv_bn_bwd(r1, dz1, grads, parts=fz1, dx_out=dres, dx_beta=1.0,
                                              fuse_prev=prev3, r16=True)
            del dz1, brec, dres
            g = dx
            if ready is not None:
                ready([(p, grads[p]) for p in blk.parameters() if p in grads])
        dh = g
        am, stem_hw = ctx.pool
        _conv_bn_bwd(ctx.stem[0], None, grads, need_dx=False, pool=(dh, am))
        out = [grads.get(p) for p in ctx.params]
        ctx.blocks = ctx.stem = None
        return (None, None, None) + tuple(out)


_CHILD_NAMES = ("conv1", "bn1", "relu", "maxpool", "layer1", "layer2", "layer3", "layer4",
                "avgpool")


class ResNet50Share(nn.Sequential):

    def __init__(self, indexed=False, precision="fp32"):
        super().__init__()
        self.precision = precision
        self.infer_act16 = False
        mods = (nn.Conv2d(3, 64, 7, stride=2, padding=3, bias=False), nn.BatchNorm2d(64),
                nn.ReLU(inplace=True), nn.MaxPool2d(3, stride=2, padding=1),
                _make_layer(64, 64, 3, 1), _make_layer(256, 128, 4, 2),
                _make_layer(512, 256, 6, 2), _make_layer(1024, 512, 3, 2),
                nn.AdaptiveAvgPool2d((1, 1)))
        for i, (name, m) in enumerate(zip(_CHILD_NAMES, mods)):
            self.add_module(str(i) if indexed else name, m)
        for m in self.modules():
            if isinstance(m, nn.Conv2d):
                nn.init.kaiming_normal_(m.weight, mode="fan_out", nonlinearity="relu")
            elif isinstance(m, nn.BatchNorm2d):
                nn.init.constant_(m.weight, 1)
                nn.init.constant_(m.bias, 0)

    def trunk_parts(self):
        ch = list(self.children())
        return ch[0], ch[1], ch[4:8]

    def features_nhwc4(self, x4):
        params = list(self.parameters())
        keep = torch.is_grad_enabled() and any(p.requires_grad for p in params)
        return TrunkFn.apply(x4, self, keep, *params)

    def forward(self, x):
        x = x.reshape(-1, 3, x.shape[-2], x.shape[-1]).contiguous()
        x4 = ops.nchw_to_nhwc(x, cpad=4)
        feat = self.features_nhwc4(x4)
        return feat.view(feat.shape[0], feat.shape[1], 1, 1)


def resnet50_share():
    return ResNet50Share()
```

Measured before the change: 3789 frames/s.

## Fuse BN-backward apply into fp32 wgrad GEMM's A-operand staging

Adds a wgrad GEMM variant that computes dY = a*g + b*y + c from BN-backward coefficients while staging g into LDS. The first N-tile block writes dY back to global memory, so the separate BN-backward apply pass over g and y is skipped for bottleneck convs where the tile config allows it. BN parts finalization now only produces coefficients, and dgrad later reads the stored dY. The cost is an extra y load inside the wgrad mainloop and a store on one column of blocks, which could slow the GEMM. The fused path only applies to fp32, ungrouped convs with aligned, dense tensors.

```diff
diff --git a/include/tmr.h b/include/tmr.h
--- a/include/tmr.h
+++ b/include/tmr.h
@@ -63,6 +63,12 @@
 size_t tmr_conv2d_wgrad_ws_bytes(const tmr_conv_desc* d);
 int tmr_conv2d_wgrad(const tmr_conv_desc* d, const float* x, const float* dy, float* dw_oihw,
                      int c_real, float beta, float* ws, size_t ws_bytes, hipStream_t stream);
+int tmr_conv2d_wgrad_bnbwd_ok(const tmr_conv_desc* d, const void* x, const void* g, const void* y,
+                              const void* dy_out);
+int tmr_conv2d_wgrad_bnbwd(const tmr_conv_desc* d, const float* x, const float* g, const float* y,
+                           const float* coef, float* dy_out, float* dw_oihw, int c_real,
+                           float beta, float* ws, size_t ws_bytes, hipStream_t stream);
+long tmr_wgrad_bnbwd_launches(void);
 int tmr_conv2d_dgrad_bnbwd_acc(const tmr_conv_desc* d, const float* dy, const float* w_krsc,
                                void* dx, float beta, const void* dx_old, int old_bf16,
                                const float* y, const float* z, const float* scale,
@@ -141,6 +147,7 @@
                        const float* save_mean, const float* save_invstd, const float* gamma,
                        void* dy, float* dgamma, float* dbeta, int rows, int c, void* ws,
                        size_t ws_bytes, int out_bf16, hipStream_t stream);
+size_t tmr_bn_parts_coef_offset(int nparts, int c);
 int tmr_bn_bwd_x(const float* dz, const float* y, const float* z, const float* scale,
                  const float* shift, const float* save_mean, const float* save_invstd,
                  const float* gamma, void* dy, float* dres, float* dgamma, float* dbeta, int rows,
diff --git a/tmrnet_amd/_lib.py b/tmrnet_amd/_lib.py
--- a/tmrnet_amd/_lib.py
+++ b/tmrnet_amd/_lib.py
@@ -52,6 +52,10 @@
     "tmr_conv2d_dgrad_bnbwd": [DP, P, P, P, F, P, P, P, P, P, I, P, SZ, P],
     "tmr_conv2d_wgrad_ws_bytes": [DP],
     "tmr_conv2d_wgrad": [DP, P, P, P, I, F, P, SZ, P],
+    "tmr_conv2d_wgrad_bnbwd_ok": [DP, P, P, P, P],
+    "tmr_conv2d_wgrad_bnbwd": [DP, P, P, P, P, P, P, I, F, P, SZ, P],
+    "tmr_wgrad_bnbwd_launches": [],
+    "tmr_bn_parts_coef_offset": [I, I],
     "tmr_conv2d_dgrad_bnbwd_acc": [DP, P, P, P, F, P, I, P, P, P, P, P, I, P, SZ, P],
     "tmr_bn_apply_x": [P, P, P, P, P, I, I, I, I, P],
     "tmr_bn_bwd_parts_x": [P, P, P, I, P, P, P, P, P, P, I, I, P, SZ, I, P],
@@ -186,6 +190,8 @@
     "tmr_clear_error": None,
     "tmr_conv2d_wgrad_ws_bytes": SZ,
     "tmr_dgrad_ws_launches": L,
+    "tmr_wgrad_bnbwd_launches": L,
+    "tmr_bn_parts_coef_offset": SZ,
     "tmr_resize_tmp_bytes": SZ,
     "tmr_margin_ws_bytes": SZ,
     "tmr_jpeg_ws_bytes": SZ,
diff --git a/tmrnet_amd/csrc/bn.hip b/tmrnet_amd/csrc/bn.hip
--- a/tmrnet_amd/csrc/bn.hip
+++ b/tmrnet_amd/csrc/bn.hip
@@ -1090,6 +1090,14 @@
     return 0;
   }
   return slab_ws_bytes(nparts, c) + (size_t)3 * c * sizeof(float) + 64;
+}
+
+TMR_API size_t tmr_bn_parts_coef_offset(int nparts, int c) {
+  if (nparts <= 0 || c <= 0) {
+    tmr_set_error("tmr_bn_parts_coef_offset: bad size (parts %d, channels %d)", nparts, c);
+    return 0;
+  }
+  return slab_ws_bytes(nparts, c);
 }
 
 TMR_API int tmr_bn_finalize_ws(const void* partials, int nparts, int c, const float* gamma,
@@ -1451,6 +1459,7 @@
                      (const double*)slabs, sp.nslabs, rows, c, save_mean, save_invstd, gamma,
                      dgamma, dbeta, coef);
   TMR_CHECK_LAUNCH("bn_bwd_final_slabs");
+  if (!dyv) return 0;
   const long n4 = (long)rows * c / 4;
   if (out_bf16)
     hipLaunchKernelGGL((bn_bwd_apply<0, false, __bf16, float>), dim3(ew_blocks(n4)), dim3(NT), 0, stream, g,
diff --git a/tmrnet_amd/csrc/gemm16_kernel.h b/tmrnet_amd/csrc/gemm16_kernel.h
--- a/tmrnet_amd/csrc/gemm16_kernel.h
+++ b/tmrnet_amd/csrc/gemm16_kernel.h
@@ -446,7 +446,7 @@
 }
 
 template <int MODE, int BM, int BN, int WM, int WN, int TAPV, int PIPE, int F32, int NST, int EPF = 0,
-          int INF16 = 0>
+          int INF16 = 0, int BNW = 0>
 __device__ __forceinline__ void gemm16_body(const GemmArgs& a, const int bid, const int split) {
   constexpr uint32_t ES = F32 ? 4u : 2u;
   constexpr int EPC = 16 / ES;
@@ -464,6 +464,8 @@
   using Frag = typename std::conditional<F32 != 0, f32x4_t, bf16x8>::type;
   constexpr int EPI = WM * BN * 2 * 4;
   static_assert(NST == 2 || (NST == 1 && MODE != MODE_WGRAD), "one-stage form: FWD / DGRAD");
+  static_assert(!BNW || (MN && F32 != 0 && PIPE == 1), "dY-producing form: the fp32 WGRAD view");
+  static_assert(!BNW || ((64 * NW) % (2 * (BM / 4)) == 0), "dY-producing form: fixed piece columns");
   constexpr int LDSROWB = (BN + 4) * (BM / WM) * 4, LDSFULL = (BN + 4) * BM * 4;
   constexpr int LDSNEED = MODE != MODE_DGRAD ? 0 : (LDSFULL <= 70 * 1024 ? LDSFULL : LDSROWB);
   constexpr int SMEM1 = STAGE > EPI ? (STAGE > LDSNEED ? STAGE : LDSNEED) : (EPI > LDSNEED ? EPI : LDSNEED);
@@ -526,6 +528,21 @@
       akr[q] = k;
       acok[q] = i < a.M;
       aco[q] = (uint32_t)i * ES;
+    }
+  }
+  __amdgpu_buffer_rsrc_t rY = rA, rD = rA;
+  f32x4_t cfA = {0.f, 0.f, 0.f, 0.f}, cfB = cfA, cfC = cfA;
+  f32x4_t ypc[BNW ? NIA : 1];
+  bool dyw = false;
+  if constexpr (BNW != 0) {
+    rY = make_rsrc(a.bn_y, a.Abytes);
+    rD = make_rsrc(reinterpret_cast<const float*>(a.Cold), a.Abytes);
+    dyw = n0 == 0;
+    if (acok[0]) {
+      const int i = (int)(aco[0] / ES);
+      cfA = *reinterpret_cast<const f32x4_t*>(a.bn_sc + i);
+      cfB = *reinterpret_cast<const f32x4_t*>(a.bn_sc + a.M + i);
+      cfC = *reinterpret_cast<const f32x4_t*>(a.bn_sc + 2 * a.M + i);
     }
   }
   uint32_t brow[MN ? 1 : NIB];
@@ -634,6 +651,8 @@
         const bool ok = acok[q] && m < kend;
         const uint32_t off = (uint32_t)m * (uint32_t)a.ldb * ES + aco[q];
         glds16(rA, As + 1024 * (wave + NW * q), ok ? off : OOB);
+        if constexpr (BNW != 0)
+          ypc[q] = __builtin_bit_cast(f32x4_t, __builtin_amdgcn_raw_buffer_load_b128(rY, ok ? off : OOB, 0, 0));
       }
 #pragma unroll
       for (int q = 0; q < NIB; ++q) {
@@ -753,6 +772,34 @@
     }
   };
 
+  f32x4_t dyo[BNW ? NIA : 1];
+  auto bnw_apply = [&](int kt, int buf) {
+    const int kb = kbeg + kt * BK;
+    unsigned char* As = smem + buf * STAGE;
+#pragma unroll
+    for (int q = 0; q < NIA; ++q) {
+      f32x4_t* pc = reinterpret_cast<f32x4_t*>(As + 1024 * (wave + NW * q) + 16 * lane);
+      const int m = kb + akr[q];
+      const bool ok = acok[q] && m < kend;
+      const f32x4_t gv = *pc, yv = ypc[q];
+      f32x4_t o;
+#pragma unroll
+      for (int e = 0; e < 4; ++e) o[e] = ok ? fmaf(cfA[e], gv[e], fmaf(cfB[e], yv[e], cfC[e])) : 0.f;
+      *pc = o;
+      dyo[q] = o;
+    }
+  };
+  auto bnw_store = [&](int kt) {
+    const int kb = kbeg + kt * BK;
+#pragma unroll
+    for (int q = 0; q < NIA; ++q) {
+      const int m = kb + akr[q];
+      const bool ok = acok[q] && m < kend;
+      const uint32_t off = (uint32_t)m * (uint32_t)a.ldb * ES + aco[q];
+      __builtin_amdgcn_raw_buffer_store_b128(__builtin_bit_cast(u32x4_t, dyo[q]), rD, ok ? off : OOB, 0, 0);
+    }
+  };
+
   if (ntiles > 0 && PIPE == 0) {
     stage(0, 0);
     for (int kt = 0; kt < ntiles; ++kt) {
@@ -773,10 +820,14 @@
     stage(0, 0);
     for (int kt = 0; kt < ntiles; ++kt) {
       asm volatile("s_waitcnt vmcnt(0)" ::: "memory");
+      if constexpr (BNW != 0) bnw_apply(kt, kt & 1);
       __syncthreads();
       const int buf = kt & 1;
       Frag a0[TM], b0[TN], a1[TM], b1[TN];
       frags(buf, 0, a0, b0);
+      if constexpr (BNW != 0) {
+        if (dyw) bnw_store(kt);
+      }
       if (kt + 1 < ntiles) stage(kt + 1, buf ^ 1);
       frags(buf, 1, a1, b1);
       mfmas(a0, b0);
@@ -813,6 +864,14 @@
   int bid, split;
   xcd_work(bid, split);
   gemm16_body<MODE, BM, BN, WM, WN, TAPV, PIPE, F32, NST, EPF>(a, bid, split);
+}
+
+template <int BM, int BN, int WM, int WN>
+__global__ __launch_bounds__(64 * WM * WN, (occ16<BM, BN, WM, WN, 2>()))
+void gemm16_wgrad_bnbwd_kernel(const GemmArgs a) {
+  int bid, split;
+  xcd_work(bid, split);
+  gemm16_body<MODE_WGRAD, BM, BN, WM, WN, 0, 1, 1, 2, 0, 0, 1>(a, bid, split);
 }
 
 __device__ __forceinline__ void par_tile(const GemmPar& p, int w, int& cls, int& t) {
diff --git a/tmrnet_amd/csrc/gemm16_select.h b/tmrnet_amd/csrc/gemm16_select.h
--- a/tmrnet_amd/csrc/gemm16_select.h
+++ b/tmrnet_amd/csrc/gemm16_select.h
@@ -109,6 +109,10 @@
 extern template int launch_gemm16<MODE_WGRAD, 0>(const GemmArgs&, int, hipStream_t);
 extern template int launch_gemm16<MODE_WGRAD, 1>(const GemmArgs&, int, hipStream_t);
 
+inline bool wgrad_bnbwd_cfg(int cfg) { return cfg == 4 || cfg == 5 || cfg == 7; }
+int launch_gemm16_wgrad_bnbwd(const GemmArgs& a, int splits, hipStream_t st);
+extern long g_wgrad_bnbwd_launches;
+
 template <int BM, int BN, int WM, int WN>
 int launch16_inf16(const GemmArgs& a, bool tapv, dim3 grid, hipStream_t st);
 extern template int launch16_inf16<256, 128, 4, 2>(const GemmArgs&, bool, dim3, hipStream_t);
diff --git a/tmrnet_amd/csrc/gemm16_wgrad_f32.hip b/tmrnet_amd/csrc/gemm16_wgrad_f32.hip
--- a/tmrnet_amd/csrc/gemm16_wgrad_f32.hip
+++ b/tmrnet_amd/csrc/gemm16_wgrad_f32.hip
@@ -2,4 +2,28 @@
 
 namespace tmrg {
 template int launch_gemm16<MODE_WGRAD, 1>(const GemmArgs& a, int splits, hipStream_t st);
+
+int launch_gemm16_wgrad_bnbwd(const GemmArgs& a, int splits, hipStream_t st) {
+  TMR_CHECK_ARG(use16(a, MODE_WGRAD) && a.prec == TMR_MATH_F32,
+                "wgrad_bnbwd: not an fp32 LDS-DMA wgrad");
+  const int cfg = pick_cfg16(a.M, a.N, a.K, MODE_WGRAD, true);
+  TMR_CHECK_ARG(wgrad_bnbwd_cfg(cfg), "wgrad_bnbwd: tile config %d has no dY-producing form", cfg);
+  GemmArgs plain = a;
+  plain.Cold = nullptr;
+  if (const int rc = check16<MODE_WGRAD, 1>(plain, cfg)) return rc;
+  TMR_CHECK_ARG(a.bn_y && a.bn_sc && a.Cold &&
+                    ((((uintptr_t)a.bn_y | (uintptr_t)a.bn_sc | (uintptr_t)a.Cold)) & 15) == 0,
+                "wgrad_bnbwd: y, coefficients and dy must be 16-B aligned");
+  const Cfg16 c = kCfgs16[cfg];
+  const dim3 grid(cdiv(a.M, c.bm) * cdiv(a.N, c.bn), splits, 1);
+  if (grid.x == 0) return 0;
+  switch (cfg) {
+    case 4: hipLaunchKernelGGL((gemm16_wgrad_bnbwd_kernel<64, 256, 1, 4>), grid, dim3(256), 0, st, a); break;
+    case 5: hipLaunchKernelGGL((gemm16_wgrad_bnbwd_kernel<64, 64, 2, 2>), grid, dim3(256), 0, st, a); break;
+    case 7: hipLaunchKernelGGL((gemm16_wgrad_bnbwd_kernel<128, 128, 4, 2>), grid, dim3(512), 0, st, a); break;
+    default: break;
+  }
+  TMR_CHECK_LAUNCH("gemm16_wgrad_bnbwd_kernel");
+  return 0;
 }
+}
diff --git a/tmrnet_amd/csrc/gemm_conv.hip b/tmrnet_amd/csrc/gemm_conv.hip
--- a/tmrnet_amd/csrc/gemm_conv.hip
+++ b/tmrnet_amd/csrc/gemm_conv.hip
@@ -573,6 +573,24 @@
   return bytes;
 }
 
+static int wgrad_reduce(const tmr_conv_desc* d, const float* ws, int sp, long slab, float* dw_oihw,
+                        int c_real, float beta, hipStream_t stream) {
+  const int ntaps = d->r * d->s;
+  if (ntaps > 1 && ntaps <= kReduceTaps) {
+    hipLaunchKernelGGL(wgrad_reduce_taps_kernel, dim3(d->k, cdiv(c_real, 64)), dim3(256), 0,
+                       stream, ws, sp, slab, dw_oihw, ntaps, d->c, c_real, beta);
+    TMR_CHECK_LAUNCH("wgrad_reduce_taps_kernel");
+    return 0;
+  }
+  long total = (long)d->k * ntaps * c_real;
+  int blocks = (int)((total + 255) / 256);
+  if (blocks > 4096) blocks = 4096;
+  hipLaunchKernelGGL(wgrad_reduce_kernel, dim3(blocks), dim3(256), 0, stream, ws, sp, slab,
+                     dw_oihw, d->k, ntaps, d->c, c_real, beta);
+  TMR_CHECK_LAUNCH("wgrad_reduce_kernel");
+  return 0;
+}
+
 static int conv_wgrad_impl(const tmr_conv_desc* d, const float* x, const float* dy,
                            float* dw_oihw, int c_real, float beta, float* ws, size_t ws_bytes,
                            hipStream_t stream) {
@@ -603,20 +621,7 @@
   bool al = aligned16(x) && aligned16(dy) && (d->k % 4 == 0) && a.lds % 4 == 0 && a.ldb % 4 == 0;
   const int rc = launch_gemm<MODE_WGRAD>(a, al, sp, stream);
   if (rc) return rc;
-  const int ntaps = d->r * d->s;
-  if (ntaps > 1 && ntaps <= kReduceTaps) {
-    hipLaunchKernelGGL(wgrad_reduce_taps_kernel, dim3(d->k, cdiv(c_real, 64)), dim3(256), 0,
-                       stream, ws, sp, slab, dw_oihw, ntaps, d->c, c_real, beta);
-    TMR_CHECK_LAUNCH("wgrad_reduce_taps_kernel");
-    return 0;
-  }
-  long total = (long)d->k * ntaps * c_real;
-  int blocks = (int)((total + 255) / 256);
-  if (blocks > 4096) blocks = 4096;
-  hipLaunchKernelGGL(wgrad_reduce_kernel, dim3(blocks), dim3(256), 0, stream, ws, sp, slab,
-                     dw_oihw, d->k, ntaps, d->c, c_real, beta);
-  TMR_CHECK_LAUNCH("wgrad_reduce_kernel");
-  return 0;
+  return wgrad_reduce(d, ws, sp, slab, dw_oihw, c_real, beta, stream);
 }
 
 TMR_API int tmr_conv2d_wgrad(const tmr_conv_desc* d, const float* x, const float* dy,
@@ -628,6 +633,70 @@
                            dw_oihw + (long)g * c.k * c_real * c.r * c.s, c_real,
                            f0 == 0 ? beta : 1.f, ws, ws_bytes, stream);
   });
+}
+
+static const char* wgrad_bnbwd_why(const tmr_conv_desc* d, int c_real, const void* x, const void* g,
+                                   const void* y, const void* dy_out) {
+  if (d->n <= 0 || d->k <= 0 || d->c <= 0 || d->r <= 0 || d->s <= 0) return "empty descriptor";
+  if (d->math != TMR_MATH_F32) return "fp32 math only";
+  if (d->io & (TMR_IO_X_BF16 | TMR_IO_DY_BF16)) return "a bf16 operand";
+  if (ngroups(d) > 1) return "grouped conv";
+  if (frames_per_launch(d) < d->n) return "frame-chunked tensors";
+  if (d->k % 8 != 0) return "output channels not a multiple of 8 (the 8-wide apply's domain)";
+  if (yld_of(d) != d->k) return "g / y / dy must be dense";
+  if (ilog2_exact(d->c) < 2) return "stored input channels must be a power of two >= 4";
+  if (direct_wgrad(d, c_real)) return "the wgrad runs on a direct kernel";
+  if ((((uintptr_t)x | (uintptr_t)g | (uintptr_t)y | (uintptr_t)dy_out) & 15) != 0)
+    return "operands must be 16-B aligned";
+  GemmArgs a;
+  wgrad_fill(d, a);
+  if (!use16(a, MODE_WGRAD)) return "not an LDS-DMA engine wgrad";
+  if (!wgrad_bnbwd_cfg(pick_cfg16(a.M, a.N, a.K, MODE_WGRAD, true)))
+    return "tile config without the fused form (256x256)";
+  return nullptr;
+}
+
+TMR_API int tmr_conv2d_wgrad_bnbwd_ok(const tmr_conv_desc* d, const void* x, const void* g,
+                                      const void* y, const void* dy_out) {
+  return d && !wgrad_bnbwd_why(d, 0, x, g, y, dy_out) ? 1 : 0;
+}
+
+long tmrg::g_wgrad_bnbwd_launches = 0;
+TMR_API long tmr_wgrad_bnbwd_launches(void) {
+  return __atomic_load_n(&g_wgrad_bnbwd_launches, __ATOMIC_RELAXED);
+}
+
+TMR_API int tmr_conv2d_wgrad_bnbwd(const tmr_conv_desc* d, const float* x, const float* g,
+                                   const float* y, const float* coef, float* dy_out,
+                                   float* dw_oihw, int c_real, float beta, float* ws,
+                                   size_t ws_bytes, hipStream_t stream) {
+  TMR_CHECK_ARG(d && x && g && y && coef && dy_out && dw_oihw, "tmr_conv2d_wgrad_bnbwd: null operand");
+  TMR_CHECK_ARG(c_real >= 1 && c_real <= d->c, "tmr_conv2d_wgrad_bnbwd: bad c_real %d", c_real);
+  const char* why = wgrad_bnbwd_why(d, c_real, x, g, y, dy_out);
+  TMR_CHECK_ARG(!why, "tmr_conv2d_wgrad_bnbwd: no fused form (%s); ask tmr_conv2d_wgrad_bnbwd_ok "
+                "and keep tmr_bn_bwd_parts + tmr_conv2d_wgrad", why);
+  TMR_CHECK_ARG(((uintptr_t)coef & 15) == 0, "tmr_conv2d_wgrad_bnbwd: coef must be 16-B aligned");
+  const size_t ybytes = (size_t)d->n * d->ho * d->wo * d->k * sizeof(float);
+  const auto apart = [&](const void* p) {
+    return (const char*)p + ybytes <= (const char*)dy_out || (const char*)dy_out + ybytes <= (const char*)p;
+  };
+  TMR_CHECK_ARG(apart(g) && apart(y), "tmr_conv2d_wgrad_bnbwd: dy_out overlaps g or y");
+  int sp, kc;
+  long slab;
+  wgrad_plan(d, &sp, &kc, &slab);
+  TMR_CHECK_ARG(ws && ws_bytes >= (size_t)sp * slab * sizeof(float),
+                "tmr_conv2d_wgrad_bnbwd: workspace too small (%zu < %zu)", ws_bytes,
+                (size_t)sp * slab * sizeof(float));
+  GemmArgs a;
+  wgrad_fill(d, a);
+  a.A = g; a.B = x; a.C = ws; a.bias = nullptr;
+  a.bn_y = y; a.bn_sc = coef; a.Cold = dy_out;
+  a.kchunk = kc; a.slab = slab;
+  a.Cbytes = clamp_bytes(slab);
+  const int rc = launch_gemm16_wgrad_bnbwd(a, sp, stream);
+  if (rc) return rc;
+  __atomic_fetch_add(&g_wgrad_bnbwd_launches, 1L, __ATOMIC_RELAXED);
+  return wgrad_reduce(d, ws, sp, slab, dw_oihw, c_real, beta, stream);
 }
 
 TMR_API int tmr_gemm_nt(int M, int N, int K, const float* A, int lda, const float* B, int ldb,
diff --git a/tmrnet_amd/ops.py b/tmrnet_amd/ops.py
--- a/tmrnet_amd/ops.py
+++ b/tmrnet_amd/ops.py
@@ -405,6 +405,54 @@
     return out
 
 
+def bn_bwd_parts_coef(y, parts, nparts, mean, inv, gamma):
+    c = y.shape[-1]
+    rows = y.numel() // c
+    nb = query("tmr_bn_parts_ws_bytes", int(nparts), c)
+    off = query("tmr_bn_parts_coef_offset", int(nparts), c)
+    ws = torch.empty(((nb + 7) // 8,), dtype=torch.float64, device=y.device)
+    dgamma = _empty((c,), y); dbeta = _empty((c,), y)
+    call("tmr_bn_bwd_parts_x", None, None, parts, int(nparts), mean, inv, gamma, None, dgamma,
+         dbeta, rows, c, ws, ctypes.c_size_t(ws.numel() * 8), 0, stream_ptr())
+    return ws.view(f32)[off // 4: off // 4 + 3 * c], dgamma, dbeta
+
+
+def _wgrad_bnbwd_desc(x, g, r, s, stride, pad, math, groups):
+    n, h, w, c = x.shape
+    d = conv_desc(n, h, w, c, g.shape[3], r, s, stride, pad, None, math=math, io=_io(x, None, g),
+                  groups=groups)
+    d.x_ld = _nhwc_ld(x, "x")
+    d.y_ld = _nhwc_ld(g, "g")
+    return d
+
+
+def conv_wgrad_bnbwd_ok(x, g, y, r, s, stride, pad, math="fp32", groups=1):
+    if math != "fp32" or not (x.dtype == g.dtype == y.dtype == f32) or g.shape != y.shape:
+        return False
+    if not (g.is_contiguous() and y.is_contiguous()):
+        return False
+    d = _wgrad_bnbwd_desc(x, g, r, s, stride, pad, math, groups)
+    return bool(query("tmr_conv2d_wgrad_bnbwd_ok", ctypes.byref(d), x, g, y, None))
+
+
+def conv_wgrad_bnbwd(x, g, y, coef, r, s, stride, pad, c_real=None, math="fp32"):
+    n, h, w, c = x.shape
+    k = g.shape[3]
+    c_real = c if c_real is None else c_real
+    d = _wgrad_bnbwd_desc(x, g, r, s, stride, pad, math, 1)
+    assert (d.ho, d.wo) == tuple(g.shape[1:3])
+    out = _empty((k, c_real, r, s), x)
+    dy = torch.empty_like(y)
+    ws_bytes = query("tmr_conv2d_wgrad_ws_bytes", ctypes.byref(d))
+    ws = torch.empty(max(1, (ws_bytes + 3) // 4), dtype=f32, device=x.device)
+    with _prof("conv_wgrad" + _SUFFIX[math], 2.0 * n * d.ho * d.wo * k * r * s * c_real,
+               (n, h, w, c, k, r, stride),
+               _esz(x) * n * h * w * c + 3 * 4 * n * d.ho * d.wo * k + 4 * k * r * s * c_real):
+        call("tmr_conv2d_wgrad_bnbwd", ctypes.byref(d), x, g, y, coef, dy, out, int(c_real), 0.0,
+             ws, ctypes.c_size_t(ws.numel() * 4), stream_ptr())
+    return out, dy
+
+
 def gemm_nt(a, b, bias=None, out=None, beta=0.0, M=None, N=None, K=None, lda=None, ldb=None,
             ldc=None):
     M = a.shape[0] if M is None else M
diff --git a/tmrnet_amd/trunk.py b/tmrnet_amd/trunk.py
--- a/tmrnet_amd/trunk.py
+++ b/tmrnet_amd/trunk.py
@@ -70,6 +70,8 @@
 R16 = os.environ.get("TMR_BF16_RESGRAD", "1") != "0"
 
 DS_DUAL = True
+
+WGRAD_BNBWD = True
 
 
 def _ds_dual(g, r3, rd):
@@ -162,16 +164,26 @@
 
 def _conv_bn_bwd(rec, dz, grads, want_dres=False, dx_out=None, dx_beta=0.0, need_dx=True,
                  dres_inplace=False, parts=None, fuse_prev=None, pool=None, dy=None, g16=False,
-                 r16=False):
+                 r16=False, fold=False):
     conv, bn = rec["conv"], rec["bn"]
     s16 = _store16(rec["math"])
     dy_given = dy is not None
+    dw = None
+    kr, ks = conv.weight.shape[2:]
     if dy_given:
         dres = None
     elif pool is not None:
         dy, dg, db = ops.bn_bwd_maxpool(pool[0], pool[1], rec["y"], rec["scale"], rec["shift"],
                                         rec["mean"], rec["inv"], bn.weight.detach(), bf16=s16)
         dres = None
+    elif (parts is not None and fold and WGRAD_BNBWD and rec["math"] == "fp32"
+          and rec.get("groups", 1) == 1
+          and ops.conv_wgrad_bnbwd_ok(rec["x"], dz, rec["y"], kr, ks, rec["stride"], rec["pad"])):
+        coef, dg, db = ops.bn_bwd_parts_coef(rec["y"], parts[0], parts[1], rec["mean"],
+                                             rec["inv"], bn.weight.detach())
+        dw, dy = ops.conv_wgrad_bnbwd(rec["x"], dz, rec["y"], coef, kr, ks, rec["stride"],
+                                      rec["pad"], c_real=rec["c_real"])
+        dres = dz if want_dres else None
     elif parts is not None:
         dy, dg, db = ops.bn_bwd_parts(dz, rec["y"], parts[0], parts[1], rec["mean"], rec["inv"],
                                       bn.weight.detach(), bf16=s16)
@@ -187,9 +199,9 @@
     x = rec["x"]
     k, c, r, s = conv.weight.shape
     grp = rec.get("groups", 1)
-    grads[conv.weight] = ops.conv_wgrad(x, dy, r, s, rec["stride"], rec["pad"],
-                                        c_real=rec["c_real"], math=rec["math"],
-                                        groups=grp)
+    grads[conv.weight] = dw if dw is not None else ops.conv_wgrad(
+        x, dy, r, s, rec["stride"], rec["pad"], c_real=rec["c_real"], math=rec["math"],
+        groups=grp)
     dx, fused = None, None
     if need_dx:
         hw = (x.shape[1], x.shape[2])
@@ -322,8 +334,9 @@
                 del dy3
             else:
                 dz2, dres, fz2 = _conv_bn_bwd(r3, g, grads, want_dres=True, dres_inplace=True,
-                                              parts=pending, fuse_prev=r2, g16=True)
-            dz1, _, fz1 = _conv_bn_bwd(r2, dz2, grads, parts=fz2, fuse_prev=r1, g16=True)
+                                              parts=pending, fuse_prev=r2, g16=True, fold=True)
+            dz1, _, fz1 = _conv_bn_bwd(r2, dz2, grads, parts=fz2, fuse_prev=r1, g16=True,
+                                      fold=True)
             del dz2
             if has_ds:
                 if dyd is not None:
@@ -332,10 +345,10 @@
                 else:
                     dx, _, _ = _conv_bn_bwd(rd, dres, grads)
                 dx, _, pending = _conv_bn_bwd(r1, dz1, grads, parts=fz1, dx_out=dx, dx_beta=1.0,
-                                              fuse_prev=prev3, r16=True)
+                                              fuse_prev=prev3, r16=True, fold=True)
             else:
                 dx, _, pending = _conv_bn_bwd(r1, dz1, grads, parts=fz1, dx_out=dres, dx_beta=1.0,
-                                              fuse_prev=prev3, r16=True)
+                                              fuse_prev=prev3, r16=True, fold=True)
             del dz1, brec, dres
             g = dx
             if ready is not None:
```

New measurement: 3857 frames/s, median of 6. 1.8% higher.
